# simonamtoft/downsampled-diffusion

Hardware: AMD Instinct MI355X
Metric: images/sec (T=1000 sampling), 256x256 dDDPM-x3 (higher is better)
Workload: dtype f32

## Files before the change

### downsampled-diffusion_amd/csrc/conv_wino.hip

```cpp
#include <atomic>
#include <cstdlib>
#include <type_traits>
#include <utility>

#include "cluster_sync.h"
#include "conv_common.h"
#include "pack_elems.h"

namespace ddk {

__device__ __attribute__((aligned(128))) float g_wino_zero[32];

struct WinoParams {
    const float* src0;
    const float* src1;
    const float* wu;
    const float* bias;
    const float* resid;
    float* out;
    int c0, c1, cin;
    int B, H, W, TH, TW;
    int N, tiles;
    int splits, chunks, chunks_per_split;
    long long slab_stride;
    int post_mish;
    FastDivU dTW, dTH;
    float2* gn_part;
    int cpg, groups;
    const float* gn_gamma;
    const float* gn_beta;
    const float* gn_temb;
    const long long* gn_temb_rows;
    int gn_temb_stride;
    float gn_eps;
    float* cl_rec;
    unsigned* cl_cnt;
    unsigned* cl_fail;
    int cl_np;
    float* cl_slab;
    unsigned* cl_pair;
    const float* r1_x;
    const float* r1_w;
    const float* r1_b;
    int r1_cin, r1_ld;
};

constexpr int WBT = 32, WBN = 64;
constexpr int W_V = 4 * WBT * 32, W_U = 4 * WBN * 32;
constexpr int W_STAGE = W_V + W_U, W_NS = 3;
constexpr int W_LDS_FLOATS = W_NS * W_STAGE;
constexpr int W_TP = WBN + 4;
#ifndef DDK_WINO_LP
#define DDK_WINO_LP 4
#endif
constexpr int W_LP = DDK_WINO_LP;
static_assert(4 * 2 * WBT * W_TP <= W_LDS_FLOATS, "epilogue staging fits");

template <bool DGRAD>
__global__ __launch_bounds__(256) void pack_conv_weight_wino_kernel(const float* __restrict__ w, float* __restrict__ dst, int O, int I,
                                                                     int i_pad, long long total, int lo, int wi) {
    for (long long idx = blockIdx.x * 256LL + threadIdx.x; idx < total; idx += (long long)gridDim.x * 256)
        pack_wino_elem<DGRAD>(w, dst, idx, O, I, i_pad, lo, wi);
}

typedef int i32x4 __attribute__((ext_vector_type(4)));
typedef float f32x4 __attribute__((ext_vector_type(4)));

__device__ __forceinline__ i32x4 make_srd(const void* p, unsigned bytes) {
    const unsigned long long a = reinterpret_cast<unsigned long long>(p);
    i32x4 r;
    r.x = __builtin_amdgcn_readfirstlane((int)(unsigned)a);
    r.y = __builtin_amdgcn_readfirstlane((int)(unsigned)((a >> 32) & 0xFFFFu));
    r.z = __builtin_amdgcn_readfirstlane((int)bytes);
    r.w = 0x00020000;
    return r;
}
constexpr unsigned WINO_OOB = 0x80000000u;

__device__ __forceinline__ void buf_load16(f32x4& d, unsigned voff, const i32x4& srd, unsigned soff) {
    asm volatile("buffer_load_dwordx4 %0, %1, %2, %3 offen" : "=v"(d) : "v"(voff), "s"(srd), "s"(soff) : "memory");
}

__device__ __forceinline__ float4 f4add(float4 a, float4 b) { return make_float4(a.x + b.x, a.y + b.y, a.z + b.z, a.w + b.w); }
typedef float wino_f32x4 __attribute__((ext_vector_type(4)));
__device__ __forceinline__ void st_sc1_f4(float* p, float4 v) {
    const wino_f32x4 t = {v.x, v.y, v.z, v.w};
    asm volatile("global_store_dwordx4 %0, %1, off sc1\n\ts_nop 1" ::"v"(p), "v"(t) : "memory");
}
__device__ __forceinline__ void ld_sc1_f4x4(float4& a, float4& b, float4& c, float4& d, const float* pa, const float* pb, const float* pc,
                                            const float* pd) {
    wino_f32x4 x, y, z, w;
    asm volatile("global_load_dwordx4 %0, %4, off sc1\n\tglobal_load_dwordx4 %1, %5, off sc1\n\tglobal_load_dwordx4 %2, %6, off sc1\n\t"
                 "global_load_dwordx4 %3, %7, off sc1\n\ts_waitcnt vmcnt(0)"
                 : "=&v"(x), "=&v"(y), "=&v"(z), "=&v"(w)
                 : "v"(pa), "v"(pb), "v"(pc), "v"(pd)
                 : "memory");
    a = make_float4(x.x, x.y, x.z, x.w); b = make_float4(y.x, y.y, y.z, y.w);
    c = make_float4(z.x, z.y, z.z, z.w); d = make_float4(w.x, w.y, w.z, w.w);
}
__device__ __forceinline__ float4 f4sub(float4 a, float4 b) { return make_float4(a.x - b.x, a.y - b.y, a.z - b.z, a.w - b.w); }

__device__ unsigned long long g_wino_stamps[8 * 1024];

template <int DBG, bool CL = false>
__global__ __launch_bounds__(512) void conv3x3_wino_kernel(const WinoParams p) {
    extern __shared__ __attribute__((aligned(16))) float smem[];
    unsigned long long r_entry = 0;
    if (DBG) r_entry = __builtin_amdgcn_s_memrealtime();
    const int tid = threadIdx.x, lane = tid & 63;
    const int wid = __builtin_amdgcn_readfirstlane(tid >> 6);
    int tile_m, tile_n, split;
    {
        const int nwg = gridDim.x * gridDim.y * gridDim.z;
        const int bid = blockIdx.x + gridDim.x * (blockIdx.y + gridDim.y * blockIdx.z);
        const int q = nwg >> 3, r = nwg & 7, xcd = bid & 7, idx = bid >> 3;
        const int logical = (xcd < r ? xcd * (q + 1) : r * (q + 1) + (xcd - r) * q) + idx;
        tile_n = logical % gridDim.y;
        const int rest = logical / gridDim.y;
        tile_m = rest % gridDim.x;
        split = rest / gridDim.x;
    }
    const int t0 = tile_m * WBT, n0 = tile_n * WBN;
    const int c_begin = split * p.chunks_per_split;
    const int n_chunks = min(p.chunks, c_begin + p.chunks_per_split) - c_begin;
    const int n_stages = n_chunks * 4;
    const unsigned lds_base = (unsigned)(size_t)(__attribute__((address_space(3))) float*)smem;

// ... 326 lines not shown
                    rs[it][0] = rs[it][1] = make_float4(0.f, 0.f, 0.f, 0.f);
                    if (p.resid) {
                        rs[it][0] = *reinterpret_cast<const float4*>(p.resid + oo[it]);
                        rs[it][1] = *reinterpret_cast<const float4*>(p.resid + oo[it] + p.N);
                    }
                }
            };
            if (wid != 0) { load_affine(); load_resid(); }
            if (wid == 0) {
                asm volatile("s_waitcnt vmcnt(0)" ::: "memory");
                if (lane == 0) __hip_atomic_fetch_add(cnt, 1u, __ATOMIC_RELAXED, __HIP_MEMORY_SCOPE_AGENT);
                load_affine();
                load_resid();
                if (lane == 0 && cl_wait_ge<4>(cnt, (unsigned)p.cl_np, p.cl_fail)) *gave_up = 1;
            }
            __syncthreads();
            const unsigned long long* r0 = reinterpret_cast<const unsigned long long*>(p.cl_rec) +
                                           ((long long)image * p.cl_np * gridDim.y + tile_n) * 16 + gl;
            const bool poisoned = *gave_up != 0;
            float rm[8], rq[8];
            cl_load_stats(r0, (long long)gridDim.y * 16, p.cl_np, rm, rq);
            if (tid == 0) cl_depart(cnt, cnt + 1, (unsigned)p.cl_np);
            const float2 st = cl_merge_stats(rm, rq, p.cl_np, 128.0f * (float)p.cpg, p.gn_eps, poisoned);
            const float gmean = st.x, rstd = st.y;
            auto fin = [&](float4 v) {
                return make_float4(mish_f((v.x - gmean) * rstd * ga.x + be.x) + ts.x, mish_f((v.y - gmean) * rstd * ga.y + be.y) + ts.y,
                                   mish_f((v.z - gmean) * rstd * ga.z + be.z) + ts.z, mish_f((v.w - gmean) * rstd * ga.w + be.w) + ts.w);
            };
#pragma unroll
            for (int it = 0; it < 2; ++it) {
                *reinterpret_cast<float4*>(p.out + oo[it]) = f4add(fin(keep[it][0]), rs[it][0]);
                *reinterpret_cast<float4*>(p.out + oo[it] + p.N) = f4add(fin(keep[it][1]), rs[it][1]);
            }
        }
    }
    if (DBG && tid == 0) {
        asm volatile("s_waitcnt vmcnt(0)" ::: "memory");
        const int wg = (blockIdx.x + gridDim.x * (blockIdx.y + gridDim.y * blockIdx.z)) & 1023;
        g_wino_stamps[wg * 8 + 6] = __builtin_amdgcn_s_memrealtime();
        g_wino_stamps[wg * 8 + 7] = 1;
    }
}

#include "conv_wino2_kernel.inc"
#include "conv_winoT_kernel.inc"

enum { WINO_V_OLD = 0, WINO_V_D = 1, WINO_V_F = 2 };
static int wino_variant(int B, int H, int W, int N) {
#ifdef DDK_TUNING
    if (const char* e = getenv("DDK_WINO_VARIANT")) {
        const int v = atoi(e);
        if (v == WINO_V_OLD || v == WINO_V_D || (v == WINO_V_F && N % 128 == 0)) return v;
    }
#endif
    const long long mt = ceil_div((long long)B * (H / 2) * (W / 2), WBT);
    return (N % 128 == 0 && mt * (N / 128) >= 224) ? WINO_V_F : WINO_V_D;
}
static int wino_nt(int variant) { return variant == WINO_V_F ? 128 : WBN; }
bool conv_wino_ok(int kind, int H, int W, int cin, int N) {
    return kind == DDK_CONV3X3_S1 && H >= 2 && W >= 2 && H % 2 == 0 && W % 2 == 0 && cin > 0 && cin % 32 == 0 && N % 64 == 0;
}

int conv_wino_splits(int B, int H, int W, int cin, int N) {
    const long long tiles = (long long)B * (H / 2) * (W / 2);
    const long long wgs = ceil_div(tiles, WBT) * (N / wino_nt(wino_variant(B, H, W, N)));
    const int chunks = cin / 32;
    int s = 1;
    while (wgs * s < 256 && s * 2 <= chunks) s *= 2;
    const int cps = (int)ceil_div(chunks, s);
    return (int)ceil_div(chunks, cps);
}

static int wino_stats_shape_parts(int B, int H, int W, int cin, int N, int groups) {
    if (!conv_wino_ok(DDK_CONV3X3_S1, H, W, cin, N) || groups <= 0 || N % groups) return 0;
    const int cpg = N / groups, tpi = (H / 2) * (W / 2), nt_w = wino_nt(wino_variant(B, H, W, N));
    if (cpg % 4 || nt_w % cpg || nt_w / cpg > 8 || tpi % WBT || tpi / WBT > 32) return 0;
    return tpi / WBT;
}
int conv_wino_stats_parts(int B, int H, int W, int cin, int N, int groups) {
    if (conv_wino_splits(B, H, W, cin, N) != 1) return 0;
    return wino_stats_shape_parts(B, H, W, cin, N, groups);
}

bool convT_wino_ok(int H, int W, int cin, int N) {
    return H >= 2 && W >= 2 && H % 2 == 0 && W % 2 == 0 && cin > 0 && cin % 32 == 0 && N > 0 && N % WT_NT == 0;
}
int convT_wino_splits(int B, int H, int W, int cin, int N) {
    const long long wgs = ceil_div((long long)B * (H / 2) * (W / 2), WBT) * (N / WT_NT) * 4;
    const int chunks = cin / 32;
    int s = 1;
    while (wgs * s < 256 && s * 2 <= chunks) s *= 2;
    const int cps = (int)ceil_div(chunks, s);
    return (int)ceil_div(chunks, cps);
}
int convT_wino_forward(const ddk_conv_args& a, int splits, hipStream_t st) {
    WinoParams p{};
    p.src0 = a.src0; p.wu = a.weight_wino; p.bias = a.bias; p.out = a.out;
    p.c0 = a.c0; p.c1 = 0; p.cin = a.c0;
    p.B = a.B; p.H = a.H; p.W = a.W; p.TH = a.H / 2; p.TW = a.W / 2;
    p.N = a.N; p.tiles = a.B * p.TH * p.TW;
    p.chunks = p.cin / 32;
    p.chunks_per_split = (int)ceil_div(p.chunks, splits);
    p.splits = (int)ceil_div(p.chunks, p.chunks_per_split);
    p.slab_stride = (long long)a.B * (2 * a.H) * (2 * a.W) * a.N;
    p.dTW = make_fastdiv_u((unsigned)p.TW);
    p.dTH = make_fastdiv_u((unsigned)p.TH);
    if (p.splits > 1) p.out = static_cast<float*>(a.workspace);
    dim3 grid((unsigned)ceil_div(p.tiles, WBT), (unsigned)(a.N / WT_NT), (unsigned)(4 * p.splits));
#ifdef DDK_TUNING
    if (getenv("DDK_WINO_STAMPS")) {
        hipLaunchKernelGGL(convT_wino_kernel<1>, grid, dim3(1024), WT_LDS_FL * sizeof(float), st, p);
        return check_launch("convT_wino_kernel<dbg>");
    }
#endif
    hipLaunchKernelGGL(convT_wino_kernel<0>, grid, dim3(1024), WT_LDS_FL * sizeof(float), st, p);
    return check_launch("convT_wino_kernel");
}

int conv_wino_init_device() {
    DDK_HIP(hipFuncSetAttribute(reinterpret_cast<const void*>(&convT_wino_kernel<0>), hipFuncAttributeMaxDynamicSharedMemorySize,
                                (int)(WT_LDS_FL * sizeof(float))));
#ifdef DDK_TUNING
    DDK_HIP(hipFuncSetAttribute(reinterpret_cast<const void*>(&convT_wino_kernel<1>), hipFuncAttributeMaxDynamicSharedMemorySize,
                                (int)(WT_LDS_FL * sizeof(float))));
#endif
    DDK_HIP(hipFuncSetAttribute(reinterpret_cast<const void*>(&conv3x3_wino_kernel<0>), hipFuncAttributeMaxDynamicSharedMemorySize,
                                (int)(W_LDS_FLOATS * sizeof(float))));
    DDK_HIP(hipFuncSetAttribute(reinterpret_cast<const void*>(&conv3x3_wino_kernel<0, true>), hipFuncAttributeMaxDynamicSharedMemorySize,
                                (int)(W_LDS_FLOATS * sizeof(float))));
    DDK_HIP(hipFuncSetAttribute(reinterpret_cast<const void*>(&conv3x3_wino2_kernel<2, 0, false>), hipFuncAttributeMaxDynamicSharedMemorySize,
                                (int)(W2<2>::LDS_FL * sizeof(float))));
    DDK_HIP(hipFuncSetAttribute(reinterpret_cast<const void*>(&conv3x3_wino2_kernel<2, 0, true>), hipFuncAttributeMaxDynamicSharedMemorySize,
                                (int)(W2<2>::LDS_FL * sizeof(float))));
    DDK_HIP(hipFuncSetAttribute(reinterpret_cast<const void*>(&conv3x3_wino2_kernel<4, 0, false>), hipFuncAttributeMaxDynamicSharedMemorySize,
                                (int)(W2<4>::LDS_FL * sizeof(float))));
    DDK_HIP(hipFuncSetAttribute(reinterpret_cast<const void*>(&conv3x3_wino2_kernel<4, 0, true>), hipFuncAttributeMaxDynamicSharedMemorySize,
                                (int)(W2<4>::LDS_FL * sizeof(float))));
#ifdef DDK_TUNING
#define W2_DBG_ATTR(P_, D_) DDK_HIP(hipFuncSetAttribute(reinterpret_cast<const void*>(&conv3x3_wino2_kernel<P_, D_, false>), \
                                                hipFuncAttributeMaxDynamicSharedMemorySize, (int)(W2<P_>::LDS_FL * sizeof(float))))
    W2_DBG_ATTR(2, 1); W2_DBG_ATTR(2, 7); W2_DBG_ATTR(2, 9); W2_DBG_ATTR(2, 15); W2_DBG_ATTR(2, 17);
    W2_DBG_ATTR(4, 1); W2_DBG_ATTR(4, 7); W2_DBG_ATTR(4, 9); W2_DBG_ATTR(4, 15); W2_DBG_ATTR(4, 17);
#undef W2_DBG_ATTR
    DDK_HIP(hipFuncSetAttribute(reinterpret_cast<const void*>(&conv3x3_wino_kernel<1>), hipFuncAttributeMaxDynamicSharedMemorySize, (int)(W_LDS_FLOATS * sizeof(float))));
    DDK_HIP(hipFuncSetAttribute(reinterpret_cast<const void*>(&conv3x3_wino_kernel<2>), hipFuncAttributeMaxDynamicSharedMemorySize, (int)(W_LDS_FLOATS * sizeof(float))));
    DDK_HIP(hipFuncSetAttribute(reinterpret_cast<const void*>(&conv3x3_wino_kernel<3>), hipFuncAttributeMaxDynamicSharedMemorySize, (int)(W_LDS_FLOATS * sizeof(float))));
    DDK_HIP(hipFuncSetAttribute(reinterpret_cast<const void*>(&conv3x3_wino_kernel<4>), hipFuncAttributeMaxDynamicSharedMemorySize, (int)(W_LDS_FLOATS * sizeof(float))));
#endif
    return DDK_OK;
}

int conv_wino_cluster_np(int B, int H, int W, int cin, int N, int groups) {
    const int np = conv_wino_stats_parts(B, H, W, cin, N, groups);
    if (np <= 0 || np > 8) return 0;
    const int nt_w = wino_nt(wino_variant(B, H, W, N));
    if (N / groups > 32 || nt_w % (N / groups)) return 0;
    if (nt_w / (N / groups) > 8) return 0;
    const long long mt = (long long)B * np, nt = N / nt_w;
    if ((mt * nt) % 8) return 0;
    const long long run = mt * nt / 8;
    const long long per_round = run < 32 ? run : 32;
    if (run % (np * nt) || per_round % (np * nt)) return 0;
    return np;
}
int conv_wino_cluster_split_np(int B, int H, int W, int cin, int N, int groups, int* splits_out) {
    if (!conv_wino_ok(DDK_CONV3X3_S1, H, W, cin, N)) return 0;
    const int splits = conv_wino_splits(B, H, W, cin, N);
    if (splits_out) *splits_out = splits;
    if (splits <= 1 || splits > 4) return 0;
    const int np = wino_stats_shape_parts(B, H, W, cin, N, groups);
    if (np <= 0 || np > 8) return 0;
    const int variant = wino_variant(B, H, W, N);
    if (variant != WINO_V_D) return 0;
    const int nt_w = wino_nt(variant);
    if (N / groups > 32 || nt_w % (N / groups) || nt_w / (N / groups) > 8) return 0;
    const long long mt = (long long)B * np, nt = N / nt_w;
    if (mt * nt * splits > 256) return 0;
    return np;
}
size_t conv_wino_cluster_pair_words(int B, int H, int W, int N) {
    return (size_t)ceil_div((long long)B * (H / 2) * (W / 2), WBT) * (size_t)(N / WBN) * 16;
}
size_t conv_wino_cluster_ws_floats(int B, int H, int W, int N) {
    const long long mt = (long long)B * (H / 2) * (W / 2) / WBT, nt = N / WBN;
    return (size_t)(mt * nt * 32 + (long long)B * nt * 16);
}

bool conv_wino_cluster_device_ok() {
    static std::atomic<int> cached[64];
    int dev = 0;
    if (hipGetDevice(&dev) != hipSuccess || dev < 0 || dev >= 64) return false;
    int v = cached[dev].load(std::memory_order_relaxed);
    if (v == 0) {
        int cus = 0, xccs = 0;
        bool ok = hipDeviceGetAttribute(&cus, hipDeviceAttributeMultiprocessorCount, dev) == hipSuccess && cus == 256;
        ok = ok && hipDeviceGetAttribute(&xccs, hipDeviceAttributeNumberOfXccs, dev) == hipSuccess && xccs == 8;
        ok = ok && !getenv("HSA_CU_MASK") && !getenv("ROC_GLOBAL_CU_MASK");
        (void)hipGetLastError();
        v = ok ? 1 : 2;
        cached[dev].store(v, std::memory_order_relaxed);
    }
    return v == 1;
}

bool conv_wino_variant_new(int B, int H, int W, int N) { return wino_variant(B, H, W, N) != WINO_V_OLD; }

int conv_wino_forward(const ddk_conv_args& a, int splits, hipStream_t st, const WinoGnFuse* fuse) {
    WinoParams p{};
    if (fuse) {
        const int np = splits == 1 ? conv_wino_cluster_np(a.B, a.H, a.W, a.c0 + a.c1, a.N, fuse->groups)
                                   : conv_wino_cluster_split_np(a.B, a.H, a.W, a.c0 + a.c1, a.N, fuse->groups, nullptr);
        DDK_REQUIRE(np > 0 && !a.post_mish && !a.gn_partials, "conv(wino): shape not eligible for the in-launch GroupNorm");
        if (splits > 1) {
            DDK_REQUIRE(fuse->pairs && a.workspace && aligned16(a.workspace) && !fuse->res_x,
                        "conv(wino, cluster): a split shape needs pair counters and the slab workspace");
// ... 236 lines not shown
```

### downsampled-diffusion_amd/csrc/conv_wino2_kernel.inc

```

template <int... I, class F>
__device__ __forceinline__ void static_for_impl(std::integer_sequence<int, I...>, F&& f) { (f(std::integral_constant<int, I>{}), ...); }
template <int N, class F>
__device__ __forceinline__ void static_for(F&& f) { static_for_impl(std::make_integer_sequence<int, N>{}, f); }

#ifndef DDK_WINO2_LP_F
#define DDK_WINO2_LP_F 8
#endif
#ifndef DDK_WINO2_LP_D
#define DDK_WINO2_LP_D 4
#endif
template <int P>
struct W2 {
    static constexpr int NT = 256 / P;
    static constexpr int NB = NT / 32;
    static constexpr int SPC = 16 / P;
    static constexpr int SPR = 4 / P;
    static constexpr int V_FL = P * WBT * 32;
    static constexpr int U_FL = P * NT * 32;
    static constexpr int STAGE = V_FL + U_FL;
    static constexpr int PPI = NT / 8;
    static constexpr int TP = NT + 4;
    static constexpr int T_FL = 4 * 2 * WBT * TP;
    static constexpr int LDS_FL = (3 * STAGE > T_FL + 320) ? 3 * STAGE : T_FL + 320;
    static constexpr int QUADS = NT / 4;
    static constexpr int ITEMS = 2 * WBT * QUADS / 512;
    static constexpr int LPL = P == 2 ? DDK_WINO2_LP_F : DDK_WINO2_LP_D;
    static constexpr int LPM = (32 - 4 * LPL) / 8;
    static_assert(4 * LPL + 8 * LPM == 32 && LPL % 2 == 0 && LPM % 2 == 0, "piece split: (8,0), (4,2) or (0,4)");
};
#ifndef DDK_WINO2_STAGGER
#define DDK_WINO2_STAGGER 1
#endif
constexpr bool W2_STAGGER = DDK_WINO2_STAGGER != 0;

__device__ unsigned long long g_wino_timeline[12 * 8 * 2];

template <int P, int DBG, bool CL>
__global__ __launch_bounds__(768) void conv3x3_wino2_kernel(const WinoParams p) {
    using G = W2<P>;
    constexpr int NT = G::NT, SPC = G::SPC, SPR = G::SPR, STAGE = G::STAGE, V_FL = G::V_FL;
    extern __shared__ __attribute__((aligned(16))) float smem[];
    unsigned long long r_entry = 0;
    if (DBG) r_entry = __builtin_amdgcn_s_memrealtime();
    const int tid = threadIdx.x, lane = tid & 63;
    const int wid = __builtin_amdgcn_readfirstlane(tid >> 6);
    int tile_m, tile_n, split;
    {
        const int nwg = gridDim.x * gridDim.y * gridDim.z;
        const int bid = blockIdx.x + gridDim.x * (blockIdx.y + gridDim.y * blockIdx.z);
        const int q = nwg >> 3, r = nwg & 7, xcd = bid & 7, idx = bid >> 3;
        const int logical = (xcd < r ? xcd * (q + 1) : r * (q + 1) + (xcd - r) * q) + idx;
        tile_n = logical % gridDim.y;
        const int rest = logical / gridDim.y;
        tile_m = rest % gridDim.x;
        split = rest / gridDim.x;
    }
    const int t0 = tile_m * WBT, n0 = tile_n * NT;
    const int c_begin = split * p.chunks_per_split;
    const int n_chunks = min(p.chunks, c_begin + p.chunks_per_split) - c_begin;
    const int n_stages = n_chunks * SPC;
    const unsigned lds_base = (unsigned)(size_t)(__attribute__((address_space(3))) float*)smem;
    const int prow = lane >> 3, ppos = lane & 7;
    const unsigned uv_even = (unsigned)((prow * 32 + ((ppos ^ (prow >> 1)) << 2)) * 4);
    const unsigned uv_odd = (unsigned)((prow * 32 + ((ppos ^ (4 + (prow >> 1))) << 2)) * 4);
    auto issue_u = [&](int T, int buf, int g_first, auto count) {
        const int chunk = c_begin + T / SPC, st = T % SPC;
        const float* base = p.wu + (((long long)chunk * 16 + P * st) * p.N + n0) * 32;
        const unsigned dst = lds_base + (unsigned)((buf * STAGE + V_FL) * 4);
#pragma unroll
        for (int j = 0; j < decltype(count)::value; ++j) {
            const int g = g_first + j;
            const int image = g / G::PPI, rb = g % G::PPI;
            lds_dma16_s(base + ((long long)image * p.N + rb * 8) * 32, (j & 1) ? uv_odd : uv_even, dst + (unsigned)(g * 1024));
        }
    };

    if (wid >= 8) {
        const int lw = wid - 8;
        const int lt = lw * 64 + lane;
        const int t = lt >> 3, cq = lt & 7;
        __builtin_amdgcn_s_setprio(3);
        const int g = t0 + t;
        const bool tile_ok = g < p.tiles;
        const unsigned gg = tile_ok ? (unsigned)g : 0u;
        const unsigned tmp = fdiv_u(gg, p.dTW);
        const int tx = (int)(gg - tmp * (unsigned)p.TW);
        const unsigned bq = fdiv_u(tmp, p.dTH);
        const int ty = (int)(tmp - bq * (unsigned)p.TH), b = (int)bq;
        const int py0 = 2 * ty - 1, px0 = 2 * tx - 1;
        const int pix0 = (b * p.H + py0) * p.W + px0;
        unsigned mask = 0;
#pragma unroll
        for (int dy = 0; dy < 4; ++dy)
#pragma unroll
            for (int dx = 0; dx < 4; ++dx)
                if (tile_ok && (unsigned)(py0 + dy) < (unsigned)p.H && (unsigned)(px0 + dx) < (unsigned)p.W) mask |= 1u << (dy * 4 + dx);
        const i32x4 srd0 = make_srd(p.src0, (unsigned)((long long)p.B * p.H * p.W * p.c0 * 4));
        const i32x4 srd1 = make_srd(p.src1 ? p.src1 : p.src0, (unsigned)((long long)p.B * p.H * p.W * (p.src1 ? p.c1 : p.c0) * 4));
        unsigned voff[16];
        int cur_src = -1;
        auto set_source = [&](int which) {
            const int cs = which == 0 ? p.c0 : p.c1;
#pragma unroll
            for (int dy = 0; dy < 4; ++dy)
#pragma unroll
                for (int dx = 0; dx < 4; ++dx)
                    voff[dy * 4 + dx] = ((mask >> (dy * 4 + dx)) & 1u) ? (unsigned)(((pix0 + dy * p.W + dx) * cs + cq * 4) * 4) : WINO_OOB;
            cur_src = which;
        };
        const int v_off = t * 32 + ((cq ^ ((t >> 1) & 7)) << 2);
        f32x4 d[16];
        auto load_row = [&](int chunk, int row) {
            const int cc = chunk << 5;
            const bool first = cc < p.c0;
            if ((first ? 0 : 1) != cur_src) set_source(first ? 0 : 1);
            const unsigned soff = (unsigned)((first ? cc : cc - p.c0) * 4);
            i32x4 srd;
            srd.x = first ? srd0.x : srd1.x; srd.y = first ? srd0.y : srd1.y; srd.z = first ? srd0.z : srd1.z; srd.w = srd0.w;
#pragma unroll
            for (int dy = 0; dy < 4; ++dy)
                if (dy == row) {
// ... 169 lines not shown
                            frag(a[1], b[1], As, Bs, 0);
                            __builtin_amdgcn_sched_barrier(0);
                            mma4(acc[(s + SPC - 1) % SPC], a[0], b[0]);
                        }
                        frag(a[0], b[0], As, Bs, 1);
                        __builtin_amdgcn_sched_barrier(0);
                        mma4(acc[s], a[1], b[1]);
                        dma();
                        frag(a[1], b[1], As, Bs, 2);
                        __builtin_amdgcn_sched_barrier(0);
                        mma4(acc[s], a[0], b[0]);
                        frag(a[0], b[0], As, Bs, 3);
                        __builtin_amdgcn_sched_barrier(0);
                        mma4(acc[s], a[1], b[1]);
                    }
                    if (more && !(DBG & 4)) wait_vmcnt<G::LPM>(); else wait_vmcnt<0>();
                    unsigned long long tA = 0, tB = 0;
                    if (DBG) { asm volatile("s_memtime %0\n\ts_waitcnt lgkmcnt(0)" : "=s"(tA)::"memory"); }
                    __builtin_amdgcn_s_barrier();
                    if (DBG) { asm volatile("s_memtime %0\n\ts_waitcnt lgkmcnt(0)" : "=s"(tB)::"memory"); c_wait += tB - tA; if (c_mma == 0) c_mma = tA; }
                    if ((DBG & 16) && blockIdx.x + blockIdx.y + blockIdx.z == 0 && S >= 8 && S < 16 && lane == 0) {
                        g_wino_timeline[(wid * 8 + (S - 8)) * 2] = tA;
                        g_wino_timeline[(wid * 8 + (S - 8)) * 2 + 1] = tB;
                    }
                    buf = nbuf;
                    ++S;
                });
            }
            if (STG) mma4(acc[SPC - 1], a[0], b[0]);
        };
        if (W2_STAGGER && wid >= 4) mloop(std::true_type{}); else mloop(std::false_type{});
        if (DBG && lane == 0 && wid == 0) {
            const int wg = (blockIdx.x + gridDim.x * (blockIdx.y + gridDim.y * blockIdx.z)) & 1023;
            unsigned long long tE;
            asm volatile("s_memtime %0\n\ts_waitcnt lgkmcnt(0)" : "=s"(tE)::"memory");
            g_wino_stamps[wg * 8 + 0] = r_entry;
            g_wino_stamps[wg * 8 + 1] = r_loop0;
            g_wino_stamps[wg * 8 + 2] = __builtin_amdgcn_s_memrealtime();
            g_wino_stamps[wg * 8 + 3] = c_wait;
            g_wino_stamps[wg * 8 + 4] = tE - c_mma;
            g_wino_stamps[wg * 8 + 5] = (unsigned long long)n_stages;
        }
    }
    {
        constexpr int TP = G::TP;
#pragma unroll
        for (int r = 0; r < 16; ++r) {
            const int row = (r & 3) + 8 * (r >> 2) + 4 * (lane >> 5);
            const int col = nb * 32 + (lane & 31);
            if constexpr (P == 4) {
                float* Ts = smem + pp * (2 * WBT * TP);
                const float m0 = acc[0][r], m1 = acc[1][r], m2 = acc[2][r], m3 = acc[3][r];
                Ts[row * TP + col] = (m0 + m1) + m2;
                Ts[(WBT + row) * TP + col] = (m1 - m2) - m3;
            } else {
                const float l0 = acc[0][r], l1 = acc[2][r], l2 = acc[4][r], l3 = acc[6][r];
                const float h0 = acc[1][r], h1 = acc[3][r], h2 = acc[5][r], h3 = acc[7][r];
                const float tl0 = (l0 + l1) + l2, tl1 = (l1 - l2) - l3;
                const float th0 = (h0 + h1) + h2, th1 = (h1 - h2) - h3;
                float* B0 = smem + (pp * 2 + 0) * (2 * WBT * TP);
                float* B1 = smem + (pp * 2 + 1) * (2 * WBT * TP);
                if (pp == 0) {
                    B0[row * TP + col] = tl0 + th0;          B0[(WBT + row) * TP + col] = tl1 + th1;
                    B1[row * TP + col] = -th0;               B1[(WBT + row) * TP + col] = -th1;
                } else {
                    B0[row * TP + col] = tl0;                B0[(WBT + row) * TP + col] = tl1;
                    B1[row * TP + col] = tl0 - th0;          B1[(WBT + row) * TP + col] = tl1 - th1;
                }
            }
        }
    }
    __syncthreads();

    constexpr int TP = G::TP, QUADS = G::QUADS, ITEMS = G::ITEMS;
    constexpr bool CLS = CL && P == 4;
    const bool partner = CLS && split > 0;
    const bool direct = p.splits == 1 || (CLS && !partner);
    float* outp = p.splits == 1 ? p.out : CLS ? p.cl_slab + (long long)(split - 1) * p.slab_stride : p.out + (long long)split * p.slab_stride;
    float4 keep[ITEMS][2];
    long long oo[ITEMS];
    int opix[ITEMS];
    const int cq = tid & (QUADS - 1);
    const int gn = n0 + cq * 4;
#pragma unroll
    for (int it = 0; it < ITEMS; ++it) {
        const int item = tid + it * 512;
        const int t = item / (2 * QUADS), a = (item / QUADS) & 1;
        const int g = t0 + t;
        keep[it][0] = keep[it][1] = make_float4(0.f, 0.f, 0.f, 0.f);
        oo[it] = -1;
        opix[it] = 0;
        if (g >= p.tiles || gn >= p.N) continue;
        const float* tp = smem + (a * WBT + t) * TP + cq * 4;
        const float4 q0 = *reinterpret_cast<const float4*>(tp);
        const float4 q1 = *reinterpret_cast<const float4*>(tp + 1 * (2 * WBT * TP));
        const float4 q2 = *reinterpret_cast<const float4*>(tp + 2 * (2 * WBT * TP));
        const float4 q3 = *reinterpret_cast<const float4*>(tp + 3 * (2 * WBT * TP));
        float4 y0, y1;
        if constexpr (P == 4) {
            y0 = f4add(f4add(q0, q1), q2);
            y1 = f4sub(f4sub(q1, q2), q3);
        } else {
            y0 = f4add(q0, q2);
            y1 = f4add(q1, q3);
        }
        const unsigned tmp = fdiv_u((unsigned)g, p.dTW);
        const int tx = g - (int)tmp * p.TW;
        const unsigned bq = fdiv_u(tmp, p.dTH);
        const int ty = (int)tmp - (int)bq * p.TH;
        const long long o0 = ((((long long)bq * p.H + 2 * ty + a) * p.W) + 2 * tx) * p.N + gn;
        oo[it] = o0;
        opix[it] = ((int)bq * p.H + 2 * ty + a) * p.W + 2 * tx;
        if (direct) {
            if (p.bias) {
                const float4 bb = *reinterpret_cast<const float4*>(p.bias + gn);
                y0 = f4add(y0, bb);
                y1 = f4add(y1, bb);
            }
            if (!CL && p.resid) {
                y0 = f4add(y0, *reinterpret_cast<const float4*>(p.resid + o0));
                y1 = f4add(y1, *reinterpret_cast<const float4*>(p.resid + o0 + p.N));
            }
            if (p.post_mish) {
                y0 = make_float4(mish_f(y0.x), mish_f(y0.y), mish_f(y0.z), mish_f(y0.w));
                y1 = make_float4(mish_f(y1.x), mish_f(y1.y), mish_f(y1.z), mish_f(y1.w));
            }
        }
        if (!CL) {
            *reinterpret_cast<float4*>(outp + o0) = y0;
            *reinterpret_cast<float4*>(outp + o0 + p.N) = y1;
        } else if (CLS && partner) {
            st_sc1_f4(outp + o0, y0);
            st_sc1_f4(outp + o0 + p.N, y1);
        }
        keep[it][0] = y0;
        keep[it][1] = y1;
    }
    if (CLS && p.splits > 1) {
        unsigned* pair = p.cl_pair + ((long long)tile_m * gridDim.y + tile_n) * 16;
        if (partner) {
            asm volatile("s_waitcnt vmcnt(0)" ::: "memory");
            __syncthreads();
            if (tid == 0) __hip_atomic_fetch_add(pair, 1u, __ATOMIC_RELAXED, __HIP_MEMORY_SCOPE_AGENT);
            return;
        }
        int* pair_gave_up = reinterpret_cast<int*>(smem + G::T_FL + 258);
        if (tid == 0) {
            *pair_gave_up = 0;
            const unsigned want = (unsigned)p.splits - 1u;
            if (cl_wait_ge<2>(pair, want, p.cl_fail)) *pair_gave_up = 1;
            __hip_atomic_store(pair, 0u, __ATOMIC_RELAXED, __HIP_MEMORY_SCOPE_AGENT);
        }
        __syncthreads();
        const bool pair_poisoned = *pair_gave_up != 0;
        for (int s = 1; s < p.splits; ++s) {
            const float* sl = p.cl_slab + (long long)(s - 1) * p.slab_stride;
            static_assert(ITEMS % 2 == 0, "two items per load group");
#pragma unroll
            for (int it = 0; it < ITEMS; it += 2) {
                float4 a0, a1, b0, b1;
                ld_sc1_f4x4(a0, a1, b0, b1, sl + oo[it], sl + oo[it] + p.N, sl + oo[it + 1], sl + oo[it + 1] + p.N);
                keep[it][0] = f4add(keep[it][0], a0);
                keep[it][1] = f4add(keep[it][1], a1);
                keep[it + 1][0] = f4add(keep[it + 1][0], b0);
                keep[it + 1][1] = f4add(keep[it + 1][1], b1);
            }
        }
        if (pair_poisoned) {
#pragma unroll
            for (int it = 0; it < ITEMS; ++it) keep[it][0].x = __builtin_nanf("");
        }
    }
    if (CL || p.gn_part) {
        const int qpg = p.cpg >> 2;
        const int gl = cq / qpg;
        float* red = smem + G::T_FL;
        auto group_sum = [&](float v, float* rd) {
            for (int o = 1; o < qpg; o <<= 1) v += __shfl_xor(v, o, 64);
#pragma unroll
            for (int o = QUADS; o < 64; o <<= 1) v += __shfl_xor(v, o, 64);
            if (lane < QUADS && (cq & (qpg - 1)) == 0) rd[wid * 16 + gl] = v;
            asm volatile("s_waitcnt lgkmcnt(0)\n\ts_barrier" ::: "memory");
            float t = rd[gl];
#pragma unroll
            for (int w = 1; w < 8; ++w) t += rd[w * 16 + gl];
            return t;
        };
        auto sum4 = [](float4 v) { return (v.x + v.y) + (v.z + v.w); };
        const float inv = 1.0f / (float)(4 * WBT * p.cpg);
        float s1 = 0.f;
#pragma unroll
        for (int it = 0; it < ITEMS; ++it) s1 += sum4(keep[it][0]) + sum4(keep[it][1]);
// ... 116 lines not shown
```

### downsampled-diffusion_amd/csrc/ddk_internal.h

```cpp
#pragma once
#include <hip/hip_runtime.h>

#include <cstdarg>
#include <cstddef>
#include <cstdint>
#include <cstdio>

#include "ddk.h"

#ifdef DDK_HOST_SANITIZE
#include "host_sanitize.h"
#endif

namespace ddk {

void set_error(const char* fmt, ...);

inline int fail_arg(const char* what) {
    set_error("bad argument: %s", what);
    return DDK_ERR_ARG;
}

inline int check_launch(const char* what) {
    hipError_t e = hipGetLastError();
// ... 62 lines not shown
    return v;
}

__device__ __forceinline__ float block_sum(float v, float* red) {
    v = wave_sum(v);
    const int lane = threadIdx.x & 63, wid = threadIdx.x >> 6, nw = blockDim.x >> 6;
    __syncthreads();
    if (lane == 0) red[wid] = v;
    __syncthreads();
    float t = (lane < nw) ? red[lane] : 0.0f;
    t = wave_sum(t);
    return t;
}

__device__ __forceinline__ float block_max(float v, float* red) {
    v = wave_max(v);
    const int lane = threadIdx.x & 63, wid = threadIdx.x >> 6, nw = blockDim.x >> 6;
    __syncthreads();
    if (lane == 0) red[wid] = v;
    __syncthreads();
    float t = (lane < nw) ? red[lane] : -INFINITY;
    t = wave_max(t);
    return t;
}

int ensure_device_init();
int conv_init_device();
int wgrad_init_device();

size_t conv_workspace_bytes(int kind, int B, int H, int W, int cin, int N);
struct ConvLnFold {
    const float* c1;
    const float* c2;
    float eps;
};
struct WinoGnFuse {
    const float* gamma;
    const float* beta;
    const float* temb;
    const long long* temb_rows;
    int temb_stride;
    float eps;
    int groups;
    float* records;
    unsigned* counters;
    unsigned* fail;
    unsigned* pairs = nullptr;
    const float* res_x = nullptr;
    const float* res_w = nullptr;
    const float* res_b = nullptr;
    int res_cin = 0, res_ld = 0;
};
bool conv_ln_fold_ok(int B, int H, int W, int cin, int N);
int conv_forward(const ddk_conv_args& a, hipStream_t st, const ConvLnFold* ln = nullptr, const WinoGnFuse* fuse = nullptr);
int conv_splits(int kind, int B, int H, int W, int cin, int N);
bool conv_wino_ok(int kind, int H, int W, int cin, int N);
int conv_wino_splits(int B, int H, int W, int cin, int N);
int conv_wino_forward(const ddk_conv_args& a, int splits, hipStream_t st, const WinoGnFuse* fuse = nullptr);
int conv_wino_cluster_np(int B, int H, int W, int cin, int N, int groups);
int conv_wino_cluster_split_np(int B, int H, int W, int cin, int N, int groups, int* splits_out);
size_t conv_wino_cluster_pair_words(int B, int H, int W, int N);
bool conv_wino_variant_new(int B, int H, int W, int N);
bool conv_wino_cluster_device_ok();
size_t conv_wino_cluster_ws_floats(int B, int H, int W, int N);
unsigned conv_wino_cluster_timeouts();
unsigned conv_first_cluster_timeouts();
unsigned level_chain_cluster_timeouts();
unsigned attention_cluster_timeouts();
constexpr size_t CL_PAIR_WORDS = 128 * 16;
inline size_t cl_fail_offset(int B) { return (size_t)B * 8 * 16; }
inline size_t cl_front_floats(int B) { return cl_fail_offset(B) + 16; }
inline size_t cl_chain_offset(int B) { return cl_front_floats(B); }
inline size_t cl_pair_offset(int B) { return cl_chain_offset(B) + (size_t)B * 64; }
inline size_t cl_attn_offset(int B) { return cl_pair_offset(B) + CL_PAIR_WORDS; }
inline size_t cl_counter_floats(int B) { return cl_attn_offset(B) + (size_t)B * 4 * 32; }
struct ClWords { unsigned* counters; unsigned* fail; };
inline ClWords cl_words(float* cl, int B) { return {reinterpret_cast<unsigned*>(cl), reinterpret_cast<unsigned*>(cl + cl_fail_offset(B))}; }
int cluster_fail_check(unsigned* word, hipStream_t st, const char* who, const char* tail);
bool convT_wino_ok(int H, int W, int cin, int N);
int convT_wino_splits(int B, int H, int W, int cin, int N);
int convT_wino_forward(const ddk_conv_args& a, int splits, hipStream_t st);
int conv_wino_init_device();
int conv_wino_stats_parts(int B, int H, int W, int cin, int N, int groups);
bool conv_first_ok(int cin, int N, int H, int W, int groups);
int conv_first(const float* x, const float* wp, const float* bias, float* out, float* gn_partials, int B, int H, int W, int cin, int N,
               int groups, int64_t* counter, int64_t* t_cur, hipStream_t st);
int conv_first_init_device();
bool conv_first_gn_ok(int cin, int N, int H, int W, int groups);
size_t conv_first_gn_ws_floats(int B, int H, int W);
int conv_first_gn(const float* x, const float* wp, const float* bias, const float* gamma, const float* beta, const float* temb,
                  int temb_stride, const long long* temb_rows, float eps, float* out, int B, int H, int W, int cin, int N, int groups,
                  float* records, unsigned* counters, unsigned* fail, int64_t* counter, int64_t* t_cur, hipStream_t st);
bool conv1x1_sm_ok(long long M, int c0, int c1, int N);
int conv1x1_sm(const float* src0, int c0, const float* src1, int c1, const float* w, const float* bias, const float* resid, float* out,
               long long M, int N, const ConvLnFold* ln, hipStream_t st);
int conv1x1_sm_init_device();
bool conv1x1_stream_ok(long long M, int cin, int N);
int conv1x1_stream(const float* x, int cin, const float* w, const float* bias, const float* dmish_src, const float* resid, float* out,
                   float* mish_out, long long M, int N, int pre_mish, int post_mish, hipStream_t st);
bool conv1x1_ws_ok(long long M, int K, int N);
int conv1x1_ws(const float* x, const float* w, const float* bias, const float* resid, float* out, long long M, int N, const ConvLnFold* ln,
               hipStream_t st, int images = 0);
int conv1x1_ws_init_device();
struct AddendSlabs {
    int n = 1;
    long long stride = 0;
    const float* bias = nullptr;
};
bool conv_gn_local_ok(int H, int W, int cin, int c0, int N, int groups);
int conv_gn_local(const float* src0, int c0, const float* src1, int c1, const float* w, const float* bias, const float* gamma,
                  const float* beta, const float* temb, int temb_stride, const long long* temb_rows, const float* addend, float* out,
                  int B, int H, int W, int N, int groups, float eps, hipStream_t st, const AddendSlabs& as = AddendSlabs(),
                  const AddendSlabs& src_slabs = AddendSlabs());
int conv_gn_local_init_device();
bool conv_gn_wlocal_ok(int H, int W, int cin, int c0, int N, int groups);
int conv_gn_wlocal(const float* src0, int c0, const float* src1, int c1, const float* w, const float* bias, const float* gamma,
                   const float* beta, const float* temb, int temb_stride, const long long* temb_rows, const float* addend, float* out,
                   int B, int H, int W, int N, int groups, float eps, hipStream_t st, const AddendSlabs& as = AddendSlabs(),
                   const AddendSlabs& src_slabs = AddendSlabs());
double conv_flops(int kind, int B, int H, int W, int cin, int N);
size_t groupnorm_workspace_bytes(int B, int HW, int C, int groups);
int gn_train_nsplit(int HW, int cpg);
int gn_stats_partials(const float* x, float* part, int B, int HW, int C, int groups, int ns, hipStream_t st);
int groupnorm_mish(const float* x, const float* gamma, const float* beta, const float* temb, int temb_stride,
                   const float* addend, float* out, int B, int HW, int C, int groups, float eps, void* ws, size_t ws_bytes,
                   hipStream_t st, const long long* temb_rows = nullptr);
int groupnorm_mish_ex(const float* x, int nslab, long long slab_stride, const float* cbias, const float* gamma,
                      const float* beta, const float* temb, int temb_stride, const float* addend, float* out, int B, int HW, int C,
                      int groups, float eps, void* ws, size_t ws_bytes, hipStream_t st, const long long* temb_rows = nullptr);
int groupnorm_mish_parts(const float* x, const float* part, int np, const float* gamma, const float* beta, const float* temb,
                         int temb_stride, const float* addend, float* out, int B, int HW, int C, int groups, float eps, hipStream_t st,
                         const long long* temb_rows = nullptr, const float* rc_x = nullptr, const float* rc_w = nullptr,
                         const float* rc_b = nullptr, int rc_cin = 0, int rc_ld = 0);
int chan_layernorm(const float* x, const float* g, const float* b, float* out, long long M, int C, float eps, hipStream_t st);
int groupnorm_mish_generic(const float* x, const float* gamma, const float* beta, const float* temb, int temb_stride, const float* addend,
                           float* out, int B, int HW, int CP, int C, int groups, float eps, hipStream_t st, const long long* temb_rows = nullptr);
int chan_layernorm_generic(const float* x, const float* g, const float* b, float* out, long long M, int CP, int C, float eps, hipStream_t st);
int unary(int op, const float* x, float* out, long long n, hipStream_t st);
int add(const float* a, const float* b, float* out, long long n, hipStream_t st);
int avgpool2(const float* x, float* out, int B, int H, int W, int C, hipStream_t st);
int upsample_nearest2(const float* x, float* out, int B, int H, int W, int C, hipStream_t st);
size_t linattn_context_workspace_bytes(int B, int HW, int heads);
int linattn_context(const float* qkv, float* ctx, int B, int HW, int heads, void* workspace, size_t workspace_bytes, hipStream_t st,
                    bool kv_only = false);
bool attn_fold_ok(int C, int heads);
bool attn_kvctx_ok(int B, int HW, int C, int heads);
size_t attn_kvctx_workspace_bytes(int B, int HW);
int attn_kvctx(const float* x, const float* w_kv, const float* c1, const float* c2, float ln_eps, float* ctx, int B, int HW, void* workspace,
               size_t workspace_bytes, hipStream_t st);
size_t attn_fold_out_floats(int B);
int attn_fold(const float* ctx, const float* wqg, const float* c1q, const float* c2q, const float* wout, const float* bout, float* A,
              float* a1, float* a2, int B, int C, int heads, hipStream_t st);
int linattn_apply(const float* qkv, const float* ctx, float* out, int B, int HW, int heads, hipStream_t st);
int linattn_fused_small(const float* qkv, float* ctx, float* out, int B, int HW, int heads, hipStream_t st);
bool attn_split_ok(int B, int HW, int C, int heads);
size_t attn_split_counter_words(int B);
size_t attn_split_record_floats(int B);
int attn_split(const float* x, const float* w, const float* c1, const float* c2, float ln_eps, float* ctx, float* out, int B, int HW, int C,
               unsigned* counters, float* records, unsigned* fail, hipStream_t st);
bool linattn_small_qkv_ok(int HW, int C);
int linattn_small_qkv_init_device();
int qkv_operand_pack(const float* lnw, float* wop, int heads, int cp, hipStream_t st);
int linattn_small_qkv(const float* x, const float* wop, const float* c1, const float* c2, float ln_eps, float* ctx, float* out, int B, int HW,
                      int C, int heads, hipStream_t st);
int time_mlp(const int64_t* t, const float* freqs, const float* w1t, const float* b1, const float* w2t, const float* b2,
             float* act, float* raw, int B, int dim, hipStream_t st);
// ... 117 lines not shown
```

### downsampled-diffusion_amd/csrc/unet_plan.hip

```cpp
#include <algorithm>
#include <mutex>
#include <string>
#include <vector>

#include "ddk_internal.h"
#include "level_chain.h"

namespace ddk {

constexpr int HEADS = 4;
constexpr int HIDDEN = HEADS * 32;
constexpr int GROUPS = 8;
constexpr float GN_EPS = 1e-5f, LN_EPS = 1e-5f;

static inline int pad32(int c) { return (c + 31) / 32 * 32; }

enum PackKind { PK_COPY = 0, PK_CONV = 1, PK_CONVT = 2, PK_LINEAR_T = 3, PK_WINO = 4, PK_LOCAL = 5, PK_WLOCAL = 6, PK_FIRST = 7, PK_CONVT_WINO = 8,
                PK_ROWS = 9 , PK_LOCAL1 = 10 ,
                PK_CONVT_LOCAL = 11  };

struct Slot {
    std::string name;
    long long numel;
    int kind;
// ... 12 lines not shown
    size_t wl = 0;
    bool has_wl = false;
    size_t wwl = 0;
    bool has_wwl = false;
    size_t wf = 0;
    bool has_wf = false;
    size_t wl1 = 0;
    bool has_wl1 = false;
    size_t wtl = 0;
    bool has_wtl = false;
};
struct NormW { size_t g = 0, b = 0; int c_real = 0; };
struct ResW {
    int ci = 0, ci_pad = 0, co = 0, temb_off = 0, ci_real = 0, co_real = 0;
    ConvW c1, c2, res;
    NormW n1, n2;
    bool has_res = false;
};
struct AttnW {
    int c = 0, c_real = 0;
    NormW ln;
    ConvW qkv, out;
    size_t qkv_lnw = 0, ln_c1 = 0, ln_c2 = 0;
    size_t qkv_op = 0;
};

}

using namespace ddk;

struct ChainKey {
    StepKind kind;
    const void* bufs[14];
    const void* ws;
    const void* noise;
    int B, H, W, t_start, device;
    unsigned long long pack_epoch;
    int restore_n = 0;
    bool restore_mask = false;
    int restore_gray = 0;
    bool operator==(const ChainKey& o) const {
        for (int i = 0; i < 14; ++i)
            if (bufs[i] != o.bufs[i]) return false;
        return kind == o.kind && ws == o.ws && noise == o.noise && B == o.B && H == o.H && W == o.W && t_start == o.t_start &&
               device == o.device && pack_epoch == o.pack_epoch && restore_n == o.restore_n && restore_mask == o.restore_mask && restore_gray == o.restore_gray;
    }
};
struct SamplerGraph {
    ChainKey key;
    hipGraph_t graph = nullptr;
    hipGraphExec_t exec = nullptr;
    hipGraph_t graph_multi = nullptr;
    hipGraphExec_t exec_multi = nullptr;
    hipEvent_t done = nullptr;
    unsigned long long last_use = 0;
};
constexpr int SAMPLER_MULTI = 16;

struct ddk_unet {
    std::mutex mu;
    std::vector<SamplerGraph> graphs;
    unsigned long long use_clock = 0;
    unsigned long long pack_epoch = 0;
    struct {
        const void* ws = nullptr;
        int t_start = -1, B = 0, H = 0, W = 0;
        unsigned long long pack_epoch = 0;
        std::vector<int64_t> map;
    } table;
    ddk_unet_config cfg;
    int cluster_gn = 1;
    int cluster_limit = 1 << 30;
    int cluster_np_max = 8;
    bool cluster_split = true;
    bool attn_kvctx = true;
    bool attn_split = true;
    bool fold_down_reduce = false;
    bool restore_fused = true;
    bool first_gn = true;
    int level_chain = 9;
    int level_chain_max_batch = 32;
    int attn_fold_min_hw = 256;
    bool attn_fold = true;
    bool generic = false;
    std::vector<int> dimp;
    std::vector<Slot> slots;
    size_t packed_floats = 0;
    int L = 0;
    std::vector<int> dims;
    int time_dim = 0, temb_total = 0;
    size_t freqs = 0, w1t = 0, b1 = 0, w2t = 0, b2 = 0, temb_wt = 0, temb_bias = 0;
    std::vector<ResW> down_res, up_res;
    std::vector<AttnW> down_attn, up_attn;
    std::vector<ConvW> down_conv, up_conv;
    ResW mid1, mid2;
    AttnW mid_attn;
    ConvW final_conv;
    NormW final_norm;
    size_t final_w = 0, final_b = 0;

    size_t alloc(size_t n) {
        const size_t o = packed_floats;
        packed_floats += (n + 3) / 4 * 4;
        return o;
    }
    size_t add_copy(const std::string& name, long long n) {
        const size_t o = alloc((size_t)n);
        slots.push_back(Slot{name, n, PK_COPY, o, 0, 0, 0, 0, 0, 0, 0});
        return o;
    }
    void add_copy_at(const std::string& name, long long n, size_t off) {
        slots.push_back(Slot{name, n, PK_COPY, off, 0, 0, 0, 0, 0, 0, 0});
    }
    ConvW add_conv(const std::string& prefix, int cout, int cin, int k, bool bias, bool gn_follows = false, int split = 0, bool local = false) {
        ConvW c;
        c.cin = cin; c.cin_pad = split > 0 ? pad32(split) + pad32(cin - split) : pad32(cin); c.cout = cout;
        const int cout_rows = pad32(cout);
        c.w = alloc((size_t)cout_rows * k * k * c.cin_pad);
        Slot sl{prefix + "weight", (long long)cout * cin * k * k, PK_CONV, c.w, cout, cin, k, k, c.cin_pad, 0, 0};
        if (split > 0 && c.cin_pad != cin) { sl.split = split; sl.split_pad = pad32(split); }
        slots.push_back(sl);
        c.has_bias = bias;
        if (bias) {
            c.b = alloc((size_t)cout_rows);
            slots.push_back(Slot{prefix + "bias", cout, PK_COPY, c.b, 0, 0, 0, 0, 0, 0, 0});
        }
        if (generic) return c;
        if (k == 1 && bias && cout % 32 == 0 && c.cin_pad == cin && cin % 32 == 0) {
            c.wl1 = alloc((size_t)cout * c.cin_pad);
            c.has_wl1 = true;
            slots.push_back(Slot{prefix + "weight", (long long)cout * cin, PK_LOCAL1, c.wl1, cout, cin, 1, 1, c.cin_pad, 0, 0});
        }
        if (k == 3 && cout % 64 == 0) {
            c.wu = alloc((size_t)16 * cout * c.cin_pad);
            c.has_wu = true;
            slots.push_back(Slot{prefix + "weight", (long long)cout * cin * k * k, PK_WINO, c.wu, cout, cin, k, k, c.cin_pad, 0, 0});
        }
        if (k == 3 && (gn_follows || local) && cout % 32 == 0) {
            c.wl = alloc((size_t)9 * cout * c.cin_pad);
            c.has_wl = true;
            slots.push_back(Slot{prefix + "weight", (long long)cout * cin * k * k, PK_LOCAL, c.wl, cout, cin, k, k, c.cin_pad, 0, 0});
            if (gn_follows && (c.cin_pad <= 320 || c.cin_pad == 512)) {
                c.wwl = alloc((size_t)16 * cout * c.cin_pad);
                c.has_wwl = true;
                slots.push_back(Slot{prefix + "weight", (long long)cout * cin * k * k, PK_WLOCAL, c.wwl, cout, cin, k, k, c.cin_pad, 0, 0});
            }
        }
        return c;
    }
    ConvW add_convT(const std::string& prefix, int ch, bool local = false) {
        ConvW c;
        c.cin = ch; c.cin_pad = pad32(ch); c.cout = ch;
        c.w = alloc((size_t)16 * pad32(ch) * pad32(ch));
        slots.push_back(Slot{prefix + "weight", (long long)16 * ch * ch, PK_CONVT, c.w, ch, ch, 4, 4, pad32(ch), 0, 0});
        c.has_bias = true;
        c.b = alloc((size_t)pad32(ch));
        slots.push_back(Slot{prefix + "bias", ch, PK_COPY, c.b, 0, 0, 0, 0, 0, 0, 0});
        if (local && ch % 32 == 0 && !generic) {
            c.wtl = alloc((size_t)16 * ch * ch);
            c.has_wtl = true;
            slots.push_back(Slot{prefix + "weight", (long long)16 * ch * ch, PK_CONVT_LOCAL, c.wtl, ch, ch, 4, 4, ch, 0, 0});
        }
        if (ch % 128 == 0) {
            c.wu = alloc((size_t)36 * ch * ch);
            c.has_wu = true;
            slots.push_back(Slot{prefix + "weight", (long long)16 * ch * ch, PK_CONVT_WINO, c.wu, ch, ch, 4, 4, ch, 0, 0});
// ... 49 lines not shown
        return a;
    }
};

static int total_temb(const ddk_unet& u) {
    int tot = 0;
    for (int l = 0; l < u.L; ++l) tot += 2 * u.dims[l + 1];
    tot += 2 * u.dims[u.L];
    for (int i = 0; i < u.L - 1; ++i) tot += 2 * u.dims[u.L - 1 - i];
    return tot;
}

extern "C" ddk_unet* ddk_unet_create(const ddk_unet_config* cfg) {
    if (!cfg || cfg->n_levels < 1 || cfg->n_levels > 8 || cfg->in_ch < 1 || cfg->chan < 8 || cfg->chan % 8 ||
        cfg->chan > 512) {
        set_error("unet_create: need 1 <= n_levels <= 8, in_ch >= 1, unet_chan a multiple of 8 in [8, 512]");
        return nullptr;
    }
    for (int i = 0; i < cfg->n_levels; ++i)
        if (cfg->mults[i] < 1) { set_error("unet_create: unet_dims entries must be >= 1"); return nullptr; }
    if (cfg->mults[0] != 1) {
        set_error("unet_create: unet_dims[0] must be 1 (the reference's final Block(dim, dim) meets dim * unet_dims[0] channels "
                  "otherwise and raises, unet.py:69-72)");
        return nullptr;
    }
    {
        int ndev = 0;
        if (hipGetDeviceCount(&ndev) == hipSuccess && ndev > 0 && ensure_device_init() != DDK_OK) return nullptr;
        (void)hipGetLastError();
    }
    ddk_unet* u = new ddk_unet();
    u->cfg = *cfg;
    u->L = cfg->n_levels;
    u->generic = cfg->chan % 32 != 0;
    for (int i = 0; i < cfg->n_levels; ++i)
        if (cfg->chan * cfg->mults[i] > 512) { set_error("unet_create: level widths above 512 channels are not supported"); delete u; return nullptr; }
    u->dims.push_back(cfg->in_ch);
    for (int i = 0; i < u->L; ++i) u->dims.push_back(cfg->chan * cfg->mults[i]);
    for (int d : u->dims) u->dimp.push_back(u->generic ? pad32(d) : d);
    u->time_dim = cfg->chan;
    u->temb_total = total_temb(*u);
    const int td = u->time_dim;

    u->freqs = u->add_copy("@sinusoidal_freqs", td / 2);
    u->w1t = u->alloc((size_t)td * 4 * td);
    u->slots.push_back(Slot{"time_mlp.1.weight", (long long)4 * td * td, PK_LINEAR_T, u->w1t, 4 * td, td, 0, 0, 0, 4 * td, 0});
    u->b1 = u->add_copy("time_mlp.1.bias", 4 * td);
    u->w2t = u->alloc((size_t)4 * td * td);
    u->slots.push_back(Slot{"time_mlp.3.weight", (long long)4 * td * td, PK_LINEAR_T, u->w2t, td, 4 * td, 0, 0, 0, td, 0});
    u->b2 = u->add_copy("time_mlp.3.bias", td);
    u->temb_wt = u->alloc((size_t)td * u->temb_total);
    u->temb_bias = u->alloc((size_t)u->temb_total);

    int cur = 0;
    for (int l = 0; l < u->L; ++l) {
        const std::string p = "downs." + std::to_string(l) + ".";
        const int ci = u->dims[l], co = u->dims[l + 1];
        u->down_res.push_back(u->add_res(p + "0.", ci, co, cur));
        if (l == 0 && ci <= 8 && co <= 256 && !u->generic) {
            ConvW& c1 = u->down_res[0].c1;
            const int K2 = (9 * ci + 1) / 2;
            c1.wf = u->alloc((size_t)(co / 32) * K2 * 64);
            c1.has_wf = true;
            u->slots.push_back(Slot{p + "0.block1.block.0.weight", (long long)co * ci * 9, PK_FIRST, c1.wf, co, ci, 3, 3, 0, 0, 0});
        }
        u->down_res.push_back(u->add_res(p + "1.", co, co, cur));
        u->down_attn.push_back(u->add_attn(p + "2.", co));
        if (l < u->L - 1) u->down_conv.push_back(u->add_conv(p + "3.conv.", co, co, 3, true, false, 0, l == u->L - 2));
    }
    const int mid = u->dims[u->L];
    u->mid1 = u->add_res("mid_block1.", mid, mid, cur);
    u->mid_attn = u->add_attn("mid_attn.", mid);
    u->mid2 = u->add_res("mid_block2.", mid, mid, cur);
    for (int i = 0; i < u->L - 1; ++i) {
        const std::string p = "ups." + std::to_string(i) + ".";
        const int din = u->dims[u->L - 1 - i], dout = u->dims[u->L - i];
        u->up_res.push_back(u->add_res(p + "0.", 2 * dout, din, cur, dout));
        u->up_res.push_back(u->add_res(p + "1.", din, din, cur));
        u->up_attn.push_back(u->add_attn(p + "2.", din));
        u->up_conv.push_back(u->add_convT(p + "3.conv.", din, i == 0));
    }
    u->final_conv = u->add_conv("final_conv.0.block.0.", cfg->chan, cfg->chan, 3, true, true);
    u->final_norm = u->add_norm("final_conv.0.block.1.weight", "final_conv.0.block.1.bias", cfg->chan);
    if (u->generic) {
        u->final_w = u->alloc((size_t)cfg->in_ch * pad32(cfg->chan));
        u->slots.push_back(Slot{"final_conv.1.weight", (long long)cfg->in_ch * cfg->chan, PK_ROWS, u->final_w, cfg->in_ch, cfg->chan, 0, 0, 0,
                                pad32(cfg->chan), 0});
    } else {
        u->final_w = u->add_copy("final_conv.1.weight", (long long)cfg->in_ch * cfg->chan);
    }
    u->final_b = u->add_copy("final_conv.1.bias", cfg->in_ch);
    if (cur != u->temb_total) {
        set_error("unet_create: internal temb accounting mismatch");
        delete u;
        return nullptr;
    }
    return u;
}

static void drop_graphs(ddk_unet* u) {
    for (SamplerGraph& g : u->graphs) {
        if (g.exec) (void)hipGraphExecDestroy(g.exec);
        if (g.graph) (void)hipGraphDestroy(g.graph);
        if (g.exec_multi) (void)hipGraphExecDestroy(g.exec_multi);
        if (g.graph_multi) (void)hipGraphDestroy(g.graph_multi);
        if (g.done) (void)hipEventDestroy(g.done);
    }
    u->graphs.clear();
    u->table.ws = nullptr;
}

extern "C" void ddk_unet_destroy(ddk_unet* u) {
    if (!u) return;
    if (!u->graphs.empty()) (void)hipDeviceSynchronize();
    drop_graphs(u);
    delete u;
}

extern "C" int ddk_sampler_invalidate(ddk_unet* u) {
    DDK_REQUIRE(u, "sampler_invalidate: null plan");
    std::lock_guard<std::mutex> lock(u->mu);
    if (!u->graphs.empty()) DDK_HIP(hipDeviceSynchronize());
    drop_graphs(u);
    return DDK_OK;
}
static void destroy_entry(SamplerGraph& g) {
    if (g.done) { (void)hipEventSynchronize(g.done); (void)hipEventDestroy(g.done); }
    if (g.exec) (void)hipGraphExecDestroy(g.exec);
    if (g.graph) (void)hipGraphDestroy(g.graph);
    if (g.exec_multi) (void)hipGraphExecDestroy(g.exec_multi);
    if (g.graph_multi) (void)hipGraphDestroy(g.graph_multi);
}

extern "C" int ddk_sampler_release_workspace(ddk_unet* u, const void* workspace) {
    DDK_REQUIRE(u && workspace, "sampler_release_workspace: arguments");
    std::lock_guard<std::mutex> lock(u->mu);
    for (size_t i = 0; i < u->graphs.size();) {
        if (u->graphs[i].key.ws == workspace) {
            destroy_entry(u->graphs[i]);
            u->graphs.erase(u->graphs.begin() + (long)i);
        } else {
            ++i;
        }
    }
    if (u->table.ws == workspace) u->table.ws = nullptr;
    return DDK_OK;
}

extern "C" int ddk_unet_set_option(ddk_unet* u, int option, int value) {
    DDK_REQUIRE(u, "unet_set_option: null plan");
    static const struct {
        int option;
        bool drops_graphs;
        void (*set)(ddk_unet&, int);
    } options[] = {
        {DDK_OPT_CLUSTER_GROUPNORM, true, [](ddk_unet& p, int v) { p.cluster_gn = v < 0 ? 0 : v > 2 ? 2 : v; }},
        {DDK_OPT_ATTENTION_FOLD, true, [](ddk_unet& p, int v) { p.attn_fold = v != 0; }},
        {DDK_OPT_ATTENTION_KV_CONTEXT, true, [](ddk_unet& p, int v) { p.attn_kvctx = v != 0; }},
        {DDK_OPT_FIRST_GROUPNORM, true, [](ddk_unet& p, int v) { p.first_gn = v != 0; }},
        {DDK_OPT_RESTORE_FUSED_TAIL, true, [](ddk_unet& p, int v) { p.restore_fused = v != 0; }},
        {DDK_OPT_ATTENTION_SPLIT, true, [](ddk_unet& p, int v) { p.attn_split = v != 0; }},
        {DDK_OPT_LEVEL_CHAIN, true, [](ddk_unet& p, int v) {
             p.level_chain = v == 1 ? 9 : v == 2 ? 1 : v == 3 ? 15 : v == 4 ? 6 : v == 8 ? 2 : v == 16 ? 4 : v != 0 ? 9 : 0;
         }},
        {DDK_OPT_FOLD_DOWNSAMPLE_REDUCE, true, [](ddk_unet& p, int v) { p.fold_down_reduce = v != 0; }},
        {10, true, [](ddk_unet& p, int v) { p.level_chain_max_batch = v; }},
        {9, true, [](ddk_unet& p, int v) { p.attn_fold_min_hw = v; }},
        {2, false, [](ddk_unet& p, int v) { p.cluster_limit = v; }},
        {4, true, [](ddk_unet& p, int v) { p.cluster_np_max = v; }},
        {11, true, [](ddk_unet& p, int v) { p.cluster_split = v != 0; }},
    };
    for (const auto& o : options) {
        if (o.option != option) continue;
        std::lock_guard<std::mutex> lock(u->mu);
        if (o.drops_graphs) {
            if (!u->graphs.empty()) DDK_HIP(hipDeviceSynchronize());
            drop_graphs(u);
        }
        o.set(*u, value);
        return DDK_OK;
    }
    return fail_arg("unet_set_option: unknown option");
}
extern "C" unsigned ddk_debug_cluster_timeouts(void) {
    unsigned sum = 0;
    for (unsigned v : {ddk::conv_wino_cluster_timeouts(), ddk::conv_first_cluster_timeouts(), ddk::level_chain_cluster_timeouts(),
                       ddk::attention_cluster_timeouts()}) {
        if (v == ~0u) return ~0u;
        sum += v;
    }
    return sum;
}
extern "C" int ddk_unet_num_slots(const ddk_unet* u) { return u ? (int)u->slots.size() : 0; }
extern "C" const char* ddk_unet_slot_name(const ddk_unet* u, int slot) {
    return (u && slot >= 0 && slot < (int)u->slots.size()) ? u->slots[slot].name.c_str() : nullptr;
}
extern "C" long long ddk_unet_slot_numel(const ddk_unet* u, int slot) {
    return (u && slot >= 0 && slot < (int)u->slots.size()) ? u->slots[slot].numel : -1;
}
extern "C" size_t ddk_unet_packed_bytes(const ddk_unet* u) { return u ? u->packed_floats * sizeof(float) : 0; }

__global__ __launch_bounds__(64) void ln_fold_kernel(const float* __restrict__ w, const float* __restrict__ g, const float* __restrict__ b,
                                                     float* __restrict__ wg, float* __restrict__ c1, float* __restrict__ c2, int C, int cp) {
    const int n = blockIdx.x;
    float s1 = 0.f, s2 = 0.f;
    for (int c = threadIdx.x; c < cp; c += 64) {
        const float wv = w[(long long)n * cp + c];
        const float gv = c < C ? g[c] : 0.f, bv = c < C ? b[c] : 0.f;
        wg[(long long)n * cp + c] = wv * gv;
        s1 += wv * gv;
        s2 += wv * bv;
    }
    s1 = wave_sum(s1);
    s2 = wave_sum(s2);
    if (threadIdx.x == 0) { c1[n] = s1; c2[n] = s2; }
}

static int fold_attn(const AttnW& a, float* P, hipStream_t st) {
    hipLaunchKernelGGL(ln_fold_kernel, dim3(3 * HIDDEN), dim3(64), 0, st, P + a.qkv.w, P + a.ln.g, P + a.ln.b, P + a.qkv_lnw, P + a.ln_c1,
                       P + a.ln_c2, a.c, pad32(a.c));
    DDK_TRY(check_launch("ln_fold_kernel"));
    return qkv_operand_pack(P + a.qkv_lnw, P + a.qkv_op, HEADS, pad32(a.c), st);
}

static void weights_changed(const ddk_unet* u) {
    ddk_unet* m = const_cast<ddk_unet*>(u);
    std::lock_guard<std::mutex> lock(m->mu);
    ++m->pack_epoch;
}

extern "C" int ddk_unet_finalize_pack(const ddk_unet* u, void* packed, ddk_stream_t s) {
    DDK_REQUIRE(u && packed, "unet_finalize_pack: arguments");
    weights_changed(u);
    for (const AttnW& a : u->attn_all) DDK_TRY(fold_attn(a, static_cast<float*>(packed), as_stream(s)));
    return DDK_OK;
}

extern "C" int ddk_unet_pack_slot(const ddk_unet* u, int slot, const float* canonical, void* packed, ddk_stream_t s) {
    DDK_REQUIRE(u && canonical && packed && slot >= 0 && slot < (int)u->slots.size(), "unet_pack_slot: arguments");
    const Slot& sl = u->slots[slot];
    float* dst = static_cast<float*>(packed) + sl.off;
    weights_changed(u);
    int rc;
    switch (sl.kind) {
        case PK_COPY:
            DDK_HIP(hipMemcpyAsync(dst, canonical, (size_t)sl.numel * sizeof(float), hipMemcpyDeviceToDevice, as_stream(s)));
            rc = DDK_OK;
            break;
        case PK_CONV:
            rc = sl.split > 0 ? ddk_pack_conv_weight_split(canonical, dst, sl.O, sl.I, sl.KH, sl.KW, sl.i_pad, sl.split, sl.split_pad, s)
                              : ddk_pack_conv_weight(canonical, dst, sl.O, sl.I, sl.KH, sl.KW, sl.i_pad, s);
            break;
        case PK_CONVT: rc = sl.i_pad == sl.I ? ddk_pack_convT_weight(canonical, dst, sl.I, sl.O, s)
                                             : ddk_pack_convT_weight_padded(canonical, dst, sl.I, sl.O, sl.i_pad, s); break;
        case PK_ROWS:
            DDK_HIP(hipMemcpy2DAsync(dst, (size_t)sl.ld * sizeof(float), canonical, (size_t)sl.I * sizeof(float), (size_t)sl.I * sizeof(float),
                                     (size_t)sl.O, hipMemcpyDeviceToDevice, as_stream(s)));
            rc = DDK_OK;
            break;
        case PK_LINEAR_T: rc = ddk_pack_linear_T(canonical, dst, sl.O, sl.I, sl.ld, sl.col0, s); break;
        case PK_WINO: rc = ddk_pack_conv_weight_wino(canonical, dst, sl.O, sl.I, sl.i_pad, s); break;
        case PK_LOCAL: rc = ddk_pack_conv_weight_local(canonical, dst, sl.O, sl.I, sl.i_pad, s); break;
        case PK_LOCAL1: rc = ddk_pack_conv1x1_weight_local(canonical, dst, sl.O, sl.I, sl.i_pad, s); break;
        case PK_CONVT_LOCAL: rc = ddk_pack_convT_weight_local(canonical, dst, sl.I, sl.O, s); break;
        case PK_WLOCAL: rc = ddk_pack_conv_weight_wino_local(canonical, dst, sl.O, sl.I, sl.i_pad, s); break;
        case PK_FIRST: rc = ddk_pack_conv_weight_first(canonical, dst, sl.O, sl.I, s); break;
        case PK_CONVT_WINO: rc = ddk_pack_convT_weight_wino(canonical, dst, sl.I, sl.O, sl.i_pad, s); break;
        default: return fail_arg("unet_pack_slot: slot kind");
    }
    DDK_TRY(rc);
    if (sl.attn >= 0) DDK_TRY(fold_attn(u->attn_all[sl.attn], static_cast<float*>(packed), as_stream(s)));
    return DDK_OK;
}

namespace ddk {

struct Layout {
    size_t act = 0;
    size_t qkv = 0, o = 0, ctx = 0, splitk = 0, gn_ws = 0, cl = 0, chain = 0;
    std::vector<size_t> skip;
    size_t xpad = 0, temb = 0, tact = 0;
    size_t off_A = 0, off_B = 0, off_C = 0, off_raw = 0, off_a1 = 0, off_res = 0, off_xn = 0, off_qkv = 0, off_o = 0, off_ctx = 0,
           off_splitk = 0, off_gn = 0, off_xpad = 0, off_temb = 0, off_tact = 0, off_cl = 0, off_chain = 0;
    std::vector<size_t> off_skip;
    size_t total = 0;
};

static size_t al4(size_t n) { return (n + 3) / 4 * 4; }

static void upd(size_t& m, size_t v) { if (v > m) m = v; }

static bool convT_wino_use(int B, int H, int W, int cin, int N) {
    return convT_wino_ok(H, W, cin, N) && convT_wino_splits(B, H, W, cin, N) <= 2;
}
static bool use_wino(const ConvW& cw, int H, int W, int cin, int N) {
    return cw.has_wu && conv_wino_ok(DDK_CONV3X3_S1, H, W, cin, N);
}
static size_t conv3_ws_floats(const ConvW& cw, int B, int H, int W, int cin, int N) {
    if (!use_wino(cw, H, W, cin, N)) return conv_workspace_bytes(DDK_CONV3X3_S1, B, H, W, cin, N) / 4;
    const int s = conv_wino_splits(B, H, W, cin, N);
    return s > 1 ? (size_t)s * B * H * W * N : 0;
}

constexpr int CHAIN_BUFS = 18;
constexpr int CHAIN8_BUFS = 5;

static void res_sizes(const ResW& r, int B, int H, int W, Layout& ly) {
    const size_t M = (size_t)B * H * W;
    upd(ly.act, M * r.co);
    upd(ly.splitk, conv3_ws_floats(r.c1, B, H, W, r.ci_pad, r.co));
    upd(ly.splitk, conv3_ws_floats(r.c2, B, H, W, r.co, r.co));
    if (r.has_res) upd(ly.splitk, conv_workspace_bytes(DDK_CONV1X1, B, H, W, r.ci_pad, r.co) / 4);
    upd(ly.gn_ws, groupnorm_workspace_bytes(B, H * W, r.co, GROUPS) / 4);
    upd(ly.gn_ws, (size_t)2 * GROUPS * (M / 128 + 1));
    upd(ly.cl, cl_counter_floats(B) + conv_wino_cluster_ws_floats(B, H, W, r.co));
    if (H * W % 128 == 0 && H * W / 128 <= 8) upd(ly.cl, cl_counter_floats(B) + conv_first_gn_ws_floats(B, H, W));
}

static void attn_sizes(const AttnW& a, int B, int H, int W, Layout& ly) {
    const size_t M = (size_t)B * H * W;
    upd(ly.act, M * a.c);
    upd(ly.qkv, M * 3 * HIDDEN);
    upd(ly.o, M * HIDDEN);
    upd(ly.ctx, (size_t)B * HEADS * 32 * 32);
    upd(ly.splitk, linattn_context_workspace_bytes(B, H * W, HEADS) / 4);
    if (attn_kvctx_ok(B, H * W, a.c, HEADS)) upd(ly.splitk, attn_kvctx_workspace_bytes(B, H * W) / 4);
    upd(ly.splitk, conv_workspace_bytes(DDK_CONV1X1, B, H, W, a.c, 3 * HIDDEN) / 4);
    upd(ly.splitk, conv_workspace_bytes(DDK_CONV1X1, B, H, W, HIDDEN, a.c) / 4);
    if ((H * W == 64 || H * W == 256) && B <= 32) upd(ly.cl, cl_counter_floats(B) + attn_split_record_floats(B));
}

static bool chain_plain(const ResW& r, bool wino) {
    return r.ci == 256 && r.co == 256 && !r.has_res && r.c1.has_bias && r.c2.has_bias && (wino ? r.c1.has_wwl && r.c2.has_wwl : r.c1.has_wl && r.c2.has_wl);
}
static bool chain_att(const AttnW& a) { return a.c == 256 && a.out.has_wl1 && a.out.has_bias; }
static bool chain_cat(const ResW& r, bool wino) {
    return r.ci == 512 && r.ci_pad == 512 && r.co == 256 && r.has_res && r.res.has_wl1 && r.res.has_bias && r.c1.cin_pad == 512 && r.c1.has_bias &&
           r.c2.has_bias && (wino ? r.c1.has_wwl && r.c2.has_wwl : r.c1.has_wl && r.c2.has_wl);
}
static bool level_chain_shape_ok(const ddk_unet& u, int H0, int W0) {
    if (u.generic || u.L < 2) return false;
    const int sh = u.L - 1;
    if ((H0 >> sh) != 4 || (W0 >> sh) != 4 || (H0 & ((1 << sh) - 1)) || (W0 & ((1 << sh) - 1))) return false;
    if (u.dimp[u.L] != 256 || u.dimp[u.L - 1] != 256 || GROUPS != 8) return false;
    return chain_plain(u.down_res[2 * sh], false) && chain_plain(u.down_res[2 * sh + 1], false) && chain_plain(u.mid1, false) &&
           chain_plain(u.mid2, false) && chain_plain(u.up_res[1], false) && chain_att(u.down_attn[sh]) && chain_att(u.mid_attn) &&
           chain_att(u.up_attn[0]) && chain_cat(u.up_res[0], false);
}
static bool level8_chain_shape_ok(const ddk_unet& u, int H0, int W0) {
    if (u.generic || u.L < 3) return false;
    const int sh = u.L - 2;
    if ((H0 >> sh) != 8 || (W0 >> sh) != 8 || (H0 & ((1 << sh) - 1)) || (W0 & ((1 << sh) - 1))) return false;
    if (u.dimp[sh + 1] != 256 || u.dimp[sh] != 256 || u.dimp[sh + 2] != 256 || GROUPS != 8) return false;
    return chain_plain(u.down_res[2 * sh], true) && chain_plain(u.down_res[2 * sh + 1], true) && chain_att(u.down_attn[sh]) &&
           chain_cat(u.up_res[2], true) && chain_plain(u.up_res[3], true) && chain_att(u.up_attn[1]);
}

static Layout make_layout(const ddk_unet& u, int B, int H0, int W0) {
    Layout ly;
    int H = H0, W = W0;
    ly.skip.resize(u.L);
    for (int l = 0; l < u.L; ++l) {
        res_sizes(u.down_res[2 * l], B, H, W, ly);
        res_sizes(u.down_res[2 * l + 1], B, H, W, ly);
        attn_sizes(u.down_attn[l], B, H, W, ly);
        ly.skip[l] = al4((size_t)B * H * W * u.dimp[l + 1]);
        if (l < u.L - 1) {
            upd(ly.splitk, conv_workspace_bytes(DDK_CONV3X3_S2, B, H, W, u.dimp[l + 1], u.dimp[l + 1]) / 4);
            H /= 2; W /= 2;
            upd(ly.act, (size_t)B * H * W * u.dimp[l + 1]);
        }
    }
    res_sizes(u.mid1, B, H, W, ly);
    attn_sizes(u.mid_attn, B, H, W, ly);
    res_sizes(u.mid2, B, H, W, ly);
    for (int i = 0; i < u.L - 1; ++i) {
        res_sizes(u.up_res[2 * i], B, H, W, ly);
        res_sizes(u.up_res[2 * i + 1], B, H, W, ly);
        attn_sizes(u.up_attn[i], B, H, W, ly);
        const int c = pad32(u.up_conv[i].cout);
        upd(ly.splitk, conv_workspace_bytes(DDK_CONVT4X4_S2, B, H, W, c, c) / 4);
        H *= 2; W *= 2;
        upd(ly.act, (size_t)B * H * W * c);
    }
    upd(ly.act, (size_t)B * H * W * pad32(u.cfg.chan));
    upd(ly.splitk, conv3_ws_floats(u.final_conv, B, H, W, pad32(u.cfg.chan), pad32(u.cfg.chan)));
    upd(ly.gn_ws, groupnorm_workspace_bytes(B, H * W, pad32(u.cfg.chan), GROUPS) / 4);
    upd(ly.gn_ws, (size_t)2 * GROUPS * ((size_t)B * H * W / 128 + 1));
    ly.xpad = al4((size_t)B * H0 * W0 * pad32(u.cfg.in_ch));
    ly.temb = al4((size_t)B * u.temb_total);
    ly.tact = al4((size_t)B * u.time_dim);
    ly.act = al4(ly.act); ly.qkv = al4(ly.qkv); ly.o = al4(ly.o); ly.ctx = al4(ly.ctx);
    ly.splitk = al4(ly.splitk); ly.gn_ws = al4(ly.gn_ws); ly.cl = al4(ly.cl);
    if (level_chain_shape_ok(u, H0, W0)) ly.chain = (size_t)CHAIN_BUFS * B * 16 * 256;
    if (level8_chain_shape_ok(u, H0, W0)) upd(ly.chain, (size_t)CHAIN8_BUFS * B * 64 * 256);

    size_t off = 0;
    auto take = [&](size_t n) { const size_t o = off; off += n; return o; };
    ly.off_A = take(ly.act); ly.off_B = take(ly.act); ly.off_C = take(ly.act);
    ly.off_raw = take(ly.act); ly.off_a1 = take(ly.act); ly.off_res = take(ly.act); ly.off_xn = take(ly.act);
    ly.off_qkv = take(ly.qkv); ly.off_o = take(ly.o); ly.off_ctx = take(ly.ctx);
    ly.off_splitk = take(ly.splitk); ly.off_gn = take(ly.gn_ws); ly.off_cl = take(ly.cl); ly.off_chain = take(ly.chain);
    ly.off_xpad = take(ly.xpad); ly.off_temb = take(ly.temb); ly.off_tact = take(ly.tact);
    ly.off_skip.resize(u.L);
    for (int l = 0; l < u.L; ++l) ly.off_skip[l] = take(ly.skip[l]);
    ly.total = off;
    return ly;
}

struct Ctx {
    const ddk_unet& u;
    const float* P;
    float* W;
    const Layout& ly;
    int B;
    hipStream_t st;
    const float* temb;
    const long long* temb_rows;
    bool allow_cluster = false;
    int n_cluster = 0;
    const float* x_first = nullptr;
    const float* x_padded = nullptr;

    ddk_conv_args conv_args(int kind, const ConvW& cw, const float* src0, int c0, const float* src1, int c1, float* out, int H, int Wd, int N,
                            const float* weight_override = nullptr) const {
        ddk_conv_args a{};
        a.kind = kind;
        a.src0 = src0; a.src1 = src1; a.c0 = c0; a.c1 = c1;
        a.weight = weight_override ? weight_override : P + cw.w;
        a.bias = cw.has_bias ? P + cw.b : nullptr;
        a.out = out;
        a.B = B; a.H = H; a.W = Wd; a.N = N;
        a.workspace = W + ly.off_splitk;
        a.workspace_bytes = ly.splitk * sizeof(float);
        if (kind == DDK_CONV3X3_S1 && !weight_override && use_wino(cw, H, Wd, c0 + c1, N)) a.weight_wino = P + cw.wu;
        if (kind == DDK_CONVT4X4_S2 && !weight_override && cw.has_wu && !src1 && convT_wino_use(B, H, Wd, c0, N)) a.weight_wino = P + cw.wu;
        return a;
    }
    WinoGnFuse gn_fuse(const NormW& n, const float* temb_shift, const long long* rows) const {
        float* cl = W + ly.off_cl;
        const ClWords w = cl_words(cl, B);
        return WinoGnFuse{P + n.g, P + n.b, temb_shift, rows, u.temb_total, GN_EPS, GROUPS, cl + cl_counter_floats(B), w.counters, w.fail};
    }
};

static int run_conv(Ctx& c, int kind, const ConvW& cw, const float* src0, int c0, const float* src1, int c1, const float* resid,
                    float* out, int H, int W, int N, const float* weight_override = nullptr, const ConvLnFold* ln = nullptr) {
    ddk_conv_args a = c.conv_args(kind, cw, src0, c0, src1, c1, out, H, W, N, weight_override);
    a.resid = resid;
    return conv_forward(a, c.st, ln);
}
static int run_conv_slabs(Ctx& c, int kind, const ConvW& cw, const float* src0, int c0, const float* src1, int c1, float* out, int H, int W, int N,
                          int splits, AddendSlabs& left) {
    ddk_conv_args a = c.conv_args(kind, cw, src0, c0, src1, c1, out, H, W, N);
    a.bias = nullptr;
    a.defer_reduce = 1;
    const int s = kind == DDK_CONV3X3_S2 ? 2 : 1;
    left = AddendSlabs{splits, (long long)c.B * (H / s) * (W / s) * N, cw.has_bias ? c.P + cw.b : nullptr};
    return conv_forward(a, c.st);
}
static int run_conv_parts(Ctx& c, const ConvW& cw, const float* src0, int c0, const float* src1, int c1, float* raw, int H, int W, int N) {
    ddk_conv_args a = c.conv_args(DDK_CONV3X3_S1, cw, src0, c0, src1, c1, raw, H, W, N);
    a.gn_partials = c.W + c.ly.off_gn;
    a.gn_groups = GROUPS;
    return conv_forward(a, c.st);
}

enum ConvGnPath {
    CG_GENERIC,
    CG_LOCAL,
    CG_WLOCAL,
    CG_FIRST,
    CG_CLUSTER,
    CG_CLUSTER_SPLIT,
    CG_PARTS,
    CG_SLABS,
    CG_PLAIN
};
struct ConvGnChoice {
    ConvGnPath path = CG_PLAIN;
    int np = 0;
    int cl_splits = 1;
    int splits = 1;
    bool wino = false;
    bool local() const { return path == CG_LOCAL || path == CG_WLOCAL; }
};
static ConvGnChoice classify_conv_gn(const ddk_unet& u, const ConvW& cw, int B, int H, int W, int c0, int c1, int N, bool first_input,
                                     bool cluster, size_t splitk_floats) {
// ... 197 lines not shown
        conv1(r.res, x, 256, sk, 256, (x_external ? 0 : CHF_WAIT) | CHF_SAVE_KEEP2 | CHF_NO_OUT, nullptr);
        float* h = buf(e++);
        conv3(r.c1, r.n1, x, 256, sk, 256, r.temb_off, CHF_SIGNAL, h);
        conv3(r.c2, r.n2, h, 256, nullptr, 0, -1, WS | CHF_ADD_KEEP2 | CHF_SAVE_KEEP, o);
    };
    if (part == 0) {
        const int sh = u.L - 1;
        if (down_src) {
            const ConvW& dc = u.down_conv[sh - 1];
            float* dn = buf(e++);
            ChainOp& op = p.op[n++];
            op = ChainOp{down_src, nullptr, c.P + dc.wl, c.P + dc.b, nullptr, nullptr, dn, 256, 0, CH_CONV3,
                         CHF_DOWN | CHF_NO_GN | CHF_SIGNAL | CHF_SAVE_KEEP, -1, 256};
            in = dn;
        }
        float* d0 = buf(e++);
        res_plain(u.down_res[2 * sh], in, down_src == nullptr, d0);
        float* d1 = buf(e++);
        res_plain(u.down_res[2 * sh + 1], d0, false, d1);
        attn_block(u.down_attn[sh], d1, skip, true);
        float* m1 = buf(e++);
        res_plain(u.mid1, skip, false, m1);
        float* ma = buf(e++);
        attn_block(u.mid_attn, m1, ma, true);
        float* m2 = buf(e++);
        res_plain(u.mid2, ma, false, m2);
        float* u0 = buf(e++);
        res_cat(u.up_res[0], m2, false, skip, u0);
        float* u1 = buf(e++);
        res_plain(u.up_res[1], u0, false, u1);
        if (up_out) {
            float* ua = buf(e++);
            attn_block(u.up_attn[0], u1, ua, true);
            const ConvW& uc = u.up_conv[0];
            ChainOp& op = p.op[n++];
            op = ChainOp{ua, nullptr, c.P + uc.wtl, c.P + uc.b, nullptr, nullptr, up_out, 256, 0, CH_UPT, CHF_WAIT, -1, 256};
        } else {
            attn_block(u.up_attn[0], u1, out, false);
        }
    } else if (part == 1) {
        const int sh = u.L - 2;
        float* d0 = buf(e++);
        res_plain(u.down_res[2 * sh], in, true, d0);
        float* d1 = buf(e++);
        res_plain(u.down_res[2 * sh + 1], d0, false, d1);
        attn_block(u.down_attn[sh], d1, skip, false);
    } else {
        float* u0 = buf(e++);
        res_cat(u.up_res[2], in, true, skip, u0);
        float* u1 = buf(e++);
        res_plain(u.up_res[3], u0, false, u1);
        attn_block(u.up_attn[1], u1, out, false);
    }
    if (n > CH_MAX_OPS || e > (part == 0 ? CHAIN_BUFS : CHAIN8_BUFS)) return fail_arg("level_chain: internal op / buffer count");
    p.n_ops = n;
    p.B = c.B;
    p.hw = hw;
    p.temb = c.temb;
    p.temb_rows = c.temb_rows;
    p.temb_stride = u.temb_total;
    float* cl = c.W + c.ly.off_cl;
    p.cnt = reinterpret_cast<unsigned*>(cl + cl_chain_offset(c.B));
    p.done = p.cnt + (size_t)c.B * 32;
    p.fail = cl_words(cl, c.B).fail;
    p.gn_eps = GN_EPS;
    p.ln_eps = LN_EPS;
    return level_chain_launch(p, c.st);
}

struct StepArgs {
    int64_t* state;
    float* eps_hat;
    long long per;
    StepRule rule;
};

static int fused_tail_parts(const ddk_unet& u, int B, int H, int W, int cin, StepKind kind, int restore_n = 0) {
    const int chan = u.generic ? pad32(u.cfg.chan) : u.cfg.chan, n_out = u.cfg.in_ch;
    const int npf = u.final_conv.has_wu ? conv_wino_stats_parts(B, H, W, cin, chan, GROUPS) : 0;
    if (npf <= 0 || (restore_kind(kind) && !u.restore_fused)) return 0;
    return final_tail_ok(H * W, chan, GROUPS, n_out, npf, kind, W, restore_n) ? npf : 0;
}

__global__ __launch_bounds__(256) void step_prepare_kernel(const float* __restrict__ x, float* __restrict__ xpad, long long total,
                                                           int C, int c_pad, int64_t* __restrict__ counter,
                                                           int64_t* __restrict__ t_cur, int B) {
    if (blockIdx.x == 0) {
        const int64_t v = *counter;
        for (int b = threadIdx.x; b < B; b += blockDim.x) t_cur[b] = v;
        __syncthreads();
        if (threadIdx.x == 0) *counter = v - 1;
    }
    for (long long i = blockIdx.x * 256LL + threadIdx.x; i < total; i += (long long)gridDim.x * 256) {
        const int ch = (int)(i % c_pad);
        const long long m = i / c_pad;
        xpad[i] = ch < C ? x[m * C + ch] : 0.f;
    }
}

static bool first_fast(const ddk_unet& u, int B, int H, int W) {
    const ResW& r = u.down_res[0];
    if (!r.c1.has_wf || !r.has_res || !r.c2.has_wu) return false;
    if (!conv_first_ok(r.ci, r.co, H, W, GROUPS)) return false;
    const int upr = r.co / 4;
    if (upr > 256 || 256 % upr) return false;
    if ((long long)H * W / 128 * GROUPS > 1024) return false;
    return conv_wino_stats_parts(B, H, W, r.co, r.co, GROUPS) > 0;
}

static int run_first_res(Ctx& c, const float* x, bool fused, int64_t* counter, int64_t* t_cur, float* out, int H, int W) {
    const ResW& r = c.u.down_res[0];
    const float* P = c.P;
    float* raw = c.W + c.ly.off_raw;
    float* a1 = c.W + c.ly.off_a1;
    float* gnp = c.W + c.ly.off_gn;
    const float* bias1 = r.c1.has_bias ? P + r.c1.b : nullptr;
    const float* res_b = r.res.has_bias ? P + r.res.b : nullptr;
    if (fused) {
        const WinoGnFuse f = c.gn_fuse(r.n1, c.temb + r.temb_off, c.temb_rows);
        DDK_TRY(conv_first_gn(x, P + r.c1.wf, bias1, f.gamma, f.beta, f.temb, f.temb_stride, f.temb_rows, f.eps, a1, c.B, H, W, r.ci, r.co,
                              f.groups, f.records, f.counters, f.fail, counter, t_cur, c.st));
    } else {
        DDK_TRY(conv_first(x, P + r.c1.wf, bias1, raw, gnp, c.B, H, W, r.ci, r.co, GROUPS, counter, t_cur, c.st));
        DDK_TRY(groupnorm_mish_parts(raw, gnp, H * W / 128, P + r.n1.g, P + r.n1.b, c.temb + r.temb_off, c.u.temb_total, nullptr, a1, c.B,
                                     H * W, r.co, GROUPS, GN_EPS, c.st, c.temb_rows));
    }
    const int cl_np = c.allow_cluster && conv_wino_cluster_device_ok() && r.ci <= 8 ? conv_wino_cluster_np(c.B, H, W, r.co, r.co, GROUPS) : 0;
    if (cl_np > 0 && cl_np <= c.u.cluster_np_max && conv_wino_variant_new(c.B, H, W, r.co) && c.n_cluster < c.u.cluster_limit) {
        ++c.n_cluster;
        const ddk_conv_args a = c.conv_args(DDK_CONV3X3_S1, r.c2, a1, r.co, nullptr, 0, out, H, W, r.co);
        WinoGnFuse f = c.gn_fuse(r.n2, nullptr, nullptr);
        f.res_x = x; f.res_w = P + r.res.w; f.res_b = res_b; f.res_cin = r.ci; f.res_ld = r.res.cin_pad;
        return conv_forward(a, c.st, nullptr, &f);
    }
    DDK_TRY(run_conv_parts(c, r.c2, a1, r.co, nullptr, 0, raw, H, W, r.co));
    return groupnorm_mish_parts(raw, gnp, conv_wino_stats_parts(c.B, H, W, r.co, r.co, GROUPS), P + r.n2.g, P + r.n2.b, nullptr, c.u.temb_total,
                                nullptr, out, c.B, H * W, r.co, GROUPS, GN_EPS, c.st, nullptr, x, P + r.res.w, res_b, r.ci, r.res.cin_pad);
}

static int forward_core(const ddk_unet& u, const float* P, const float* x, int64_t* t, float* out, int B, int H0, int W0,
                        float* ws, const Layout& ly, hipStream_t st, bool allow_cluster, const float* temb_table = nullptr,
                        const StepArgs* step = nullptr) {
    float* tact = ws + ly.off_tact;
    float* temb = ws + ly.off_temb;
    float* xpad = ws + ly.off_xpad;
    const bool fast0 = first_fast(u, B, H0, W0);
    if (!fast0) {
        const int C = u.cfg.in_ch, cp = pad32(C);
        const long long padded = (long long)B * H0 * W0 * cp;
        if (step) {
            const int prep_blocks = (int)(ceil_div(padded, 256) < 1024 ? ceil_div(padded, 256) : 1024);
            hipLaunchKernelGGL(step_prepare_kernel, dim3(prep_blocks), dim3(256), 0, st, x, xpad, padded, C, cp, step->state, t, B);
            DDK_TRY(check_launch("step_prepare_kernel"));
        } else {
            DDK_TRY(ddk_pad_channels(x, xpad, (long long)B * H0 * W0, C, cp, st));
        }
    }
    if (!temb_table) {
        DDK_TRY(time_mlp(t, P + u.freqs, P + u.w1t, P + u.b1, P + u.w2t, P + u.b2, tact, nullptr, B, u.time_dim, st));
        DDK_TRY(time_proj(tact, P + u.temb_wt, P + u.temb_bias, temb, B, u.time_dim, u.temb_total, st));
    }
    static_assert(sizeof(long long) == sizeof(int64_t), "timestep rows are read as long long");
    Ctx c{u, P, ws, ly, B, st, temb_table ? temb_table : temb, temb_table ? reinterpret_cast<const long long*>(t) : nullptr};
    if (!fast0) { c.x_first = x; c.x_padded = xpad; }
    c.allow_cluster = allow_cluster;
    float* bufA = ws + ly.off_A;
    float* bufB = ws + ly.off_B;
    float* bufC = ws + ly.off_C;
    float* raw = ws + ly.off_raw;
    float* a1 = ws + ly.off_a1;
    float* gnp = ws + ly.off_gn;

    int H = H0, W = W0;
    const float* cur = xpad;
    int cur_c = pad32(u.cfg.in_ch);
    AddendSlabs cur_ss;
    const bool first_fused = fast0 && c.allow_cluster && u.first_gn && conv_wino_cluster_device_ok() &&
                             conv_first_gn_ok(u.down_res[0].ci, u.down_res[0].co, H0, W0, GROUPS) && u.cluster_limit > 0;
    int64_t* dec_counter = (first_fused && step) ? step->state : nullptr;
    const bool chained = level_chain_use(c, H0, W0, 1);
    const bool chain_edges = chained && (u.level_chain & 8) && u.L >= 2 && u.down_conv[u.L - 2].has_wl && u.down_conv[u.L - 2].has_bias &&
                             u.up_conv[0].has_wtl && u.up_conv[0].cin == 256 && u.down_conv[u.L - 2].cin == 256;
    const bool chained8 = level_chain_use(c, H0, W0, 2);
    const bool chained8u = level_chain_use(c, H0, W0, 4);
    for (int l = 0; l < u.L; ++l) {
        float* skip = ws + ly.off_skip[l];
        const int co = u.dimp[l + 1];
        if (chained && l == u.L - 1) {
            DDK_TRY(run_level_chain(c, 0, cur, skip, bufB, chain_edges ? ws + ly.off_skip[l - 1] : nullptr, chain_edges ? bufA : nullptr));
            cur_c = co;
            break;
        }
        const bool level_chained = chained8 && l == u.L - 2 && cur_ss.n == 1;
        if (level_chained) {
            DDK_TRY(run_level_chain(c, 1, cur, skip, nullptr));
        } else if (l == 0 && fast0) {
            DDK_TRY(run_first_res(c, x, first_fused, step ? step->state : nullptr, step ? t : nullptr, bufB, H, W));
        } else {
            DDK_TRY(run_res(c, u.down_res[2 * l], cur, cur_c, nullptr, 0, bufB, H, W, cur_ss));
            cur_ss = AddendSlabs();
        }
        if (!level_chained) {
            DDK_TRY(run_res(c, u.down_res[2 * l + 1], bufB, co, nullptr, 0, bufC, H, W));
            DDK_TRY(run_attn(c, u.down_attn[l], bufC, skip, H, W));
        }
        if (l < u.L - 1 && chain_edges && l + 1 == u.L - 1) {
            H /= 2; W /= 2;
            cur = skip;
        } else if (l < u.L - 1) {
            const int s2 = conv_splits(DDK_CONV3X3_S2, B, H, W, co, co);
            if (u.fold_down_reduce && s2 > 1 && !(chained && l + 1 == u.L - 1) && !(chained8 && l + 1 == u.L - 2) &&
                res_takes_slab_source(u, u.down_res[2 * l + 2], B, H / 2, W / 2, co)) {
                DDK_TRY(run_conv_slabs(c, DDK_CONV3X3_S2, u.down_conv[l], skip, co, nullptr, 0, bufA, H, W, co, s2, cur_ss));
                H /= 2; W /= 2;
                cur = ws + ly.off_splitk;
            } else {
                DDK_TRY(run_conv(c, DDK_CONV3X3_S2, u.down_conv[l], skip, co, nullptr, 0, nullptr, bufA, H, W, co));
                H /= 2; W /= 2;
                cur = bufA;
            }
        } else {
            cur = skip;
        }
        cur_c = co;
    }
    if (!chained) {
        DDK_TRY(run_res(c, u.mid1, cur, cur_c, nullptr, 0, bufB, H, W));
        DDK_TRY(run_attn(c, u.mid_attn, bufB, bufC, H, W));
        DDK_TRY(run_res(c, u.mid2, bufC, cur_c, nullptr, 0, bufA, H, W));
        cur = bufA;
    }
    for (int i = 0; i < u.L - 1; ++i) {
        const int lvl = u.L - 1 - i;
        const float* skip = ws + ly.off_skip[lvl];
        const int dout = u.dimp[lvl + 1], din = u.dimp[lvl];
        if (chained8u && i == 1) {
            DDK_TRY(run_level_chain(c, 2, cur, const_cast<float*>(skip), bufB));
        } else if (!(chained && i == 0)) {
            DDK_TRY(run_res(c, u.up_res[2 * i], cur, cur_c, skip, dout, bufB, H, W));
            DDK_TRY(run_res(c, u.up_res[2 * i + 1], bufB, din, nullptr, 0, bufC, H, W));
            DDK_TRY(run_attn(c, u.up_attn[i], bufC, bufB, H, W));
        }
        if (!(chain_edges && i == 0))
            DDK_TRY(run_conv(c, DDK_CONVT4X4_S2, u.up_conv[i], bufB, din, nullptr, 0, nullptr, bufA, H, W, din));
        H *= 2; W *= 2;
        cur = bufA;
        cur_c = din;
    }
    const int chan = u.generic ? pad32(u.cfg.chan) : u.cfg.chan, n_out = u.cfg.in_ch;
    StepRule plain{};
    plain.kind = StepKind::Eps;
    plain.eps_out = out;
    const StepRule& rule = step ? step->rule : plain;
    ChainHooks hooks{};
    if (step) {
        hooks.chain_state = step->state;
        hooks.dec_counter = dec_counter;
    }
    const int npf = fused_tail_parts(u, B, H, W, cur_c, rule.kind, rule.rst.n);
    const int npe = (npf == 0 && step && restore_kind(rule.kind)) ? fused_tail_parts(u, B, H, W, cur_c, StepKind::Eps) : 0;
    if ((npf > 0 || npe > 0) && (!step || step->per == (long long)H * W * n_out)) {
        DDK_TRY(run_conv_parts(c, u.final_conv, cur, cur_c, nullptr, 0, raw, H, W, chan));
        const TailIn in{raw, gnp, npf > 0 ? npf : npe, P + u.final_norm.g, P + u.final_norm.b, GN_EPS, P + u.final_w, P + u.final_b, n_out, B, H * W, chan, GROUPS};
        if (npf > 0) return final_tail(in, rule, t, hooks, st);
        StepRule eps_only{};
        eps_only.kind = StepKind::Eps;
        eps_only.eps_out = step->eps_hat;
        DDK_TRY(final_tail(in, eps_only, t, ChainHooks{}, st));
        return p_update(rule, step->eps_hat, t, B, step->per, hooks, st);
    }
    DDK_TRY(run_conv_gn(c, u.final_conv, cur, cur_c, nullptr, 0, raw, u.final_norm, nullptr, nullptr, a1, H, W, chan));
    float* eps_hat = step ? step->eps_hat : out;
    DDK_TRY(conv1x1_small_n(a1, P + u.final_w, P + u.final_b, eps_hat, (long long)B * H * W, chan, n_out, st));
    return step ? p_update(rule, eps_hat, t, B, step->per, hooks, st) : DDK_OK;
}

static int check_shape(const ddk_unet* u, int B, int H, int W) {
    DDK_REQUIRE(u, "unet: null plan");
    DDK_REQUIRE(B > 0 && H > 0 && W > 0, "unet: B/H/W must be positive");
    const int f = 1 << (u->L - 1);
    if (H % f || W % f) {
        set_error("unet: spatial size %dx%d must be divisible by %d (%d stride-2 stages, unet.py:43-50)", H, W, f, u->L - 1);
        return DDK_ERR_ARG;
    }
    return DDK_OK;
}

__global__ void set_chain_state_kernel(int64_t* state, int64_t t_start, uint64_t seed, uint32_t stream_id) {
    state[0] = t_start;
    state[1] = (int64_t)seed;
    state[2] = (int64_t)stream_id;
}

}

extern "C" size_t ddk_unet_workspace_bytes(const ddk_unet* u, int B, int H, int W) {
    if (check_shape(u, B, H, W) != DDK_OK) return 0;
    return make_layout(*u, B, H, W).total * sizeof(float);
}

extern "C" int ddk_unet_forward(const ddk_unet* u, const void* packed, const float* x, const int64_t* t, float* out, int B, int H,
                                int W, void* workspace, size_t workspace_bytes, ddk_stream_t s) {
    DDK_TRY(check_shape(u, B, H, W));
    DDK_REQUIRE(packed && x && t && out && workspace, "unet_forward: null pointer");
    DDK_REQUIRE(aligned16(packed) && aligned16(workspace) && aligned16(x) && aligned16(out), "unet_forward: alignment");
    const Layout ly = make_layout(*u, B, H, W);
    if (workspace_bytes < ly.total * sizeof(float)) {
        set_error("unet_forward: workspace too small (%zu < %zu)", workspace_bytes, ly.total * sizeof(float));
        return DDK_ERR_WORKSPACE;
    }
    float* ws = static_cast<float*>(workspace);
    DDK_TRY(ensure_device_init());
    DDK_HIP(hipMemsetAsync(ws + ly.off_cl, 0, cl_counter_floats(B) * sizeof(float), as_stream(s)));
    return forward_core(*u, static_cast<const float*>(packed), x, const_cast<int64_t*>(t), out, B, H, W, ws, ly, as_stream(s),
                        u->cluster_gn >= 2);
}

extern "C" int ddk_unet_cluster_check(const ddk_unet* u, void* workspace, int B, int H, int W, ddk_stream_t s) {
    DDK_TRY(check_shape(u, B, H, W));
    DDK_REQUIRE(workspace, "unet_cluster_check: null workspace");
    const Layout ly = make_layout(*u, B, H, W);
    return cluster_fail_check(cl_words(static_cast<float*>(workspace) + ly.off_cl, B).fail, as_stream(s), "in-launch GroupNorm",
                              " (the GPU is shared, masked or partitioned); results on this workspace are invalid -- rerun with "
                              "DDK_OPT_CLUSTER_GROUPNORM = 0");
}

extern "C" double ddk_unet_flops(const ddk_unet* u, int B, int H0, int W0) {
    if (check_shape(u, B, H0, W0) != DDK_OK) return 0;
    double f = 0;
    auto res = [&](const ResW& r, int H, int W) {
        f += conv_flops(DDK_CONV3X3_S1, B, H, W, r.ci_real, r.co_real) + conv_flops(DDK_CONV3X3_S1, B, H, W, r.co_real, r.co_real);
        if (r.has_res) f += conv_flops(DDK_CONV1X1, B, H, W, r.ci_real, r.co_real);
        f += 2.0 * B * u->time_dim * r.co_real;
    };
    auto attn = [&](const AttnW& a, int H, int W) {
        f += conv_flops(DDK_CONV1X1, B, H, W, a.c_real, 3 * HIDDEN) + conv_flops(DDK_CONV1X1, B, H, W, HIDDEN, a.c_real);
        f += 2.0 * 2.0 * B * HEADS * 32.0 * 32.0 * H * W;
    };
    int H = H0, W = W0;
    f += 2.0 * B * (u->time_dim * 4.0 * u->time_dim) * 2;
    for (int l = 0; l < u->L; ++l) {
        res(u->down_res[2 * l], H, W); res(u->down_res[2 * l + 1], H, W); attn(u->down_attn[l], H, W);
        if (l < u->L - 1) { f += conv_flops(DDK_CONV3X3_S2, B, H, W, u->dims[l + 1], u->dims[l + 1]); H /= 2; W /= 2; }
    }
    res(u->mid1, H, W); attn(u->mid_attn, H, W); res(u->mid2, H, W);
    for (int i = 0; i < u->L - 1; ++i) {
        res(u->up_res[2 * i], H, W); res(u->up_res[2 * i + 1], H, W); attn(u->up_attn[i], H, W);
        f += conv_flops(DDK_CONVT4X4_S2, B, H, W, u->up_conv[i].cin, u->up_conv[i].cout);
        H *= 2; W *= 2;
    }
    f += conv_flops(DDK_CONV3X3_S1, B, H, W, u->cfg.chan, u->cfg.chan) + conv_flops(DDK_CONV1X1, B, H, W, u->cfg.chan, u->cfg.in_ch);
    return f;
}

extern "C" double ddk_unet_flops_executed(const ddk_unet* u, int B, int H0, int W0) {
    if (check_shape(u, B, H0, W0) != DDK_OK) return 0;
    double f = 0;
    auto conv3 = [&](const ConvW& cw, int H, int W, int c0, int c1, int N) {
        const ConvGnChoice k = classify_conv_gn(*u, cw, B, H, W, c0, c1, N, false, false, 0);
        const int cin = c0 + c1;
        if (k.path == CG_WLOCAL) return 2.0 * B * (H * W / 4) * 16.0 * cin * N;
        if (k.wino) return 2.0 * (double)(ceil_div((long long)B * (H / 2) * (W / 2), 32) * 32) * 16.0 * cin * N;
        return 2.0 * B * H * W * 9.0 * cin * N;
    };
    auto res = [&](const ResW& r, int H, int W, int c0, int c1, bool fast) {
        if (fast) {
            f += 2.0 * B * H * W * (2.0 * ((9 * r.ci + 1) / 2)) * r.co;
            f += 2.0 * B * H * W * (double)r.ci * r.co;
        } else {
            f += conv3(r.c1, H, W, c0, c1, r.co);
            if (r.has_res) f += conv_flops(DDK_CONV1X1, B, H, W, c0 + c1, r.co);
        }
        f += conv3(r.c2, H, W, r.co, 0, r.co);
    };
    auto attn = [&](const AttnW& a, int H, int W) {
        if (attn_fold_eligible(*u, a, B, H, W)) {
            f += conv_flops(DDK_CONV1X1, B, H, W, a.c, 2 * HIDDEN) + 2.0 * B * HEADS * 32.0 * 32.0 * H * W;
            f += 2.0 * B * (4.0 * HIDDEN * 32.0 * a.c + (double)a.c * HIDDEN * a.c) + conv_flops(DDK_CONV1X1, B, H, W, a.c, a.c);
            return;
        }
        f += conv_flops(DDK_CONV1X1, B, H, W, a.c, 3 * HIDDEN) + conv_flops(DDK_CONV1X1, B, H, W, HIDDEN, a.c);
        f += 2.0 * 2.0 * B * HEADS * 32.0 * 32.0 * H * W;
    };
    int H = H0, W = W0, cur_c = pad32(u->cfg.in_ch);
    for (int l = 0; l < u->L; ++l) {
        const int co = u->dims[l + 1];
        res(u->down_res[2 * l], H, W, cur_c, 0, l == 0 && first_fast(*u, B, H, W));
        res(u->down_res[2 * l + 1], H, W, co, 0, false);
        attn(u->down_attn[l], H, W);
        if (l < u->L - 1) { f += conv_flops(DDK_CONV3X3_S2, B, H, W, co, co); H /= 2; W /= 2; }
        cur_c = co;
    }
    res(u->mid1, H, W, cur_c, 0, false); attn(u->mid_attn, H, W); res(u->mid2, H, W, cur_c, 0, false);
    for (int i = 0; i < u->L - 1; ++i) {
        const int lvl = u->L - 1 - i, dout = u->dims[lvl + 1], din = u->dims[lvl];
        res(u->up_res[2 * i], H, W, cur_c, dout, false);
        res(u->up_res[2 * i + 1], H, W, din, 0, false);
        attn(u->up_attn[i], H, W);
        if (u->up_conv[i].has_wu && convT_wino_use(B, H, W, din, din))
            f += 2.0 * (double)(ceil_div((long long)B * (H / 2) * (W / 2), 32) * 32) * 36.0 * din * din;
        else
            f += conv_flops(DDK_CONVT4X4_S2, B, H, W, din, din);
        H *= 2; W *= 2;
        cur_c = din;
    }
    f += conv3(u->final_conv, H, W, cur_c, 0, u->cfg.chan) + 2.0 * B * H * W * (double)u->cfg.chan * u->cfg.in_ch;
    return f;
}

namespace ddk {
struct SamplerLayout {
    size_t unet_floats, off_eps, off_t, off_table, off_tact_all, off_tall, total;
};
static SamplerLayout sampler_layout(const ddk_unet& u, int B, int H, int W, int t_start) {
    SamplerLayout s;
    const size_t rows = (size_t)t_start + 1;
    s.unet_floats = make_layout(u, B, H, W).total;
    s.off_eps = s.unet_floats;
    s.off_t = s.off_eps + al4((size_t)B * H * W * u.cfg.in_ch);
    s.off_table = s.off_t + al4(2 * (size_t)(B + 3));
    s.off_tact_all = s.off_table + al4(rows * u.temb_total);
    s.off_tall = s.off_tact_all + al4(rows * u.time_dim);
    s.total = s.off_tall + al4(2 * rows);
    return s;
}

__global__ void iota64_kernel(int64_t* out, int n) {
    const int i = blockIdx.x * blockDim.x + threadIdx.x;
    if (i < n) out[i] = i;
}
}


namespace ddk {
static int ensure_temb_table(ddk_unet& u, const float* P, float* ws, const SamplerLayout& sl, int t_start, int B, int H, int W,
                             hipStream_t st, const int64_t* map) {
    const int rows = t_start + 1;
    const bool same_map = map ? (u.table.map.size() == (size_t)rows && std::equal(map, map + rows, u.table.map.begin()))
                              : u.table.map.empty();
    if (u.table.ws == ws && u.table.t_start == t_start && u.table.B == B && u.table.H == H && u.table.W == W &&
        u.table.pack_epoch == u.pack_epoch && same_map)
        return DDK_OK;
    u.table.ws = nullptr;
    int64_t* t_all = reinterpret_cast<int64_t*>(ws + sl.off_tall);
    float* tact_all = ws + sl.off_tact_all;
    if (map) {
        u.table.map.assign(map, map + rows);
        DDK_HIP(hipMemcpyAsync(t_all, u.table.map.data(), (size_t)rows * sizeof(int64_t), hipMemcpyHostToDevice, st));
        DDK_HIP(hipStreamSynchronize(st));
    } else {
        u.table.map.clear();
        hipLaunchKernelGGL(iota64_kernel, dim3((unsigned)ceil_div(rows, 256)), dim3(256), 0, st, t_all, rows);
        DDK_TRY(check_launch("iota64_kernel"));
    }
    DDK_TRY(time_mlp(t_all, P + u.freqs, P + u.w1t, P + u.b1, P + u.w2t, P + u.b2, tact_all, nullptr, rows, u.time_dim, st));
    DDK_TRY(time_proj(tact_all, P + u.temb_wt, P + u.temb_bias, ws + sl.off_table, rows, u.time_dim, u.temb_total, st));
    u.table.ws = ws; u.table.t_start = t_start; u.table.B = B; u.table.H = H; u.table.W = W;
    u.table.pack_epoch = u.pack_epoch;
    return DDK_OK;
}

template <class F>
static int run_chain(ddk_unet& u, const ChainKey& key, int n_steps, bool use_graph, F&& one_step, hipStream_t st, const char* who) {
    if (!use_graph || n_steps == 1) {
        for (int k = 0; k < n_steps; ++k) DDK_TRY(one_step());
        return DDK_OK;
    }
    auto capture = [&](int steps, hipGraph_t& graph, hipGraphExec_t& exec) -> int {
        hipError_t e = hipStreamBeginCapture(st, hipStreamCaptureModeThreadLocal);
        if (e != hipSuccess) {
            set_error("%s: hipStreamBeginCapture failed (%s); the legacy NULL stream cannot be captured -- pass a created stream", who,
                      hipGetErrorString(e));
            return DDK_ERR_HIP;
        }
        int rc = DDK_OK;
        for (int i = 0; i < steps && rc == DDK_OK; ++i) rc = one_step();
        e = hipStreamEndCapture(st, &graph);
        if (rc != DDK_OK) { if (graph) (void)hipGraphDestroy(graph); graph = nullptr; return rc; }
        if (e != hipSuccess) { graph = nullptr; set_error("%s: hipStreamEndCapture: %s", who, hipGetErrorString(e)); return DDK_ERR_HIP; }
        e = hipGraphInstantiate(&exec, graph, nullptr, nullptr, 0);
        if (e != hipSuccess) {
            (void)hipGraphDestroy(graph);
            graph = nullptr; exec = nullptr;
            set_error("%s: hipGraphInstantiate: %s", who, hipGetErrorString(e));
            return DDK_ERR_HIP;
        }
        return DDK_OK;
    };

    SamplerGraph* hit = nullptr;
// ... 464 lines not shown
```

### downsampled-diffusion_amd/ddk/lib.py

```python
import ctypes as C
import os

import torch

_HERE = os.path.dirname(os.path.abspath(__file__))
LIB_PATH = os.environ.get("DDK_LIB", os.path.join(os.path.dirname(_HERE), "csrc", "libddk.so"))


class DDKError(RuntimeError):
    pass


ABI_VERSION = 400
ERR_CLUSTER = -4


class ConvArgs(C.Structure):
    _fields_ = [
        ("kind", C.c_int), ("src0", C.c_void_p), ("src1", C.c_void_p), ("c0", C.c_int), ("c1", C.c_int),
        ("weight", C.c_void_p), ("bias", C.c_void_p), ("resid", C.c_void_p), ("out", C.c_void_p),
        ("B", C.c_int), ("H", C.c_int), ("W", C.c_int), ("N", C.c_int), ("pre_mish", C.c_int), ("post_mish", C.c_int), ("defer_reduce", C.c_int),
        ("workspace", C.c_void_p), ("workspace_bytes", C.c_size_t), ("weight_wino", C.c_void_p),
        ("gn_partials", C.c_void_p), ("gn_groups", C.c_int), ("mish_out", C.c_void_p), ("dmish_src", C.c_void_p),
    ]
# ... 74 lines not shown
    "ddk_conv_first": (_I, [_P, _P, _P, _P, _P, _I, _I, _I, _I, _I, _I, _P]),
    "ddk_conv1x1_ws_ok": (_I, [C.c_longlong, _I, _I]),
    "ddk_conv1x1_ws": (_I, [_P, _P, _P, _P, _P, C.c_longlong, _I, _P, _P, _F, _P]),
    "ddk_conv1x1_ws_images": (_I, [_P, _P, _P, _P, _P, C.c_longlong, _I, _P, _P, _F, _I, _P]),
    "ddk_linattn_context_kv": (_I, [_P, _P, _I, _I, _I, _P, _SZ, _P]),
    "ddk_attention_fold": (_I, [_P, _P, _P, _P, _P, _P, _P, _P, _P, _I, _I, _I, _P]),
    "ddk_groupnorm_mish_partials_res1x1": (_I, [_P, _P, _I, _P, _P, _P, _I, _P, _P, _P, _I, _P, _I, _I, _I, _I, _F, _P]),
    "ddk_final_tail": (_I, [_P, _P, _I, _P, _P, _F, _P, _P, _I, _P, _P, _P, _P, _P, _P, _P, _P, _P, C.c_uint64, C.c_uint32, _I, _I, _I, _I, _P]),
    "ddk_pack_conv_weight_local": (_I, [_P, _P, _I, _I, _I, _P]),
    "ddk_pack_conv1x1_weight_local": (_I, [_P, _P, _I, _I, _I, _P]),
    "ddk_pack_convT_weight_local": (_I, [_P, _P, _I, _I, _P]),
    "ddk_pack_conv_weight_wino_local": (_I, [_P, _P, _I, _I, _I, _P]),
    "ddk_conv3x3_gn_mish_wino_ok": (_I, [_I, _I, _I, _I, _I, _I]),
    "ddk_conv3x3_gn_mish_wino": (_I, [_P, _I, _P, _I, _P, _P, _P, _P, _P, _I, _P, _P, _I, _I, _I, _I, _I, _F, _P]),
    "ddk_conv3x3_gn_mish_slabs": (_I, [_P, _I, _LL, _P, _I, _P, _P, _P, _P, _P, _I, _P, _I, _LL, _P, _P, _I, _I, _I, _I, _I, _F, _P]),
    "ddk_attention_kv_context_workspace_bytes": (_SZ, [_I, _I]),
    "ddk_attention_kv_context_ok": (_I, [_I, _I, _I, _I]),
    "ddk_attention_kv_context": (_I, [_P, _P, _P, _P, _F, _P, _I, _I, _P, _SZ, _P]),
    "ddk_attention_split_workspace_bytes": (_SZ, [_I]),
    "ddk_attention_split_ok": (_I, [_I, _I, _I, _I]),
    "ddk_attention_split_from_x": (_I, [_P, _P, _P, _P, _F, _P, _P, _I, _I, _I, _I, _P, _SZ, _P]),
    "ddk_pack_qkv_operand": (_I, [_P, _P, _I, _I, _P]),
    "ddk_linattn_small_from_x": (_I, [_P, _P, _P, _P, _F, _P, _P, _I, _I, _I, _I, _P]),
    "ddk_conv3x3_gn_mish_ok": (_I, [_I, _I, _I, _I, _I, _I]),
    "ddk_conv3x3_gn_mish": (_I, [_P, _I, _P, _I, _P, _P, _P, _P, _P, _I, _P, _P, _I, _I, _I, _I, _I, _F, _P]),
    "ddk_conv_workspace_bytes": (_SZ, [_I, _I, _I, _I, _I, _I]),
    "ddk_conv_splits": (_I, [_I, _I, _I, _I, _I, _I]),
    "ddk_conv_forward": (_I, [C.POINTER(ConvArgs), _P]),
    "ddk_debug_read_stamps": (_I, [_P]),
    "ddk_groupnorm_mish": (_I, [_P, _P, _P, _P, _I, _P, _P, _I, _I, _I, _I, _F, _P, _SZ, _P]),
    "ddk_groupnorm_workspace_bytes": (_SZ, [_I, _I, _I, _I]),
    "ddk_groupnorm_mish_slabs": (_I, [_P, _I, _LL, _P, _P, _P, _P, _I, _P, _P, _I, _I, _I, _I, _F, _P]),
    "ddk_chan_layernorm": (_I, [_P, _P, _P, _P, _LL, _I, _F, _P]),
    "ddk_mish": (_I, [_P, _P, _LL, _P]),
    "ddk_tanh": (_I, [_P, _P, _LL, _P]),
    "ddk_avgpool2": (_I, [_P, _P, _I, _I, _I, _I, _P]),
    "ddk_upsample_nearest2": (_I, [_P, _P, _I, _I, _I, _I, _P]),
    "ddk_add": (_I, [_P, _P, _P, _LL, _P]),
    "ddk_linattn_context_workspace_bytes": (_SZ, [_I, _I, _I]),
    "ddk_linattn_context": (_I, [_P, _P, _I, _I, _I, _P, _SZ, _P]),
    "ddk_linattn_apply": (_I, [_P, _P, _P, _I, _I, _I, _P]),
    "ddk_linattn_fused_small": (_I, [_P, _P, _P, _I, _I, _I, _P]),
    "ddk_time_mlp": (_I, [_P, _P, _P, _P, _P, _P, _P, _P, _I, _I, _P]),
    "ddk_time_proj": (_I, [_P, _P, _P, _P, _I, _I, _I, _P]),
    "ddk_conv1x1_small_n": (_I, [_P, _P, _P, _P, _LL, _I, _I, _P]),
    "ddk_q_sample": (_I, [_P, _P, _P, _P, _P, _P, _I, _LL, _P]),
    "ddk_p_sample_update": (_I, [_P, _P, _P, _P, _P, _P, _P, _P, _P, _I, _LL, C.c_uint64, C.c_uint32, _P]),
    "ddk_p_sample_update_multistep": (_I, [_P, _P, _P, _P, _P, _P, _P, _P, _P, _I, _LL, _P]),
    "ddk_p_sample_update_inpaint": (_I, [_P] * 14 + [_I, _LL, C.c_uint64, C.c_uint32, _P]),
    "ddk_p_sample_update_restore": (_I, [_P, _P, _P, _I] + [_P] * 6 + [_I, _I, _I, _I, C.c_uint64, C.c_uint32, _P]),
    "ddk_p_sample_update_restore_masked": (_I, [_P, _P, _P, _P, _I] + [_P] * 6 + [_I, _I, _I, _I, C.c_uint64, C.c_uint32, _P]),
    "ddk_p_sample_update_restore_multistep": (_I, [_P, _P, _P, _P, _P, _I] + [_P] * 6 + [_I, _I, _I, _I, _P]),
    "ddk_p_sample_update_restore_noisy": (_I, [_P, _P, _P, _P, _I] + [_P] * 8 + [_I, _I, _I, _I, C.c_uint64, C.c_uint32, _P]),
    "ddk_p_sample_update_restore_gray": (_I, [_P, _P, _P, _P, _I, _I] + [_P] * 8 + [_I, _I, _I, _I, C.c_uint64, C.c_uint32, _P]),
    "ddk_separable_apply": (_I, [_P, _P, _P, _P, _I, _I, _I, _I, _P]),
    "ddk_separable_apply_rect": (_I, [_P, _P, _P, _P, _P, _I, _I, _I, _I, _I, _I, _P]),
    "ddk_p_sample_update_restore_blur": (_I, [_P] * 12 + [_I, _I, _I, _I, C.c_uint64, C.c_uint32, _P]),
    "ddk_randn": (_I, [_P, _LL, C.c_uint64, C.c_uint32, C.c_uint32, _P]),
    "ddk_fix_samples": (_I, [_P, _P, _I, _I, _I, _I, _P]),
    "ddk_sq_err_sum": (_I, [_P, _P, _P, _I, _LL, _P]),
    "ddk_vlb_terms_workspace_bytes": (_SZ, [_I, _LL]),
    "ddk_vlb_terms": (_I, [_P, _P, _P, _P, _P, _P, _P, _P, _P, _P, _P, _P, _I, _LL, _P, _SZ, _P]),
    "ddk_image_metrics_workspace_bytes": (_SZ, [_I, _I, _I, _I]),
    "ddk_image_metrics": (_I, [_P, _P, _P, _I, _I, _I, _I, _P, _P, _P, _SZ, _P]),
    "ddk_knn_radii_workspace_bytes": (_SZ, [_I]),
    "ddk_knn_radii": (_I, [_P, _I, _I, _I, _P, _P, _SZ, _P]),
    "ddk_manifold_members_workspace_bytes": (_SZ, [_I, _I]),
    "ddk_manifold_members": (_I, [_P, _P, _I, _P, _P, _I, _I, _P, _P, _P, _SZ, _P]),
    "ddk_unet_create": (_P, [C.POINTER(UnetConfig)]),
    "ddk_unet_destroy": (None, [_P]),
    "ddk_unet_num_slots": (_I, [_P]),
    "ddk_unet_slot_name": (C.c_char_p, [_P, _I]),
    "ddk_unet_slot_numel": (_LL, [_P, _I]),
    "ddk_unet_packed_bytes": (_SZ, [_P]),
    "ddk_unet_pack_slot": (_I, [_P, _I, _P, _P, _P]),
    "ddk_unet_finalize_pack": (_I, [_P, _P, _P]),
    "ddk_unet_workspace_bytes": (_SZ, [_P, _I, _I, _I]),
    "ddk_unet_forward": (_I, [_P, _P, _P, _P, _P, _I, _I, _I, _P, _SZ, _P]),
    "ddk_conv3x3_gn_mish_cluster_ok": (_I, [_I, _I, _I, _I, _I, _I]),
    "ddk_conv3x3_gn_mish_cluster_workspace_bytes": (_SZ, [_I, _I, _I, _I]),
    "ddk_conv3x3_gn_mish_cluster_split_workspace_bytes": (_SZ, [_I, _I, _I, _I, _I, _I]),
    "ddk_conv3x3_gn_mish_cluster": (_I, [_P, _I, _P, _I, _P, _P, _P, _P, _P, _I, _P, _P, _I, _I, _I, _I, _I, _F, _P, _SZ, _P]),
    "ddk_unet_set_option": (_I, [_P, _I, _I]),
    "ddk_debug_cluster_timeouts": (C.c_uint, []),
    "ddk_conv3x3_gn_mish_cluster_check": (_I, [_P, _I, _P]),
    "ddk_unet_cluster_check": (_I, [_P, _P, _I, _I, _I, _P]),
    "ddk_debug_occupy": (_I, [_I, _I, _I, _P]),
    "ddk_debug_clock_probe": (_I, [_P, _I, _P]),
    "ddk_unet_flops": (C.c_double, [_P, _I, _I, _I]),
    "ddk_unet_flops_executed": (C.c_double, [_P, _I, _I, _I]),
    "ddk_sampler_workspace_bytes": (_SZ, [_P, _I, _I, _I, _I]),
    "ddk_sampler_run": (_I, [C.POINTER(SamplerArgs), _P]),
    "ddk_sampler_run_spaced": (_I, [C.POINTER(SamplerArgs), C.POINTER(C.c_int64), _P]),
    "ddk_sampler_multistep_workspace_bytes": (_SZ, [_P, _I, _I, _I, _I]),
    "ddk_sampler_run_multistep": (_I, [C.POINTER(SamplerArgs), C.POINTER(C.c_int64), _P, _P]),
    "ddk_sampler_inpaint_workspace_bytes": (_SZ, [_P, _I, _I, _I, _I]),
    "ddk_sampler_run_inpaint": (_I, [C.POINTER(SamplerArgs), C.POINTER(InpaintArgs), _P]),
    "ddk_sampler_restore_workspace_bytes": (_SZ, [_P, _I, _I, _I, _I]),
    "ddk_sampler_restore_tail_parts": (_I, [_P, _I, _I, _I, _I]),
    "ddk_sampler_run_restore": (_I, [C.POINTER(SamplerArgs), C.POINTER(C.c_int64), _P, _I, _P]),
    "ddk_sampler_restore_masked_workspace_bytes": (_SZ, [_P, _I, _I, _I, _I, _I]),
    "ddk_sampler_restore_masked_tail_parts": (_I, [_P, _I, _I, _I, _I]),
    "ddk_sampler_run_restore_masked": (_I, [C.POINTER(SamplerArgs), C.POINTER(C.c_int64), _P, _P, _I, _P]),
    "ddk_sampler_restore_multistep_workspace_bytes": (_SZ, [_P, _I, _I, _I, _I, _I]),
    "ddk_sampler_restore_multistep_tail_parts": (_I, [_P, _I, _I, _I, _I]),
    "ddk_sampler_run_restore_multistep": (_I, [C.POINTER(SamplerArgs), C.POINTER(C.c_int64), _P, _P, _P, _I, _P]),
    "ddk_sampler_restore_noisy_workspace_bytes": (_SZ, [_P, _I, _I, _I, _I, _I]),
    "ddk_sampler_restore_noisy_tail_parts": (_I, [_P, _I, _I, _I, _I]),
    "ddk_sampler_run_restore_noisy": (_I, [C.POINTER(SamplerArgs), C.POINTER(C.c_int64), _P, _P, _P, _P, _I, _P]),
    "ddk_sampler_restore_gray_workspace_bytes": (_SZ, [_P, _I, _I, _I, _I, _I]),
    "ddk_sampler_restore_gray_tail_parts": (_I, [_P, _I, _I, _I, _I]),
    "ddk_sampler_run_restore_gray": (_I, [C.POINTER(SamplerArgs), C.POINTER(C.c_int64), _P, _P, _P, _P, _I, _I, _P]),
    "ddk_sampler_restore_blur_workspace_bytes": (_SZ, [_P, _I, _I, _I, _I]),
    "ddk_sampler_restore_blur_tail_parts": (_I, [_P, _I, _I, _I]),
    "ddk_sampler_run_restore_blur": (_I, [C.POINTER(SamplerArgs), C.POINTER(C.c_int64), _P, _P, _P, _P, _P, _P]),
    "ddk_sampler_run_restore_sep": (_I, [C.POINTER(SamplerArgs), C.POINTER(C.c_int64), _P, _P, _P, _P, _P, _I, _I, _P]),
    "ddk_sampler_invalidate": (_I, [_P]),
    "ddk_sampler_release_workspace": (_I, [_P, _P]),
    "ddk_vlb_sweep_workspace_bytes": (_SZ, [_P, _I, _I, _I, _I]),
    "ddk_vlb_sweep_run": (_I, [C.POINTER(VlbSweepArgs), _P]),
    "ddk_pack_conv_weight_dgrad": (_I, [_P, _P, _I, _I, _I, _I, _I, _I, _P]),
    "ddk_zero_stuff2": (_I, [_P, _P, _I, _I, _I, _I, _I, _I, _P]),
    "ddk_conv_wgrad_workspace_bytes": (_SZ, [_I, _I, _I, _I, _I, _I]),
    "ddk_conv_wgrad": (_I, [_I, _P, _P, _P, _I, _I, _I, _I, _I, _I, _I, _I, _P, _SZ, _P]),
    "ddk_conv_wgrad_bias": (_I, [_I, _P, _P, _P, _P, _I, _I, _I, _I, _I, _I, _I, _I, _P, _SZ, _P]),
    "ddk_bias_grad": (_I, [_P, _P, _LL, _I, _I, _P, _SZ, _P]),
    "ddk_groupnorm_train_workspace_bytes": (_SZ, [_I, _I, _I, _I]),
    "ddk_dropout_epoch": (_I, [C.c_uint64, _I, _P]),
    "ddk_groupnorm_mish_train_fwd": (_I, [_P, _P, _P, _P, _I, _P, _F, C.c_uint64, C.c_uint32, _P, _I, _I, _I, _I, _F, _P, _SZ, _P]),
    "ddk_groupnorm_mish_bwd": (_I, [_P, _P, _P, _F, C.c_uint64, C.c_uint32, _P, _P, _P, _I, _I, _I, _I, _F, _P, _SZ, _P]),
    "ddk_groupnorm_mish_train_fwd_slabs": (_I, [_P, _I, _LL, _P, _P, _P, _P, _P, _I, _P, _F, C.c_uint64, C.c_uint32, _P, _I, _I, _I, _I,
                                                _F, _P]),
    "ddk_groupnorm_mish_bwd_slabs": (_I, [_P, _P, _P, _F, C.c_uint64, C.c_uint32, _P, _I, _LL, _P, _P, _I, _I, _I, _I, _F, _P]),
    "ddk_rows_sum": (_I, [_P, _I, _LL, _P, _I, _I, _P]),
    "ddk_rows_sum_batched": (_I, [_P, _I, _LL, _I, _LL, _P, _I, _I, _P]),
    "ddk_rows_sum_targets": (_I, [_P, _I, _LL, _I, _LL, _P, _P, _P, _P, _I, _I, _P]),
    "ddk_multi_add": (_I, [_P, _P, _I, _LL, _P]),
    "ddk_conv_wgrad_defer": (_I, [_I, _P, _P, _P, _P, _I, _I, _I, _I, _I, _I, _I, _I, _P, _SZ, _P, _P]),
    "ddk_wgrad_reduce_jobs": (_I, [_P, _I, _P]),
    "ddk_rows_sum_jobs": (_I, [_P, _I, _P]),
    "ddk_pack_jobs_layout": (_LL, [_P, _I]),
    "ddk_pack_jobs": (_I, [_P, _I, _LL, _P]),
    "ddk_chan_layernorm_bwd": (_I, [_P, _P, _P, _P, _P, _I, C.POINTER(C.c_int), _LL, _I, _F, _P]),
    "ddk_chan_layernorm_bwd_add": (_I, [_P, _P, _P, _P, _P, _P, _I, C.POINTER(C.c_int), _LL, _I, _F, _P]),
    "ddk_groupnorm_mish_generic_train_fwd": (_I, [_P, _P, _P, _P, _I, _P, _F, C.c_uint64, C.c_uint32, _P, _I, _I, _I, _I, _I, _F, _P]),
    "ddk_groupnorm_mish_generic_bwd": (_I, [_P, _P, _P, _F, C.c_uint64, C.c_uint32, _P, _P, _P, _I, _I, _I, _I, _I, _F, _P]),
    "ddk_chan_layernorm_generic": (_I, [_P, _P, _P, _P, _LL, _I, _I, _F, _P]),
    "ddk_chan_layernorm_generic_bwd": (_I, [_P, _P, _P, _P, _P, _P, _I, C.POINTER(C.c_int), _LL, _I, _I, _F, _P]),
    "ddk_linattn_train_workspace_bytes": (_SZ, [_I, _I, _I]),
    "ddk_linattn_stats": (_I, [_P, _P, _I, _I, _I, _P, _SZ, _P]),
    "ddk_linattn_bwd": (_I, [_P, _P, _P, _P, _P, _P, _I, _I, _I, _P, _SZ, _P]),
    "ddk_linattn_bwd_recompute": (_I, [_P, _P, _P, _P, _P, _P, _I, _I, _I, _P, _SZ, _P]),
    "ddk_mish_bwd": (_I, [_P, _P, _P, _LL, _P]),
    "ddk_tanh_bwd": (_I, [_P, _P, _P, _LL, _P]),
    "ddk_avgpool2_bwd": (_I, [_P, _P, _I, _I, _I, _I, _P]),
    "ddk_upsample_nearest2_bwd": (_I, [_P, _P, _I, _I, _I, _I, _P]),
    "ddk_sq_err_grad": (_I, [_P, _P, _P, _P, _I, _LL, _P]),
    "ddk_ae_objective": (_I, [_P, _P, _P, _I, _I, _P, _P]),
    "ddk_ae_objective_bwd": (_I, [_P, _P, _I, _I, _P, _P, _P]),
    "ddk_scale_per_sample": (_I, [_P, _P, _P, _I, _LL, _P]),
    "ddk_conv1x1_small_n_bwd": (_I, [_P, _P, _P, _P, _P, _I, C.POINTER(C.c_int), _LL, _I, _I, _P]),
    "ddk_small_gemm_workspace_bytes": (_SZ, [_I, _I, _I, _I]),
    "ddk_small_gemm": (_I, [_I, _P, _P, _P, _I, _I, _I, _I, _I, _I, _I, _P, _SZ, _P]),
    "ddk_sincos_embed": (_I, [_P, _P, _P, _I, _I, _P]),
    "ddk_bias_act": (_I, [_P, _P, _P, _LL, _I, _P]),
    "ddk_grad_norm_clip": (_I, [_P, _LL, _F, _P, _P, _SZ, _P]),
# ... 59 lines not shown
```

### downsampled-diffusion_amd/ddk/plan.py

```python
import contextlib
import ctypes as C
import math
import warnings

import torch

from . import lib as L


def sinusoidal_freqs(dim):
    half = dim // 2
    step = math.log(10000) / (half - 1)
    return torch.exp(torch.arange(half) * -step)


SAMPLERS = {"smp": ("sample", "sampler", "sampler"), "sms": ("sample_multistep", "sampler_multistep", "multistep sampler"),
            "sin": ("sample_inpaint", "sampler_inpaint", "inpainting sampler"),
            "srs": ("sample_restore", "sampler_restore", "super-resolution sampler"),
            "srm": ("sample_restore_masked", "sampler_restore_masked", "masked restoration sampler"),
            "srx": ("sample_restore_multistep", "sampler_restore_multistep", "restoration solver"),
            "srn": ("sample_restore_noisy", "sampler_restore_noisy", "noisy restoration sampler"),
            "srg": ("sample_restore_gray", "sampler_restore_gray", "colourisation sampler"),
            "srb": ("sample_restore_blur", "sampler_restore_blur", "deblurring sampler"),
            "srq": ("sample_restore_sep", "sampler_restore_sep", "separable restoration sampler")}
CHAIN_WORKSPACES = (*SAMPLERS, "vsw")


class UnetPlan:
    def __init__(self, in_ch, chan, mults):
        lib = L.load()
        cfg = L.UnetConfig(in_ch, chan, len(mults), (C.c_int * 8)(*list(mults) + [0] * (8 - len(mults))))
        self._lib = lib
        self.handle = lib.ddk_unet_create(C.byref(cfg))
        if not self.handle:
            raise L.DDKError(f"ddk_unet_create failed: {L.last_error()}")
        self.in_ch, self.chan, self.mults = in_ch, chan, tuple(mults)
        self.slot_names = [lib.ddk_unet_slot_name(self.handle, i).decode() for i in range(lib.ddk_unet_num_slots(self.handle))]
        self.slot_numel = [lib.ddk_unet_slot_numel(self.handle, i) for i in range(len(self.slot_names))]
        self.packed = None
        self._ws = {}
        self._state = {}
        self._cluster = 1
        self._cluster_dev = None

    def __deepcopy__(self, memo):
        return None

    def __del__(self):
        try:
            if getattr(self, "handle", None):
                self._lib.ddk_unet_destroy(self.handle)
                self.handle = None
        except Exception:
            pass

    def pack(self, tensors, device):
        lib = self._lib
        nbytes = lib.ddk_unet_packed_bytes(self.handle)
        packed = torch.zeros(nbytes // 4, device=device, dtype=torch.float32)
        keep = []
        for i, name in enumerate(self.slot_names):
            if name == "@sinusoidal_freqs":
                src = sinusoidal_freqs(self.chan)
            else:
                if name not in tensors:
                    raise L.DDKError(f"UNet weight '{name}' missing from the state dict")
                src = tensors[name]
            src = src.detach().to(device=device, dtype=torch.float32).contiguous()
            if src.numel() != self.slot_numel[i]:
                raise L.DDKError(f"UNet weight '{name}': expected {self.slot_numel[i]} elements, got {src.numel()}")
            keep.append(src)
            L.check(lib.ddk_unet_pack_slot(self.handle, i, L.ptr(src), L.ptr(packed), L.stream()), f"pack {name}")
        torch.cuda.current_stream().synchronize()
        self.packed = packed
        return packed

    def _workspace(self, kind, nbytes, device):
        key = (kind, nbytes, str(device))
        hit = self._ws.get(key)
        if hit is not None:
            self._ws[key] = self._ws.pop(key)
            return hit
        if kind in CHAIN_WORKSPACES:
            mine = [k for k in self._ws if k[0] == kind]
            if len(mine) >= 3:
                old = self._ws[mine[0]]
                L.check(self._lib.ddk_sampler_release_workspace(self.handle, L.ptr(old)), "sampler_release_workspace")
                del self._ws[mine[0]]
        else:
            for k in [k for k in self._ws if k[0] == kind]:
                del self._ws[k]
        buf = torch.empty(max(nbytes, 16) // 4 + 4, device=device, dtype=torch.float32)
        self._ws[key] = buf
        return buf

    OPT_CLUSTER_GROUPNORM = 1
    OPT_ATTENTION_FOLD = 3
    OPT_FOLD_DOWNSAMPLE_REDUCE = 5
    OPT_ATTENTION_KV_CONTEXT = 6
    OPT_LEVEL_CHAIN = 7
    OPT_FIRST_GROUPNORM = 8
    OPT_RESTORE_FUSED_TAIL = 12
    OPT_ATTENTION_SPLIT = 13

    def set_option(self, option, value):
        L.check(self._lib.ddk_unet_set_option(self.handle, option, int(value)), "unet_set_option")
        if option == self.OPT_CLUSTER_GROUPNORM:
            self._cluster = max(0, min(2, int(value)))

    @contextlib.contextmanager
    def forwards_as_in_chain(self):
        raised = self._cluster == 1
        if raised:
            self.set_option(self.OPT_CLUSTER_GROUPNORM, 2)
        try:
            yield
        finally:
            if raised and self._cluster == 2:
                self.set_option(self.OPT_CLUSTER_GROUPNORM, 1)

    def _cluster_failed(self, ws, b, h, w, stream_ptr):
        rc = self._lib.ddk_unet_cluster_check(self.handle, L.ptr(ws), b, h, w, stream_ptr)
        if rc == 0:
            return False
        if rc != L.ERR_CLUSTER:
            L.check(rc, "unet_cluster_check")
        warnings.warn("ddk: " + L.last_error() + " -- switching DDK_OPT_CLUSTER_GROUPNORM off for this plan and rerunning",
                      RuntimeWarning, stacklevel=3)
        self.set_option(self.OPT_CLUSTER_GROUPNORM, 0)
        return True

    def _chain_guarded(self):
        if self._cluster_dev is None:
            self._cluster_dev = self._lib.ddk_conv3x3_gn_mish_cluster_ok(32, 32, 32, 128, 128, 8) > 0
        return self._cluster >= 1 and self._cluster_dev

    def _run_chain(self, who, call, ws, b, h, w, graphed, restore=None):
        guard = self._chain_guarded()
        for rerun in (False, True):
            if rerun and restore is not None:
                restore()
            if graphed:
                cur = torch.cuda.current_stream()
                side = _side_stream(ws.device)
                side.wait_stream(cur)
                with torch.cuda.stream(side):
                    call(side.cuda_stream)
                    failed = guard and self._cluster >= 1 and self._cluster_failed(ws, b, h, w, side.cuda_stream)
                cur.wait_stream(side)
            else:
                call(L.stream())
                failed = guard and self._cluster >= 1 and self._cluster_failed(ws, b, h, w, L.stream())
            if not failed:
                return
        raise L.DDKError(f"{who}: in-launch GroupNorm reported a failure with the option off")

    def cluster_timeouts(self):
        return int(self._lib.ddk_debug_cluster_timeouts())

    def flops(self, b, h, w):
        return self._lib.ddk_unet_flops(self.handle, b, h, w)

    def flops_executed(self, b, h, w):
        return self._lib.ddk_unet_flops_executed(self.handle, b, h, w)

    def forward_nhwc(self, x, t):
        if self.packed is None:
            raise L.DDKError("UnetPlan.forward before pack()")
        b, h, w, c = x.shape
        if c != self.in_ch:
            raise L.DDKError(f"expected {self.in_ch} input channels, got {c}")
        if t.dtype != torch.int64:
            raise L.DDKError("timesteps must be int64")
        lib = self._lib
        nbytes = lib.ddk_unet_workspace_bytes(self.handle, b, h, w)
        if nbytes == 0:
            raise L.DDKError(f"unet workspace query failed: {L.last_error()}")
        ws = self._workspace("fwd", nbytes, x.device)
        out = torch.empty_like(x)
        for _ in range(2):
            L.check(lib.ddk_unet_forward(self.handle, L.ptr(self.packed), L.ptr(x), L.ptr(t), L.ptr(out), b, h, w,
                                         L.ptr(ws), nbytes, L.stream()), "unet_forward")
            if self._cluster < 2 or not self._cluster_failed(ws, b, h, w, L.stream()):
                break
        return out

    def _need_packed(self, kind):
        if self.packed is None:
            raise L.DDKError(f"UnetPlan.{SAMPLERS[kind][0]} before pack()")

    def _run_sampler(self, kind, x, t_start, t_end, bytes_query, call, use_graph):
        _, who, label = SAMPLERS[kind]
        b, h, w, _ = x.shape
        nbytes = bytes_query(b, h, w)
        if nbytes == 0:
            raise L.DDKError(f"{label} workspace query failed: {L.last_error()}")
        ws = self._workspace(kind, nbytes, x.device)
        caller_x, x = x, self._chain_x(x)
        x_start = x.clone() if self._chain_guarded() else None
        self._run_chain(who, lambda stream_ptr: call(x, ws, nbytes, stream_ptr), ws, b, h, w, use_graph and t_start - t_end + 1 > 1,
                        restore=lambda: x.copy_(x_start))
        if caller_x.data_ptr() != x.data_ptr():
            caller_x.copy_(x)
        return caller_x

    @staticmethod
    def _timestep_map(timesteps, t_start):
        if timesteps is None:
            return None
        if len(timesteps) != t_start + 1:
            raise L.DDKError(f"timestep map must have t_start + 1 = {t_start + 1} entries, got {len(timesteps)}")
        return (C.c_int64 * len(timesteps))(*[int(v) for v in timesteps])

    def _sampler_args(self, x, noise, tables, t_start, t_end, seed, stream_id, use_graph, ws, nbytes):
        b, h, w, _ = x.shape
        return L.SamplerArgs(self.handle, L.ptr(self.packed), L.ptr(x), L.ptr(noise), L.ptr(tables["c_recip"]),
                             L.ptr(tables["c_recipm1"]), L.ptr(tables["c1"]), L.ptr(tables["c2"]), L.ptr(tables.get("sigma")),
                             b, h, w, t_start, t_end, seed, stream_id, int(use_graph), L.ptr(ws), nbytes)

    def sample_nhwc(self, x, tables, t_start, t_end=0, noise=None, seed=0, stream_id=0, use_graph=True, timesteps=None):
        self._need_packed("smp")
        lib = self._lib
        tmap = self._timestep_map(timesteps, t_start)
        n_steps = t_start - t_end + 1
        if noise is not None and tuple(noise.shape) != (n_steps, *x.shape):
            raise L.DDKError(f"injected noise must be {(n_steps, *x.shape)}, got {tuple(noise.shape)}")

        def call(x, ws, nbytes, stream_ptr):
            a = self._sampler_args(x, noise, tables, t_start, t_end, seed, stream_id, use_graph, ws, nbytes)
            if tmap is None:
                L.check(lib.ddk_sampler_run(C.byref(a), stream_ptr), "sampler_run")
            else:
                L.check(lib.ddk_sampler_run_spaced(C.byref(a), tmap, stream_ptr), "sampler_run_spaced")

        return self._run_sampler("smp", x, t_start, t_end,
                                 lambda b, h, w: lib.ddk_sampler_workspace_bytes(self.handle, b, h, w, t_start), call, use_graph)

    def _chain_x(self, x):
        skey = (tuple(x.shape), str(x.device))
        mode = self._state.get(skey)
        if mode is None:
            mode = self._state[skey] = {"ptr": x.data_ptr(), "buf": None}
        if mode["buf"] is None and mode["ptr"] != x.data_ptr():
            mode["buf"] = torch.empty_like(x)
        if mode["buf"] is not None:
            mode["buf"].copy_(x)
            return mode["buf"]
# ... 186 lines not shown
```

### include/ddk.h

```cpp
#ifndef DDK_H
#define DDK_H

#include <stddef.h>
#include <stdint.h>

#ifdef __cplusplus
extern "C" {
#endif

typedef void* ddk_stream_t;

#define DDK_OK 0
#define DDK_ERR_ARG (-1)
#define DDK_ERR_HIP (-2)
#define DDK_ERR_WORKSPACE (-3)
#define DDK_ERR_CLUSTER (-4)

int ddk_version(void);
const char* ddk_last_error(void);
int ddk_device_ok(void);

int ddk_nchw_to_nhwc(const float* src, float* dst, int B, int C, int H, int W, int c_pad, ddk_stream_t s);
int ddk_nhwc_to_nchw(const float* src, float* dst, int B, int C, int H, int W, int c_stride, ddk_stream_t s);
int ddk_pad_channels(const float* src, float* dst, long long M, int C, int c_pad, ddk_stream_t s);
// ... 10 lines not shown
    DDK_CONV1X1 = 2,
    DDK_CONVT4X4_S2 = 3,
    DDK_CONV4X4_S2 = 4
};

typedef struct ddk_conv_args {
    int kind;
    const float* src0;
    const float* src1;
    int c0, c1;
    const float* weight;
    const float* bias;
    const float* resid;
    float* out;
    int B, H, W;
    int N;
    int pre_mish;
    int post_mish;
    int defer_reduce;
    void* workspace;
    size_t workspace_bytes;
    const float* weight_wino;
    float* gn_partials;
    int gn_groups;
    float* mish_out;
    const float* dmish_src;
} ddk_conv_args;

int ddk_pack_conv_weight_wino(const float* w_oihw, float* dst, int O, int I, int i_pad, ddk_stream_t s);
int ddk_conv_gn_partials(int B, int H, int W, int cin, int N, int groups);
int ddk_conv_wino_splits(int B, int H, int W, int cin, int N);
size_t ddk_conv_workspace_bytes(int kind, int B, int H, int W, int cin, int N);
int ddk_conv_splits(int kind, int B, int H, int W, int cin, int N);
int ddk_conv_forward(const ddk_conv_args* a, ddk_stream_t s);
int ddk_debug_read_stamps(unsigned long long* host_out);

int ddk_groupnorm_mish(const float* x, const float* gamma, const float* beta, const float* temb,
                       int temb_stride, const float* addend, float* out, int B, int HW, int C, int groups,
                       float eps, void* workspace, size_t workspace_bytes, ddk_stream_t s);
size_t ddk_groupnorm_workspace_bytes(int B, int HW, int C, int groups);
int ddk_groupnorm_mish_slabs(const float* slabs, int nslab, long long slab_stride, const float* conv_bias,
                             const float* gamma, const float* beta, const float* temb, int temb_stride,
                             const float* addend, float* out, int B, int HW, int C, int groups, float eps,
                             ddk_stream_t s);
int ddk_pack_conv_weight_local(const float* w_oihw, float* dst, int O, int I, int i_pad, ddk_stream_t s);
int ddk_pack_conv1x1_weight_local(const float* w_oi, float* dst, int O, int I, int i_pad, ddk_stream_t s);
int ddk_pack_convT_weight_local(const float* w_iohw, float* dst, int I, int O, ddk_stream_t s);
int ddk_conv3x3_gn_mish_ok(int H, int W, int cin, int c0, int N, int groups);
int ddk_conv3x3_gn_mish(const float* src0, int c0, const float* src1, int c1, const float* weight, const float* bias,
                        const float* gamma, const float* beta, const float* temb, int temb_stride, const float* addend,
                        float* out, int B, int H, int W, int N, int groups, float eps, ddk_stream_t s);
int ddk_groupnorm_mish_partials(const float* x, const float* partials, int tiles_per_image, const float* gamma, const float* beta,
                                const float* temb, int temb_stride, const float* addend, float* out, int B, int HW, int C,
                                int groups, float eps, ddk_stream_t s);
int ddk_pack_conv_weight_first(const float* w_oihw, float* dst, int O, int I, ddk_stream_t s);
int ddk_conv_first_ok(int cin, int N, int H, int W, int groups);
int ddk_conv_first(const float* x, const float* w_first, const float* bias, float* out, float* gn_partials, int B, int H, int W,
                   int cin, int N, int groups, ddk_stream_t s);
int ddk_conv1x1_ws_ok(long long M, int K, int N);
int ddk_conv1x1_ws(const float* x, const float* w, const float* bias, const float* resid, float* out, long long M, int N,
                   const float* ln_c1, const float* ln_c2, float ln_eps, ddk_stream_t s);
int ddk_conv1x1_ws_images(const float* x, const float* w, const float* bias, const float* resid, float* out, long long M, int N,
                          const float* ln_c1, const float* ln_c2, float ln_eps, int images, ddk_stream_t s);
int ddk_groupnorm_mish_partials_res1x1(const float* x, const float* partials, int tiles_per_image, const float* gamma, const float* beta,
                                       const float* temb, int temb_stride, const float* res_x, const float* res_w, const float* res_b,
                                       int res_cin, float* out, int B, int HW, int C, int groups, float eps, ddk_stream_t s);
int ddk_pack_conv_weight_wino_local(const float* w_oihw, float* dst, int O, int I, int i_pad, ddk_stream_t s);
int ddk_conv3x3_gn_mish_wino_ok(int H, int W, int cin, int c0, int N, int groups);
int ddk_conv3x3_gn_mish_wino(const float* src0, int c0, const float* src1, int c1, const float* weight, const float* bias,
                             const float* gamma, const float* beta, const float* temb, int temb_stride, const float* addend,
                             float* out, int B, int H, int W, int N, int groups, float eps, ddk_stream_t s);
int ddk_conv3x3_gn_mish_slabs(const float* src, int src_slabs, long long src_stride, const float* src_bias, int c0, const float* weight,
                              const float* bias, const float* gamma, const float* beta, const float* temb, int temb_stride,
                              const float* addend, int addend_slabs, long long addend_stride, const float* addend_bias, float* out, int B,
                              int H, int W, int N, int groups, float eps, ddk_stream_t s);
int ddk_conv3x3_gn_mish_cluster_ok(int B, int H, int W, int cin, int N, int groups);
int ddk_conv3x3_gn_mish_cluster_check(void* workspace, int B, ddk_stream_t s);
size_t ddk_conv3x3_gn_mish_cluster_workspace_bytes(int B, int H, int W, int N);
size_t ddk_conv3x3_gn_mish_cluster_split_workspace_bytes(int B, int H, int W, int cin, int N, int groups);
int ddk_conv3x3_gn_mish_cluster(const float* src0, int c0, const float* src1, int c1, const float* weight_wino, const float* bias,
                                const float* gamma, const float* beta, const float* temb, int temb_stride, const float* addend,
                                float* out, int B, int H, int W, int N, int groups, float eps, void* workspace, size_t workspace_bytes,
                                ddk_stream_t s);
int ddk_chan_layernorm(const float* x, const float* g, const float* b, float* out, long long M, int C,
                       float eps, ddk_stream_t s);
int ddk_mish(const float* x, float* out, long long n, ddk_stream_t s);
int ddk_tanh(const float* x, float* out, long long n, ddk_stream_t s);
int ddk_avgpool2(const float* x, float* out, int B, int H, int W, int C, ddk_stream_t s);
int ddk_upsample_nearest2(const float* x, float* out, int B, int H, int W, int C, ddk_stream_t s);
int ddk_add(const float* a, const float* b, float* out, long long n, ddk_stream_t s);

size_t ddk_linattn_context_workspace_bytes(int B, int HW, int heads);
int ddk_linattn_context(const float* qkv, float* ctx, int B, int HW, int heads, void* workspace, size_t workspace_bytes, ddk_stream_t s);
int ddk_linattn_context_kv(const float* kv, float* ctx, int B, int HW, int heads, void* workspace, size_t workspace_bytes, ddk_stream_t s);
int ddk_attention_fold(const float* ctx, const float* wqg, const float* c1q, const float* c2q, const float* wout, const float* bout, float* A,
                       float* a1, float* a2, int B, int C, int heads, ddk_stream_t s);
size_t ddk_attention_kv_context_workspace_bytes(int B, int HW);
int ddk_attention_kv_context_ok(int B, int HW, int C, int heads);
int ddk_attention_kv_context(const float* x, const float* w_kv, const float* c1, const float* c2, float ln_eps, float* ctx, int B, int HW,
                             void* workspace, size_t workspace_bytes, ddk_stream_t s);
size_t ddk_attention_split_workspace_bytes(int B);
int ddk_attention_split_ok(int B, int HW, int C, int heads);
int ddk_attention_split_from_x(const float* x, const float* w_folded, const float* c1, const float* c2, float ln_eps, float* ctx, float* out,
                               int B, int HW, int C, int heads, void* workspace, size_t workspace_bytes, ddk_stream_t s);
int ddk_linattn_fused_small(const float* qkv, float* ctx, float* out, int B, int HW, int heads, ddk_stream_t s);
int ddk_linattn_apply(const float* qkv, const float* ctx, float* out, int B, int HW, int heads, ddk_stream_t s);
int ddk_pack_qkv_operand(const float* folded_w, float* dst, int heads, int c_pad, ddk_stream_t s);
int ddk_linattn_small_from_x(const float* x, const float* w_operand, const float* c1, const float* c2, float ln_eps, float* ctx,
                             float* out, int B, int HW, int C, int heads, ddk_stream_t s);

int ddk_time_mlp(const int64_t* t, const float* freqs, const float* w1t, const float* b1, const float* w2t,
                 const float* b2, float* act, float* raw, int B, int dim, ddk_stream_t s);
int ddk_time_proj(const float* act, const float* wt, const float* bias, float* out, int B, int dim, int n_out,
                  ddk_stream_t s);

int ddk_conv1x1_small_n(const float* x, const float* w, const float* bias, float* out, long long M, int C,
                        int n_out, ddk_stream_t s);

int ddk_q_sample(const float* x, const float* eps, const int64_t* t, const float* sqrt_acp,
                 const float* sqrt_1m_acp, float* out, int B, long long per, ddk_stream_t s);
int ddk_p_sample_update(float* x, const float* eps_hat, const float* noise, const int64_t* t,
                        const float* c_recip, const float* c_recipm1, const float* c1, const float* c2,
                        const float* sigma, int B, long long per, uint64_t seed, uint32_t stream_id,
                        ddk_stream_t s);
int ddk_p_sample_update_multistep(float* x, const float* eps_hat, float* x0_hist, const int64_t* t, const float* c_recip,
                                  const float* c_recipm1, const float* c1, const float* c2, const float* c3, int B, long long per,
                                  ddk_stream_t s);
int ddk_p_sample_update_inpaint(float* x, const float* eps_hat, const float* known, const float* mask, const int64_t* t,
                                const float* c_recip, const float* c_recipm1, const float* c1, const float* c2, const float* sigma,
                                const float* ka, const float* kb, const float* ja, const float* jb, int B, long long per, uint64_t seed,
                                uint32_t stream_id, ddk_stream_t s);
int ddk_p_sample_update_restore(float* x, const float* eps_hat, const float* y, int n, const int64_t* t, const float* c_recip,
                                const float* c_recipm1, const float* c1, const float* c2, const float* sigma, int B, int H, int W,
                                int channels, uint64_t seed, uint32_t stream_id, ddk_stream_t s);
int ddk_p_sample_update_restore_masked(float* x, const float* eps_hat, const float* y, const float* mask, int n, const int64_t* t,
                                       const float* c_recip, const float* c_recipm1, const float* c1, const float* c2, const float* sigma,
                                       int B, int H, int W, int channels, uint64_t seed, uint32_t stream_id, ddk_stream_t s);
int ddk_p_sample_update_restore_multistep(float* x, const float* eps_hat, float* x0_hist, const float* y, const float* mask, int n,
                                          const int64_t* t, const float* c_recip, const float* c_recipm1, const float* c1, const float* c2,
                                          const float* c3, int B, int H, int W, int channels, ddk_stream_t s);
int ddk_p_sample_update_restore_noisy(float* x, const float* eps_hat, const float* y, const float* mask, int n, const int64_t* t,
                                      const float* c_recip, const float* c_recipm1, const float* c1, const float* c2, const float* sigma,
                                      const float* lam, const float* sgm, int B, int H, int W, int channels, uint64_t seed, uint32_t stream_id,
                                      ddk_stream_t s);
int ddk_p_sample_update_restore_gray(float* x, const float* eps_hat, const float* y, const float* mask, int n, int weights, const int64_t* t,
                                     const float* c_recip, const float* c_recipm1, const float* c1, const float* c2, const float* sigma,
                                     const float* lam, const float* sgm, int B, int H, int W, int channels, uint64_t seed, uint32_t stream_id,
                                     ddk_stream_t s);
int ddk_separable_apply(const float* in, const float* L, const float* R, float* out, int B, int H, int W, int channels, ddk_stream_t s);
int ddk_separable_apply_rect(const float* in, const float* L, const float* R, float* out, float* scratch, int B, int Hi, int Wi, int Ho, int Wo,
                             int channels, ddk_stream_t s);
int ddk_p_sample_update_restore_blur(float* x, const float* eps_hat, const float* P_h, const float* P_w, const float* Yp, float* scratch,
                                     const int64_t* t, const float* c_recip, const float* c_recipm1, const float* c1, const float* c2,
                                     const float* sigma, int B, int H, int W, int channels, uint64_t seed, uint32_t stream_id, ddk_stream_t s);
int ddk_final_tail(const float* raw, const float* partials, int tiles_per_image, const float* gamma, const float* beta, float eps,
                   const float* w, const float* bias, int n_out, float* eps_out, float* x, const float* noise, const int64_t* t,
                   const float* c_recip, const float* c_recipm1, const float* c1, const float* c2, const float* sigma, uint64_t seed,
                   uint32_t stream_id, int B, int HW, int C, int groups, ddk_stream_t s);
int ddk_randn(float* out, long long n, uint64_t seed, uint32_t step, uint32_t stream_id, ddk_stream_t s);
int ddk_fix_samples(const float* x_nchw, float* out_nhwc, int B, int C, int H, int W, ddk_stream_t s);
size_t ddk_vlb_terms_workspace_bytes(int B, long long per);
int ddk_vlb_terms(const float* x, const float* x_t, const float* eps_hat, const float* eps, const int64_t* t,
                  const float* c_recip, const float* c_recipm1, const float* c1, const float* c2,
                  const float* post_logvar, float* vlb, float* sqerr, int B, long long per, void* workspace,
                  size_t workspace_bytes, ddk_stream_t s);
int ddk_sq_err_sum(const float* a, const float* b, float* per_sample, int B, long long per, ddk_stream_t s);
size_t ddk_image_metrics_workspace_bytes(int N, int H, int W, int C);
int ddk_image_metrics(const uint8_t* a, const uint8_t* b, const uint8_t* mask, int N, int H, int W, int C,
                      unsigned long long* sq_sum_count, float* ssim, void* workspace, size_t workspace_bytes, ddk_stream_t s);
size_t ddk_knn_radii_workspace_bytes(int N);
int ddk_knn_radii(const float* x, int N, int D, int k, float* radii, void* workspace, size_t workspace_bytes, ddk_stream_t s);
size_t ddk_manifold_members_workspace_bytes(int Na, int Nb);
int ddk_manifold_members(const float* a, const float* ra, int Na, const float* b, const float* rb, int Nb, int D, uint8_t* a_in,
                         uint8_t* b_in, void* workspace, size_t workspace_bytes, ddk_stream_t s);

typedef struct ddk_unet_config {
    int in_ch;
    int chan;
    int n_levels;
    int mults[8];
} ddk_unet_config;

typedef struct ddk_unet ddk_unet;

ddk_unet* ddk_unet_create(const ddk_unet_config* cfg);
void ddk_unet_destroy(ddk_unet* u);
int ddk_unet_num_slots(const ddk_unet* u);
const char* ddk_unet_slot_name(const ddk_unet* u, int slot);
long long ddk_unet_slot_numel(const ddk_unet* u, int slot);
size_t ddk_unet_packed_bytes(const ddk_unet* u);
int ddk_unet_pack_slot(const ddk_unet* u, int slot, const float* canonical, void* packed, ddk_stream_t s);
int ddk_unet_finalize_pack(const ddk_unet* u, void* packed, ddk_stream_t s);
size_t ddk_unet_workspace_bytes(const ddk_unet* u, int B, int H, int W);
int ddk_unet_forward(const ddk_unet* u, const void* packed, const float* x, const int64_t* t, float* out,
                     int B, int H, int W, void* workspace, size_t workspace_bytes, ddk_stream_t s);
#define DDK_OPT_CLUSTER_GROUPNORM 1
#define DDK_OPT_ATTENTION_FOLD 3
#define DDK_OPT_FOLD_DOWNSAMPLE_REDUCE 5
#define DDK_OPT_ATTENTION_KV_CONTEXT 6
#define DDK_OPT_LEVEL_CHAIN 7
#define DDK_OPT_FIRST_GROUPNORM 8
#define DDK_OPT_RESTORE_FUSED_TAIL 12
#define DDK_OPT_ATTENTION_SPLIT 13
int ddk_unet_set_option(ddk_unet* u, int option, int value);
int ddk_unet_cluster_check(const ddk_unet* u, void* workspace, int B, int H, int W, ddk_stream_t s);
unsigned ddk_debug_cluster_timeouts(void);
int ddk_debug_clock_probe(unsigned long long* out, int workgroups, ddk_stream_t s);
int ddk_debug_occupy(int workgroups, int lds_bytes, int microseconds, ddk_stream_t s);
double ddk_unet_flops(const ddk_unet* u, int B, int H, int W);
double ddk_unet_flops_executed(const ddk_unet* u, int B, int H, int W);

typedef struct ddk_sampler_args {
    const ddk_unet* unet;
    const void* packed;
    float* x;
    const float* noise;
    const float* c_recip;
    const float* c_recipm1;
    const float* c1;
    const float* c2;
    const float* sigma;
    int B, H, W;
    int t_start;
    int t_end;
    uint64_t seed;
    uint32_t stream_id;
    int use_graph;
    void* workspace;
    size_t workspace_bytes;
} ddk_sampler_args;

size_t ddk_sampler_workspace_bytes(const ddk_unet* u, int B, int H, int W, int t_start);
int ddk_sampler_run(const ddk_sampler_args* a, ddk_stream_t s);
int ddk_sampler_run_spaced(const ddk_sampler_args* a, const int64_t* timestep_map, ddk_stream_t s);
size_t ddk_sampler_multistep_workspace_bytes(const ddk_unet* u, int B, int H, int W, int t_start);
int ddk_sampler_run_multistep(const ddk_sampler_args* a, const int64_t* timestep_map, const float* c3, ddk_stream_t s);
typedef struct ddk_inpaint_args {
    const int64_t* timestep_map;
    const float* known;
    const float* mask;
    const float* ka;
    const float* kb;
    const float* ja;
    const float* jb;
} ddk_inpaint_args;
size_t ddk_sampler_inpaint_workspace_bytes(const ddk_unet* u, int B, int H, int W, int n_ops);
int ddk_sampler_run_inpaint(const ddk_sampler_args* a, const ddk_inpaint_args* ip, ddk_stream_t s);
size_t ddk_sampler_restore_workspace_bytes(const ddk_unet* u, int B, int H, int W, int t_start);
int ddk_sampler_restore_tail_parts(const ddk_unet* u, int B, int H, int W, int n);
int ddk_sampler_run_restore(const ddk_sampler_args* a, const int64_t* timestep_map, const float* y, int n, ddk_stream_t s);
size_t ddk_sampler_restore_masked_workspace_bytes(const ddk_unet* u, int B, int H, int W, int t_start, int n);
int ddk_sampler_restore_masked_tail_parts(const ddk_unet* u, int B, int H, int W, int n);
int ddk_sampler_run_restore_masked(const ddk_sampler_args* a, const int64_t* timestep_map, const float* y, const float* mask, int n,
                                   ddk_stream_t s);
size_t ddk_sampler_restore_multistep_workspace_bytes(const ddk_unet* u, int B, int H, int W, int t_start, int n);
int ddk_sampler_restore_multistep_tail_parts(const ddk_unet* u, int B, int H, int W, int n);
int ddk_sampler_run_restore_multistep(const ddk_sampler_args* a, const int64_t* timestep_map, const float* c3, const float* y,
                                      const float* mask, int n, ddk_stream_t s);
size_t ddk_sampler_restore_noisy_workspace_bytes(const ddk_unet* u, int B, int H, int W, int t_start, int n);
int ddk_sampler_restore_noisy_tail_parts(const ddk_unet* u, int B, int H, int W, int n);
int ddk_sampler_run_restore_noisy(const ddk_sampler_args* a, const int64_t* timestep_map, const float* lam, const float* sgm, const float* y,
                                  const float* mask, int n, ddk_stream_t s);
size_t ddk_sampler_restore_gray_workspace_bytes(const ddk_unet* u, int B, int H, int W, int t_start, int n);
int ddk_sampler_restore_gray_tail_parts(const ddk_unet* u, int B, int H, int W, int n);
int ddk_sampler_run_restore_gray(const ddk_sampler_args* a, const int64_t* timestep_map, const float* lam, const float* sgm, const float* y,
                                 const float* mask, int n, int weights, ddk_stream_t s);
size_t ddk_sampler_restore_blur_workspace_bytes(const ddk_unet* u, int B, int H, int W, int t_start);
int ddk_sampler_restore_blur_tail_parts(const ddk_unet* u, int B, int H, int W);
int ddk_sampler_run_restore_blur(const ddk_sampler_args* a, const int64_t* timestep_map, const float* P_h, const float* P_w, const float* Q_h,
                                 const float* Q_w, const float* y, ddk_stream_t s);
int ddk_sampler_run_restore_sep(const ddk_sampler_args* a, const int64_t* timestep_map, const float* P_h, const float* P_w, const float* Q_h,
                                const float* Q_w, const float* y, int h, int w, ddk_stream_t s);
int ddk_sampler_invalidate(ddk_unet* u);
int ddk_sampler_release_workspace(ddk_unet* u, const void* workspace);

typedef struct ddk_vlb_sweep_args {
    const ddk_unet* unet;
    const void* packed;
    const float* x;
    const float* noise;
    const float* sqrt_acp;
    const float* sqrt_1m_acp;
    const float* c_recip;
    const float* c_recipm1;
    const float* c1;
    const float* c2;
    const float* post_logvar;
// ... 152 lines not shown
```

Measured before the change: 26.43.

## Fold last transposed-conv upsample into final 3x3 conv via depth-to-space Winograd

Composes the final 4x4 stride-2 transposed conv with the following 3x3 conv into one 3x3 conv at low resolution that emits 4x channels, written out through a depth-to-space epilogue. Border pixels, where the composition does not hold, are fixed with a separate ring correction kernel. Folded weights are built at pack time. This removes the full-resolution intermediate activation and one conv launch, at the cost of four times as many output channels per low-res pixel and an extra ring kernel.

Result: no change. 26.65, median of 6 (+0.8%).

```diff
diff --git a/downsampled-diffusion_amd/csrc/conv_wino.hip b/downsampled-diffusion_amd/csrc/conv_wino.hip
--- a/downsampled-diffusion_amd/csrc/conv_wino.hip
+++ b/downsampled-diffusion_amd/csrc/conv_wino.hip
@@ -43,6 +43,9 @@
     const float* r1_w;
     const float* r1_b;
     int r1_cin, r1_ld;
+    int d2s_n;
+    FastDivU d2s_dn;
+    const float* ring;
 };
 
 constexpr int WBT = 32, WBN = 64;
@@ -535,6 +538,40 @@
     return wino_stats_shape_parts(B, H, W, cin, N, groups);
 }
 
+int conv_wino_d2s_parts(int B, int H, int W, int cin, int n_out, int groups, bool forced) {
+    const int N = 4 * n_out;
+    if (B <= 0 || n_out <= 0 || n_out % 4 || groups <= 0 || n_out % groups || !conv_wino_ok(DDK_CONV3X3_S1, H, W, cin, N) || N % 128) return 0;
+    const int cpg = n_out / groups, tpi = (H / 2) * (W / 2);
+    if (cpg % 4 || 128 % cpg || 128 / cpg > 8 || tpi % WBT || tpi / WBT > 8) return 0;
+    if ((long long)B * (2 * H) * (2 * W) * n_out >= (1LL << 29) || (long long)B * H * W * cin >= (1LL << 29)) return 0;
+    if (!forced && (wino_variant(B, H, W, N) != WINO_V_F || conv_wino_splits(B, H, W, cin, N) != 1)) return 0;
+    return 4 * (tpi / WBT);
+}
+int conv_wino_d2s_forward(const float* x, const float* wu, const float* bias, const float* ring, float* out, float* gn_partials, int B, int H,
+                          int W, int cin, int n_out, int groups, hipStream_t st) {
+    DDK_REQUIRE(x && wu && ring && out && aligned16(x) && aligned16(wu) && aligned16(bias) && aligned16(ring) && aligned16(out) &&
+                    (reinterpret_cast<uintptr_t>(gn_partials) & 7u) == 0, "conv(wino, depth-to-space): pointers");
+    DDK_REQUIRE(conv_wino_d2s_parts(B, H, W, cin, n_out, groups, true) > 0, "conv(wino, depth-to-space): shape");
+    WinoParams p{};
+    p.src0 = x; p.wu = wu; p.bias = bias; p.out = out;
+    p.c0 = cin; p.cin = cin;
+    p.B = B; p.H = H; p.W = W; p.TH = H / 2; p.TW = W / 2;
+    p.N = 4 * n_out; p.tiles = B * p.TH * p.TW;
+    p.chunks = cin / 32; p.chunks_per_split = p.chunks; p.splits = 1;
+    p.slab_stride = (long long)B * H * W * p.N;
+    p.dTW = make_fastdiv_u((unsigned)p.TW);
+    p.dTH = make_fastdiv_u((unsigned)p.TH);
+    p.d2s_n = n_out; p.d2s_dn = make_fastdiv_u((unsigned)n_out); p.ring = ring;
+    if (gn_partials) {
+        p.gn_part = reinterpret_cast<float2*>(gn_partials);
+        p.groups = 4 * groups;
+        p.cpg = n_out / groups;
+    }
+    dim3 grid((unsigned)ceil_div(p.tiles, WBT), (unsigned)(p.N / 128), 1u);
+    hipLaunchKernelGGL((conv3x3_wino2_kernel<2, 0, false, true>), grid, dim3(768), (size_t)W2<2>::LDS_FL * sizeof(float), st, p);
+    return check_launch("conv3x3_wino2_kernel<depth-to-space>");
+}
+
 bool convT_wino_ok(int H, int W, int cin, int N) {
     return H >= 2 && W >= 2 && H % 2 == 0 && W % 2 == 0 && cin > 0 && cin % 32 == 0 && N > 0 && N % WT_NT == 0;
 }
@@ -584,6 +621,8 @@
     DDK_HIP(hipFuncSetAttribute(reinterpret_cast<const void*>(&conv3x3_wino2_kernel<2, 0, false>), hipFuncAttributeMaxDynamicSharedMemorySize,
                                 (int)(W2<2>::LDS_FL * sizeof(float))));
     DDK_HIP(hipFuncSetAttribute(reinterpret_cast<const void*>(&conv3x3_wino2_kernel<2, 0, true>), hipFuncAttributeMaxDynamicSharedMemorySize,
+                                (int)(W2<2>::LDS_FL * sizeof(float))));
+    DDK_HIP(hipFuncSetAttribute(reinterpret_cast<const void*>(&conv3x3_wino2_kernel<2, 0, false, true>), hipFuncAttributeMaxDynamicSharedMemorySize,
                                 (int)(W2<2>::LDS_FL * sizeof(float))));
     DDK_HIP(hipFuncSetAttribute(reinterpret_cast<const void*>(&conv3x3_wino2_kernel<4, 0, false>), hipFuncAttributeMaxDynamicSharedMemorySize,
                                 (int)(W2<4>::LDS_FL * sizeof(float))));
diff --git a/downsampled-diffusion_amd/csrc/conv_wino2_kernel.inc b/downsampled-diffusion_amd/csrc/conv_wino2_kernel.inc
--- a/downsampled-diffusion_amd/csrc/conv_wino2_kernel.inc
+++ b/downsampled-diffusion_amd/csrc/conv_wino2_kernel.inc
@@ -36,8 +36,9 @@
 
 __device__ unsigned long long g_wino_timeline[12 * 8 * 2];
 
-template <int P, int DBG, bool CL>
+template <int P, int DBG, bool CL, bool D2S = false>
 __global__ __launch_bounds__(768) void conv3x3_wino2_kernel(const WinoParams p) {
+    static_assert(!D2S || (P == 2 && !CL), "depth-to-space epilogue: variant F, plain finish");
     using G = W2<P>;
     constexpr int NT = G::NT, SPC = G::SPC, SPR = G::SPR, STAGE = G::STAGE, V_FL = G::V_FL;
     extern __shared__ __attribute__((aligned(16))) float smem[];
@@ -373,6 +374,13 @@
     int opix[ITEMS];
     const int cq = tid & (QUADS - 1);
     const int gn = n0 + cq * 4;
+    int d2s_c = 0, d2s_py = 0, d2s_px = 0;
+    if constexpr (D2S) {
+        const int ph = (int)fdiv_u((unsigned)gn, p.d2s_dn);
+        d2s_c = gn - ph * p.d2s_n;
+        d2s_py = ph >> 1;
+        d2s_px = ph & 1;
+    }
 #pragma unroll
     for (int it = 0; it < ITEMS; ++it) {
         const int item = tid + it * 512;
@@ -399,6 +407,27 @@
         const int tx = g - (int)tmp * p.TW;
         const unsigned bq = fdiv_u(tmp, p.dTH);
         const int ty = (int)tmp - (int)bq * p.TH;
+        if constexpr (D2S) {
+            const int H2 = 2 * p.H, W2 = 2 * p.W;
+            const int Y = 2 * (2 * ty + a) + d2s_py, X = 4 * tx + d2s_px;
+            const long long o0 = (((long long)bq * H2 + Y) * W2 + X) * p.d2s_n + d2s_c;
+            if (p.bias) {
+                const float4 bb = *reinterpret_cast<const float4*>(p.bias + gn);
+                y0 = f4add(y0, bb);
+                y1 = f4add(y1, bb);
+            }
+            const int rrow = Y == 0 ? 0 : Y == H2 - 1 ? W2 : -1;
+            const long long rbase = (long long)bq * (2 * W2 + 2 * H2 - 4) * p.d2s_n + d2s_c;
+            const int r0 = rrow >= 0 ? rrow + X : X == 0 ? 2 * W2 + Y - 1 : -1;
+            const int r1 = rrow >= 0 ? rrow + X + 2 : X + 2 == W2 - 1 ? 2 * W2 + (H2 - 2) + Y - 1 : -1;
+            if (r0 >= 0) y0 = f4add(y0, *reinterpret_cast<const float4*>(p.ring + rbase + (long long)r0 * p.d2s_n));
+            if (r1 >= 0) y1 = f4add(y1, *reinterpret_cast<const float4*>(p.ring + rbase + (long long)r1 * p.d2s_n));
+            *reinterpret_cast<float4*>(p.out + o0) = y0;
+            *reinterpret_cast<float4*>(p.out + o0 + 2 * p.d2s_n) = y1;
+            keep[it][0] = y0;
+            keep[it][1] = y1;
+            continue;
+        }
         const long long o0 = ((((long long)bq * p.H + 2 * ty + a) * p.W) + 2 * tx) * p.N + gn;
         oo[it] = o0;
         opix[it] = ((int)bq * p.H + 2 * ty + a) * p.W + 2 * tx;
diff --git a/downsampled-diffusion_amd/csrc/ddk_internal.h b/downsampled-diffusion_amd/csrc/ddk_internal.h
--- a/downsampled-diffusion_amd/csrc/ddk_internal.h
+++ b/downsampled-diffusion_amd/csrc/ddk_internal.h
@@ -168,6 +168,17 @@
 int convT_wino_forward(const ddk_conv_args& a, int splits, hipStream_t st);
 int conv_wino_init_device();
 int conv_wino_stats_parts(int B, int H, int W, int cin, int N, int groups);
+int conv_wino_d2s_parts(int B, int H, int W, int cin, int n_out, int groups, bool forced);
+int conv_wino_d2s_forward(const float* x, const float* wu, const float* bias, const float* ring, float* out, float* gn_partials, int B, int H,
+                          int W, int cin, int n_out, int groups, hipStream_t st);
+struct UpFoldOps {
+    size_t wc, wu, bias, edge_w, edge_b;
+};
+UpFoldOps upsample_fold_floats(int C, int N);
+inline size_t upsample_fold_ring_floats(int B, int H, int W, int N) { return (size_t)B * (4 * H + 4 * W - 4) * N; }
+int upsample_fold_pack(const float* wt_packed, const float* bt, const float* w3_packed, const float* b3, float* wc, float* wu, float* bias4,
+                       float* edge_w, float* edge_b, int C, int N, hipStream_t st);
+int upsample_fold_ring(const float* x, const float* edge_w, const float* edge_b, float* ring, int B, int H, int W, int C, int N, hipStream_t st);
 bool conv_first_ok(int cin, int N, int H, int W, int groups);
 int conv_first(const float* x, const float* wp, const float* bias, float* out, float* gn_partials, int B, int H, int W, int cin, int N,
                int groups, int64_t* counter, int64_t* t_cur, hipStream_t st);
diff --git a/downsampled-diffusion_amd/csrc/unet_plan.hip b/downsampled-diffusion_amd/csrc/unet_plan.hip
--- a/downsampled-diffusion_amd/csrc/unet_plan.hip
+++ b/downsampled-diffusion_amd/csrc/unet_plan.hip
@@ -118,6 +118,9 @@
     int level_chain_max_batch = 32;
     int attn_fold_min_hw = 256;
     bool attn_fold = true;
+    bool up_fold = true;
+    bool has_uf = false;
+    size_t uf_wc = 0, uf_wu = 0, uf_bias = 0, uf_ew = 0, uf_eb = 0;
     bool generic = false;
     std::vector<int> dimp;
     std::vector<Slot> slots;
@@ -333,6 +336,11 @@
     }
     u->final_conv = u->add_conv("final_conv.0.block.0.", cfg->chan, cfg->chan, 3, true, true);
     u->final_norm = u->add_norm("final_conv.0.block.1.weight", "final_conv.0.block.1.bias", cfg->chan);
+    if (!u->generic && u->L >= 2 && u->final_conv.has_wu) {
+        const UpFoldOps o = upsample_fold_floats(cfg->chan, cfg->chan);
+        u->uf_wc = u->alloc(o.wc); u->uf_wu = u->alloc(o.wu); u->uf_bias = u->alloc(o.bias); u->uf_ew = u->alloc(o.edge_w); u->uf_eb = u->alloc(o.edge_b);
+        u->has_uf = true;
+    }
     if (u->generic) {
         u->final_w = u->alloc((size_t)cfg->in_ch * pad32(cfg->chan));
         u->slots.push_back(Slot{"final_conv.1.weight", (long long)cfg->in_ch * cfg->chan, PK_ROWS, u->final_w, cfg->in_ch, cfg->chan, 0, 0, 0,
@@ -411,6 +419,7 @@
         {DDK_OPT_FIRST_GROUPNORM, true, [](ddk_unet& p, int v) { p.first_gn = v != 0; }},
         {DDK_OPT_RESTORE_FUSED_TAIL, true, [](ddk_unet& p, int v) { p.restore_fused = v != 0; }},
         {DDK_OPT_ATTENTION_SPLIT, true, [](ddk_unet& p, int v) { p.attn_split = v != 0; }},
+        {DDK_OPT_UPSAMPLE_FINAL_FOLD, true, [](ddk_unet& p, int v) { p.up_fold = v != 0; }},
         {DDK_OPT_LEVEL_CHAIN, true, [](ddk_unet& p, int v) {
              p.level_chain = v == 1 ? 9 : v == 2 ? 1 : v == 3 ? 15 : v == 4 ? 6 : v == 8 ? 2 : v == 16 ? 4 : v != 0 ? 9 : 0;
          }},
@@ -474,6 +483,18 @@
     return qkv_operand_pack(P + a.qkv_lnw, P + a.qkv_op, HEADS, pad32(a.c), st);
 }
 
+static int fold_upsample(const ddk_unet& u, float* P, hipStream_t st) {
+    const ConvW& t = u.up_conv.back();
+    return upsample_fold_pack(P + t.w, P + t.b, P + u.final_conv.w, P + u.final_conv.b, P + u.uf_wc, P + u.uf_wu, P + u.uf_bias, P + u.uf_ew,
+                              P + u.uf_eb, u.cfg.chan, u.cfg.chan, st);
+}
+static bool feeds_upsample_fold(const ddk_unet& u, const Slot& sl) {
+    if (!u.has_uf) return false;
+    const ConvW& t = u.up_conv.back();
+    return (sl.kind == PK_CONVT && sl.off == t.w) || (sl.kind == PK_CONV && sl.off == u.final_conv.w) ||
+           (sl.kind == PK_COPY && (sl.off == t.b || sl.off == u.final_conv.b));
+}
+
 static void weights_changed(const ddk_unet* u) {
     ddk_unet* m = const_cast<ddk_unet*>(u);
     std::lock_guard<std::mutex> lock(m->mu);
@@ -484,6 +505,7 @@
     DDK_REQUIRE(u && packed, "unet_finalize_pack: arguments");
     weights_changed(u);
     for (const AttnW& a : u->attn_all) DDK_TRY(fold_attn(a, static_cast<float*>(packed), as_stream(s)));
+    if (u->has_uf) DDK_TRY(fold_upsample(*u, static_cast<float*>(packed), as_stream(s)));
     return DDK_OK;
 }
 
@@ -521,6 +543,7 @@
     }
     DDK_TRY(rc);
     if (sl.attn >= 0) DDK_TRY(fold_attn(u->attn_all[sl.attn], static_cast<float*>(packed), as_stream(s)));
+    if (feeds_upsample_fold(*u, sl)) DDK_TRY(fold_upsample(*u, static_cast<float*>(packed), as_stream(s)));
     return DDK_OK;
 }
 
@@ -528,11 +551,11 @@
 
 struct Layout {
     size_t act = 0;
-    size_t qkv = 0, o = 0, ctx = 0, splitk = 0, gn_ws = 0, cl = 0, chain = 0;
+    size_t qkv = 0, o = 0, ctx = 0, splitk = 0, gn_ws = 0, cl = 0, chain = 0, ring = 0;
     std::vector<size_t> skip;
     size_t xpad = 0, temb = 0, tact = 0;
     size_t off_A = 0, off_B = 0, off_C = 0, off_raw = 0, off_a1 = 0, off_res = 0, off_xn = 0, off_qkv = 0, off_o = 0, off_ctx = 0,
-           off_splitk = 0, off_gn = 0, off_xpad = 0, off_temb = 0, off_tact = 0, off_cl = 0, off_chain = 0;
+           off_splitk = 0, off_gn = 0, off_xpad = 0, off_temb = 0, off_tact = 0, off_cl = 0, off_chain = 0, off_ring = 0;
     std::vector<size_t> off_skip;
     size_t total = 0;
 };
@@ -638,7 +661,8 @@
     upd(ly.splitk, conv3_ws_floats(u.final_conv, B, H, W, pad32(u.cfg.chan), pad32(u.cfg.chan)));
     upd(ly.gn_ws, groupnorm_workspace_bytes(B, H * W, pad32(u.cfg.chan), GROUPS) / 4);
     upd(ly.gn_ws, (size_t)2 * GROUPS * ((size_t)B * H * W / 128 + 1));
-    ly.xpad = al4((size_t)B * H0 * W0 * pad32(u.cfg.in_ch));
+    if (u.has_uf) ly.ring = al4(upsample_fold_ring_floats(B, H / 2, W / 2, u.cfg.chan));
+    ly.xpad =al4((size_t)B * H0 * W0 * pad32(u.cfg.in_ch));
     ly.temb = al4((size_t)B * u.temb_total);
     ly.tact = al4((size_t)B * u.time_dim);
     ly.act = al4(ly.act); ly.qkv = al4(ly.qkv); ly.o = al4(ly.o); ly.ctx = al4(ly.ctx);
@@ -655,6 +679,7 @@
     ly.off_xpad = take(ly.xpad); ly.off_temb = take(ly.temb); ly.off_tact = take(ly.tact);
     ly.off_skip.resize(u.L);
     for (int l = 0; l < u.L; ++l) ly.off_skip[l] = take(ly.skip[l]);
+    ly.off_ring = take(ly.ring);
     ly.total = off;
     return ly;
 }
@@ -1018,6 +1043,17 @@
     return final_tail_ok(H * W, chan, GROUPS, n_out, npf, kind, W, restore_n) ? npf : 0;
 }
 
+static int upsample_fold_parts(const ddk_unet& u, int B, int H0, int W0, StepKind kind, int restore_n = 0) {
+    if (!u.up_fold || !u.has_uf || u.generic || H0 % 2 || W0 % 2) return 0;
+    if (u.L == 2 && level_chain_shape_ok(u, H0, W0)) return 0;
+    const int chan = u.cfg.chan;
+    const int np = conv_wino_d2s_parts(B, H0 / 2, W0 / 2, chan, chan, GROUPS, false);
+    if (np <= 0) return 0;
+    int tail = fused_tail_parts(u, B, H0, W0, u.dimp[1], kind, restore_n);
+    if (tail == 0 && restore_kind(kind)) tail = fused_tail_parts(u, B, H0, W0, u.dimp[1], StepKind::Eps);
+    return np == tail ? np : 0;
+}
+
 __global__ __launch_bounds__(256) void step_prepare_kernel(const float* __restrict__ x, float* __restrict__ xpad, long long total,
                                                            int C, int c_pad, int64_t* __restrict__ counter,
                                                            int64_t* __restrict__ t_cur, int B) {
@@ -1166,6 +1202,20 @@
         DDK_TRY(run_res(c, u.mid2, bufC, cur_c, nullptr, 0, bufA, H, W));
         cur = bufA;
     }
+    const int chan = u.generic ? pad32(u.cfg.chan) : u.cfg.chan, n_out = u.cfg.in_ch;
+    StepRule plain{};
+    plain.kind = StepKind::Eps;
+    plain.eps_out = out;
+    const StepRule& rule = step ? step->rule : plain;
+    ChainHooks hooks{};
+    if (step) {
+        hooks.chain_state = step->state;
+        hooks.dec_counter = dec_counter;
+    }
+    const int npf = fused_tail_parts(u, B, H0, W0, u.dimp[1], rule.kind, rule.rst.n);
+    const int npe = (npf == 0 && step && restore_kind(rule.kind)) ? fused_tail_parts(u, B, H0, W0, u.dimp[1], StepKind::Eps) : 0;
+    const bool one_launch_tail = (npf > 0 || npe > 0) && (!step || step->per == (long long)H0 * W0 * n_out);
+    const bool folded = one_launch_tail && upsample_fold_parts(u, B, H0, W0, rule.kind, rule.rst.n) > 0 && !(chain_edges && u.L == 2);
     for (int i = 0; i < u.L - 1; ++i) {
         const int lvl = u.L - 1 - i;
         const float* skip = ws + ly.off_skip[lvl];
@@ -1177,26 +1227,19 @@
             DDK_TRY(run_res(c, u.up_res[2 * i + 1], bufB, din, nullptr, 0, bufC, H, W));
             DDK_TRY(run_attn(c, u.up_attn[i], bufC, bufB, H, W));
         }
-        if (!(chain_edges && i == 0))
+        if (folded && i == u.L - 2) {
+            float* ring = ws + ly.off_ring;
+            DDK_TRY(upsample_fold_ring(bufB, P + u.uf_ew, P + u.uf_eb, ring, B, H, W, din, chan, st));
+            DDK_TRY(conv_wino_d2s_forward(bufB, P + u.uf_wu, P + u.uf_bias, ring, raw, gnp, B, H, W, din, chan, GROUPS, st));
+        } else if (!(chain_edges && i == 0)) {
             DDK_TRY(run_conv(c, DDK_CONVT4X4_S2, u.up_conv[i], bufB, din, nullptr, 0, nullptr, bufA, H, W, din));
+        }
         H *= 2; W *= 2;
         cur = bufA;
         cur_c = din;
     }
-    const int chan = u.generic ? pad32(u.cfg.chan) : u.cfg.chan, n_out = u.cfg.in_ch;
-    StepRule plain{};
-    plain.kind = StepKind::Eps;
-    plain.eps_out = out;
-    const StepRule& rule = step ? step->rule : plain;
-    ChainHooks hooks{};
-    if (step) {
-        hooks.chain_state = step->state;
-        hooks.dec_counter = dec_counter;
-    }
-    const int npf = fused_tail_parts(u, B, H, W, cur_c, rule.kind, rule.rst.n);
-    const int npe = (npf == 0 && step && restore_kind(rule.kind)) ? fused_tail_parts(u, B, H, W, cur_c, StepKind::Eps) : 0;
-    if ((npf > 0 || npe > 0) && (!step || step->per == (long long)H * W * n_out)) {
-        DDK_TRY(run_conv_parts(c, u.final_conv, cur, cur_c, nullptr, 0, raw, H, W, chan));
+    if (one_launch_tail) {
+        if (!folded) DDK_TRY(run_conv_parts(c, u.final_conv, cur, cur_c, nullptr, 0, raw, H, W, chan));
         const TailIn in{raw, gnp, npf > 0 ? npf : npe, P + u.final_norm.g, P + u.final_norm.b, GN_EPS, P + u.final_w, P + u.final_b, n_out, B, H * W, chan, GROUPS};
         if (npf > 0) return final_tail(in, rule, t, hooks, st);
         StepRule eps_only{};
@@ -1319,6 +1362,7 @@
         f += 2.0 * 2.0 * B * HEADS * 32.0 * 32.0 * H * W;
     };
     int H = H0, W = W0, cur_c = pad32(u->cfg.in_ch);
+    const bool folded = upsample_fold_parts(*u, B, H0, W0, StepKind::Eps) > 0;
     for (int l = 0; l < u->L; ++l) {
         const int co = u->dims[l + 1];
         res(u->down_res[2 * l], H, W, cur_c, 0, l == 0 && first_fast(*u, B, H, W));
@@ -1333,15 +1377,24 @@
         res(u->up_res[2 * i], H, W, cur_c, dout, false);
         res(u->up_res[2 * i + 1], H, W, din, 0, false);
         attn(u->up_attn[i], H, W);
-        if (u->up_conv[i].has_wu && convT_wino_use(B, H, W, din, din))
+        if (folded && i == u->L - 2) {
+            f += 2.0 * (double)(ceil_div((long long)B * (H / 2) * (W / 2), 32) * 32) * 16.0 * din * 4.0 * u->cfg.chan;
+            f += 2.0 * B * (4.0 * H + 4.0 * W - 4.0) * 3.0 * din * u->cfg.chan;
+        } else if (u->up_conv[i].has_wu && convT_wino_use(B, H, W, din, din))
             f += 2.0 * (double)(ceil_div((long long)B * (H / 2) * (W / 2), 32) * 32) * 36.0 * din * din;
         else
             f += conv_flops(DDK_CONVT4X4_S2, B, H, W, din, din);
         H *= 2; W *= 2;
         cur_c = din;
     }
-    f += conv3(u->final_conv, H, W, cur_c, 0, u->cfg.chan) + 2.0 * B * H * W * (double)u->cfg.chan * u->cfg.in_ch;
+    if (!folded) f += conv3(u->final_conv, H, W, cur_c, 0, u->cfg.chan);
+    f += 2.0 * B * H * W * (double)u->cfg.chan * u->cfg.in_ch;
     return f;
+}
+
+extern "C" int ddk_unet_upsample_fold_parts(const ddk_unet* u, int B, int H, int W) {
+    if (check_shape(u, B, H, W) != DDK_OK) return 0;
+    return upsample_fold_parts(*u, B, H, W, StepKind::Eps);
 }
 
 namespace ddk {
diff --git a/downsampled-diffusion_amd/csrc/upsample_fold.hip b/downsampled-diffusion_amd/csrc/upsample_fold.hip
--- /dev/null
+++ b/downsampled-diffusion_amd/csrc/upsample_fold.hip
@@ -0,0 +1,283 @@
+#include "conv_common.h"
+
+namespace ddk {
+
+constexpr int UF_JOBS = 12;
+
+__device__ __forceinline__ float uf_w3(const float* __restrict__ w3p, int C, int n, int m, int ky, int kx) {
+    return w3p[((long long)n * 9 + ky * 3 + kx) * C + m];
+}
+__device__ __forceinline__ float uf_wt(const float* __restrict__ wtp, int C, int c, int m, int ty, int tx) {
+    const int py = 1 - (ty & 1), a = ty >> 1, px = 1 - (tx & 1), b = tx >> 1;
+    return wtp[((((long long)(py * 2 + px)) * C + m) * 4 + (a * 2 + b)) * C + c];
+}
+
+__global__ __launch_bounds__(256) void upfold_compose_kernel(const float* __restrict__ wtp, const float* __restrict__ w3p, float* __restrict__ wc,
+                                                             int C, int N) {
+    const long long idx = blockIdx.x * 256LL + threadIdx.x;
+    if (idx >= 4LL * N * C) return;
+    const int c = (int)(idx % C), np = (int)(idx / C), n = np % N, ph = np / N, py = ph >> 1, px = ph & 1;
+    double acc[9];
+#pragma unroll
+    for (int i = 0; i < 9; ++i) acc[i] = 0.0;
+    for (int m = 0; m < C; ++m) {
+        float g[9];
+#pragma unroll
+        for (int i = 0; i < 9; ++i) g[i] = uf_w3(w3p, C, n, m, i / 3, i % 3);
+#pragma unroll
+        for (int dy = 0; dy < 3; ++dy)
+#pragma unroll
+            for (int dx = 0; dx < 3; ++dx)
+#pragma unroll
+                for (int ky = 0; ky < 3; ++ky)
+#pragma unroll
+                    for (int kx = 0; kx < 3; ++kx) {
+                        const int ty = py + ky - 2 * dy + 2, tx = px + kx - 2 * dx + 2;
+                        if (ty >= 0 && ty < 4 && tx >= 0 && tx < 4)
+                            acc[dy * 3 + dx] += (double)g[ky * 3 + kx] * (double)uf_wt(wtp, C, c, m, ty, tx);
+                    }
+    }
+#pragma unroll
+    for (int i = 0; i < 9; ++i) wc[idx * 9 + i] = (float)acc[i];
+}
+
+__device__ __forceinline__ void uf_rep(int job, int t, int& Y, int& X, int& iy, int& ix) {
+    if (job < 8) {
+        const int e = job >> 1, p = job & 1;
+        if (e == 0) { Y = 0; X = 8 + p; iy = 0; ix = 3 + t; }
+        else if (e == 1) { Y = 15; X = 8 + p; iy = 7; ix = 3 + t; }
+        else if (e == 2) { Y = 8 + p; X = 0; iy = 3 + t; ix = 0; }
+        else { Y = 8 + p; X = 15; iy = 3 + t; ix = 7; }
+    } else {
+        const int k = job - 8, bot = k >> 1, rgt = k & 1;
+        Y = bot ? 15 : 0; X = rgt ? 15 : 0;
+        iy = (bot ? 7 : 0) + (t == 2 ? (bot ? -1 : 1) : 0);
+        ix = (rgt ? 7 : 0) + (t == 1 ? (rgt ? -1 : 1) : 0);
+    }
+}
+
+__global__ __launch_bounds__(256) void upfold_edge_kernel(const float* __restrict__ wtp, const float* __restrict__ w3p, float* __restrict__ ew,
+                                                          int C, int N) {
+    const long long idx = blockIdx.x * 256LL + threadIdx.x;
+    if (idx >= (long long)UF_JOBS * 3 * N * C) return;
+    const int c = (int)(idx % C);
+    long long r = idx / C;
+    const int n = (int)(r % N); r /= N;
+    const int t = (int)(r % 3), job = (int)(r / 3);
+    int Y, X, iy, ix;
+    uf_rep(job, t, Y, X, iy, ix);
+    double acc = 0.0;
+    for (int ky = 0; ky < 3; ++ky)
+        for (int kx = 0; kx < 3; ++kx) {
+            const int qy = Y + ky - 1, qx = X + kx - 1;
+            if (qy >= 0 && qy < 16 && qx >= 0 && qx < 16) continue;
+            const int ty = qy + 1 - 2 * iy, tx = qx + 1 - 2 * ix;
+            if (ty < 0 || ty > 3 || tx < 0 || tx > 3) continue;
+            for (int m = 0; m < C; ++m) acc += (double)uf_w3(w3p, C, n, m, ky, kx) * (double)uf_wt(wtp, C, c, m, ty, tx);
+        }
+    const int chunk = t * (C / 8) + c / 8, lane = (n & 31) + 32 * ((c & 7) >> 2);
+    ew[((((long long)job * (N / 32) + n / 32) * (3 * C / 8) + chunk) * 64 + lane) * 4 + (c & 3)] = (float)-acc;
+}
+
+__global__ __launch_bounds__(256) void upfold_bias_kernel(const float* __restrict__ w3p, const float* __restrict__ bt, const float* __restrict__ b3,
+                                                          float* __restrict__ eb, float* __restrict__ bias4, int C, int N) {
+    const int idx = blockIdx.x * 256 + threadIdx.x;
+    if (idx >= (UF_JOBS + 4) * N) return;
+    const int n = idx % N, job = idx / N;
+    int Y = 8, X = 8, iy, ix;
+    if (job < UF_JOBS) uf_rep(job, 0, Y, X, iy, ix);
+    double acc = 0.0;
+    for (int ky = 0; ky < 3; ++ky)
+        for (int kx = 0; kx < 3; ++kx) {
+            const int qy = Y + ky - 1, qx = X + kx - 1;
+            const bool inside = qy >= 0 && qy < 16 && qx >= 0 && qx < 16;
+            if ((job < UF_JOBS) == inside || !bt) continue;
+            for (int m = 0; m < C; ++m) acc += (double)uf_w3(w3p, C, n, m, ky, kx) * (double)bt[m];
+        }
+    if (job < UF_JOBS) eb[idx] = (float)-acc;
+    else bias4[idx - UF_JOBS * N] = (float)(acc + (b3 ? (double)b3[n] : 0.0));
+}
+
+struct RingParams {
+    const float* x;
+    const float* ew;
+    const float* eb;
+    float* ring;
+    int B, H, W, C, N;
+    int ks;
+    FastDivU dH, dW;
+};
+__device__ float g_uf_trash[32];
+struct RingRow { int b, pix[3], ring; };
+
+__device__ __forceinline__ RingRow uf_row(const RingParams& p, int job, int R) {
+    RingRow o;
+    const int H = p.H, W = p.W;
+    if (job >= 8) {
+        const int k = job - 8, bot = k >> 1, rgt = k & 1;
+        const int cy = bot ? H - 1 : 0, cx = rgt ? W - 1 : 0;
+        o.b = R;
+        o.pix[0] = cy * W + cx;
+        o.pix[1] = cy * W + cx + (rgt ? -1 : 1);
+        o.pix[2] = (cy + (bot ? -1 : 1)) * W + cx;
+        o.ring = (bot ? 2 * W : 0) + (rgt ? 2 * W - 1 : 0);
+        return o;
+    }
+    const int e = job >> 1, ph = job & 1, L = e < 2 ? W : H;
+    o.b = (int)fdiv_u((unsigned)R, e < 2 ? p.dW : p.dH);
+    const int j = R - o.b * L, pos = 2 * j + ph;
+#pragma unroll
+    for (int t = 0; t < 3; ++t) {
+        const int jj = j + t - 1;
+        o.pix[t] = (jj < 0 || jj >= L) ? -1 : e == 0 ? jj : e == 1 ? (H - 1) * W + jj : e == 2 ? jj * W : jj * W + W - 1;
+    }
+    const bool corner = pos == 0 || pos == 2 * L - 1;
+    o.ring = corner ? -1 : e == 0 ? pos : e == 1 ? 2 * W + pos : e == 2 ? 4 * W + pos - 1 : 4 * W + (2 * H - 2) + pos - 1;
+    return o;
+}
+
+__global__ __launch_bounds__(512) void upfold_ring_kernel(const RingParams p) {
+    __shared__ float red[7 * 16 * 64];
+    __shared__ int rowoff[32];
+    int job, tile_m, tile_n;
+    {
+        const int nwg = gridDim.x * gridDim.y * gridDim.z;
+        const int bid = blockIdx.x + gridDim.x * (blockIdx.y + gridDim.y * blockIdx.z);
+        const int q = nwg >> 3, r = nwg & 7, xcd = bid & 7, idx = bid >> 3;
+        const int logical = (xcd < r ? xcd * (q + 1) : r * (q + 1) + (xcd - r) * q) + idx;
+        tile_m = logical % gridDim.x;
+        const int rest = logical / gridDim.x;
+        tile_n = rest % gridDim.y;
+        job = rest / gridDim.y;
+    }
+    const int lane = threadIdx.x & 63;
+    const int wid = __builtin_amdgcn_readfirstlane(threadIdx.x >> 6);
+    const int KS = p.ks, NTW = 8 / KS;
+    const int nw = wid & (NTW - 1), ks = wid / NTW;
+    const int rows = job >= 8 ? p.B : p.B * (job < 4 ? p.W : p.H);
+    const int R0 = tile_m * 32;
+    if (R0 >= rows) return;
+    const int ntile = tile_n * NTW + nw;
+    const bool n_ok = ntile < p.N / 32;
+    const int cpt = p.C / 8, CH = 3 * cpt;
+    f32x16 acc;
+#pragma unroll
+    for (int r = 0; r < 16; ++r) acc[r] = 0.f;
+    const int rlen = 4 * p.H + 4 * p.W - 4;
+    const int R = R0 + (lane & 31), h = lane >> 5;
+    RingRow me = uf_row(p, job, R < rows ? R : R0);
+    if (R >= rows) { me.pix[0] = me.pix[1] = me.pix[2] = -1; me.ring = -1; }
+    if (wid == 0 && lane < 32) rowoff[lane] = me.ring < 0 ? -1 : me.b * rlen + me.ring;
+    if (n_ok) {
+        const float* xb = p.x + (long long)me.b * p.H * p.W * p.C + 4 * h;
+        const float* wj = p.ew + (((long long)job * (p.N / 32) + ntile) * CH * 64 + lane) * 4;
+        float4 a[6], b[6];
+        auto load = [&](float4 (&av)[6], float4 (&bv)[6], int q0) {
+#pragma unroll
+            for (int t = 0; t < 3; ++t)
+#pragma unroll
+                for (int j = 0; j < 2; ++j) {
+                    const int px = me.pix[t], q = q0 + j;
+                    const float4 v = *reinterpret_cast<const float4*>(xb + (long long)(px < 0 ? 0 : px) * p.C + 8 * q);
+                    av[t * 2 + j] = make_float4(px < 0 ? 0.f : v.x, px < 0 ? 0.f : v.y, px < 0 ? 0.f : v.z, px < 0 ? 0.f : v.w);
+                    bv[t * 2 + j] = *reinterpret_cast<const float4*>(wj + (long long)(t * cpt + q) * 256);
+                }
+        };
+        const int q_begin = ks * (cpt / KS), q_end = q_begin + cpt / KS;
+        load(a, b, q_begin);
+        for (int q0 = q_begin; q0 < q_end; q0 += 2) {
+            float4 an[6] = {}, bn[6] = {};
+            if (q0 + 2 < q_end) load(an, bn, q0 + 2);
+#pragma unroll
+            for (int i = 0; i < 6; ++i) {
+                acc = __builtin_amdgcn_mfma_f32_32x32x2f32(a[i].x, b[i].x, acc, 0, 0, 0);
+                acc = __builtin_amdgcn_mfma_f32_32x32x2f32(a[i].y, b[i].y, acc, 0, 0, 0);
+                acc = __builtin_amdgcn_mfma_f32_32x32x2f32(a[i].z, b[i].z, acc, 0, 0, 0);
+                acc = __builtin_amdgcn_mfma_f32_32x32x2f32(a[i].w, b[i].w, acc, 0, 0, 0);
+            }
+#pragma unroll
+            for (int i = 0; i < 6; ++i) { a[i] = an[i]; b[i] = bn[i]; }
+        }
+    }
+    if (ks > 0) {
+#pragma unroll
+        for (int r = 0; r < 16; ++r) red[(((ks - 1) * NTW + nw) * 16 + r) * 64 + lane] = acc[r];
+    }
+    __syncthreads();
+    if (ks > 0 || !n_ok) return;
+    for (int k = 1; k < KS; ++k) {
+#pragma unroll
+        for (int r = 0; r < 16; ++r) acc[r] += red[(((k - 1) * NTW + nw) * 16 + r) * 64 + lane];
+    }
+    const int n = ntile * 32 + (lane & 31);
+    const float bias = p.eb[job * p.N + n];
+    float* trash = g_uf_trash + (lane & 31);
+#pragma unroll
+    for (int r = 0; r < 16; ++r) {
+        const int off = rowoff[(r & 3) + 8 * (r >> 2) + 4 * h];
+        float* dst = off >= 0 ? p.ring + (long long)off * p.N + n : trash;
+        *dst = acc[r] + bias;
+    }
+}
+
+UpFoldOps upsample_fold_floats(int C, int N) {
+    UpFoldOps o;
+    o.wc = (size_t)4 * N * C * 9;
+    o.wu = (size_t)16 * 4 * N * C;
+    o.bias = (size_t)4 * N;
+    o.edge_w = (size_t)UF_JOBS * 3 * N * C;
+    o.edge_b = (size_t)UF_JOBS * N;
+    return o;
+}
+
+int upsample_fold_pack(const float* wtp, const float* bt, const float* w3p, const float* b3, float* wc, float* wu, float* bias4, float* edge_w,
+                       float* edge_b, int C, int N, hipStream_t st) {
+    DDK_REQUIRE(wtp && w3p && wc && wu && bias4 && edge_w && edge_b && C > 0 && C % 32 == 0 && N > 0 && N % 32 == 0,
+                "upsample_fold_pack: arguments (C % 32 == 0, N % 32 == 0)");
+    hipLaunchKernelGGL(upfold_compose_kernel, dim3((unsigned)ceil_div(4LL * N * C, 256)), dim3(256), 0, st, wtp, w3p, wc, C, N);
+    DDK_TRY(check_launch("upfold_compose_kernel"));
+    DDK_TRY(ddk_pack_conv_weight_wino(wc, wu, 4 * N, C, C, st));
+    hipLaunchKernelGGL(upfold_edge_kernel, dim3((unsigned)ceil_div((long long)UF_JOBS * 3 * N * C, 256)), dim3(256), 0, st, wtp, w3p, edge_w, C, N);
+    DDK_TRY(check_launch("upfold_edge_kernel"));
+    hipLaunchKernelGGL(upfold_bias_kernel, dim3((unsigned)ceil_div((long long)(UF_JOBS + 4) * N, 256)), dim3(256), 0, st, w3p, bt, b3, edge_b, bias4,
+                       C, N);
+    return check_launch("upfold_bias_kernel");
+}
+
+int upsample_fold_ring(const float* x, const float* edge_w, const float* edge_b, float* ring, int B, int H, int W, int C, int N, hipStream_t st) {
+    DDK_REQUIRE(x && edge_w && edge_b && ring && aligned16(x) && aligned16(edge_w) && B > 0 && H >= 2 && W >= 2 && C > 0 && C % 32 == 0 &&
+                    N > 0 && N % 32 == 0, "upsample_fold_ring: arguments (H, W >= 2, C % 32 == 0, N % 32 == 0)");
+    const int ks = C % 128 == 0 ? 8 : C % 64 == 0 ? 4 : 2;
+    RingParams p{x, edge_w, edge_b, ring, B, H, W, C, N, ks, make_fastdiv_u((unsigned)H), make_fastdiv_u((unsigned)W)};
+    const dim3 grid((unsigned)ceil_div((long long)B * (H > W ? H : W), 32), (unsigned)ceil_div(N / 32, 8 / ks), UF_JOBS);
+    hipLaunchKernelGGL(upfold_ring_kernel, grid, dim3(512), 0, st, p);
+    return check_launch("upfold_ring_kernel");
+}
+
+}
+
+using namespace ddk;
+
+extern "C" size_t ddk_upsample_fold_floats(int C, int N, int which) {
+    if (C <= 0 || N <= 0 || C % 32 || N % 32) return 0;
+    const UpFoldOps o = upsample_fold_floats(C, N);
+    return which == 0 ? o.wc : which == 1 ? o.wu : which == 2 ? o.bias : which == 3 ? o.edge_w : which == 4 ? o.edge_b : 0;
+}
+
+extern "C" int ddk_upsample_fold_pack(const float* wt_packed, const float* bt, const float* w3_packed, const float* b3, float* wc, float* wu,
+                                      float* bias4, float* edge_w, float* edge_b, int C, int N, ddk_stream_t s) {
+    return upsample_fold_pack(wt_packed, bt, w3_packed, b3, wc, wu, bias4, edge_w, edge_b, C, N, as_stream(s));
+}
+
+extern "C" int ddk_upsample_fold_parts(int B, int H, int W, int C, int N, int groups) {
+    return (C > 0 && C % 32 == 0 && N > 0 && N % 32 == 0) ? conv_wino_d2s_parts(B, H, W, C, N, groups, true) : 0;
+}
+
+extern "C" int ddk_upsample_fold_forward(const float* x, const float* wu, const float* bias4, const float* edge_w, const float* edge_b,
+                                         float* ring, float* out, float* gn_partials, int B, int H, int W, int C, int N, int groups,
+                                         ddk_stream_t s) {
+    DDK_REQUIRE(ddk_upsample_fold_parts(B, H, W, C, N, groups) > 0, "upsample_fold_forward: shape not eligible (ddk_upsample_fold_parts)");
+    DDK_TRY(ensure_device_init());
+    DDK_TRY(upsample_fold_ring(x, edge_w, edge_b, ring, B, H, W, C, N, as_stream(s)));
+    return conv_wino_d2s_forward(x, wu, bias4, ring, out, gn_partials, B, H, W, C, N, groups, as_stream(s));
+}
diff --git a/downsampled-diffusion_amd/ddk/lib.py b/downsampled-diffusion_amd/ddk/lib.py
--- a/downsampled-diffusion_amd/ddk/lib.py
+++ b/downsampled-diffusion_amd/ddk/lib.py
@@ -180,6 +180,11 @@
     "ddk_conv3x3_gn_mish_cluster_split_workspace_bytes": (_SZ, [_I, _I, _I, _I, _I, _I]),
     "ddk_conv3x3_gn_mish_cluster": (_I, [_P, _I, _P, _I, _P, _P, _P, _P, _P, _I, _P, _P, _I, _I, _I, _I, _I, _F, _P, _SZ, _P]),
     "ddk_unet_set_option": (_I, [_P, _I, _I]),
+    "ddk_unet_upsample_fold_parts": (_I, [_P, _I, _I, _I]),
+    "ddk_upsample_fold_floats": (_SZ, [_I, _I, _I]),
+    "ddk_upsample_fold_pack": (_I, [_P, _P, _P, _P, _P, _P, _P, _P, _P, _I, _I, _P]),
+    "ddk_upsample_fold_parts": (_I, [_I, _I, _I, _I, _I, _I]),
+    "ddk_upsample_fold_forward": (_I, [_P, _P, _P, _P, _P, _P, _P, _P, _I, _I, _I, _I, _I, _I, _P]),
     "ddk_debug_cluster_timeouts": (C.c_uint, []),
     "ddk_conv3x3_gn_mish_cluster_check": (_I, [_P, _I, _P]),
     "ddk_unet_cluster_check": (_I, [_P, _P, _I, _I, _I, _P]),
diff --git a/downsampled-diffusion_amd/ddk/plan.py b/downsampled-diffusion_amd/ddk/plan.py
--- a/downsampled-diffusion_amd/ddk/plan.py
+++ b/downsampled-diffusion_amd/ddk/plan.py
@@ -102,6 +102,7 @@
     OPT_FIRST_GROUPNORM = 8
     OPT_RESTORE_FUSED_TAIL = 12
     OPT_ATTENTION_SPLIT = 13
+    OPT_UPSAMPLE_FINAL_FOLD = 14
 
     def set_option(self, option, value):
         L.check(self._lib.ddk_unet_set_option(self.handle, option, int(value)), "unet_set_option")
@@ -163,6 +164,9 @@
 
     def flops_executed(self, b, h, w):
         return self._lib.ddk_unet_flops_executed(self.handle, b, h, w)
+
+    def upsample_fold_parts(self, b, h, w):
+        return int(self._lib.ddk_unet_upsample_fold_parts(self.handle, b, h, w))
 
     def forward_nhwc(self, x, t):
         if self.packed is None:
diff --git a/include/ddk.h b/include/ddk.h
--- a/include/ddk.h
+++ b/include/ddk.h
@@ -116,6 +116,12 @@
                                 const float* gamma, const float* beta, const float* temb, int temb_stride, const float* addend,
                                 float* out, int B, int H, int W, int N, int groups, float eps, void* workspace, size_t workspace_bytes,
                                 ddk_stream_t s);
+size_t ddk_upsample_fold_floats(int C, int N, int which);
+int ddk_upsample_fold_pack(const float* wt_packed, const float* bt, const float* w3_packed, const float* b3, float* wc, float* wu,
+                           float* bias4, float* edge_w, float* edge_b, int C, int N, ddk_stream_t s);
+int ddk_upsample_fold_parts(int B, int H, int W, int C, int N, int groups);
+int ddk_upsample_fold_forward(const float* x, const float* wu, const float* bias4, const float* edge_w, const float* edge_b, float* ring,
+                              float* out, float* gn_partials, int B, int H, int W, int C, int N, int groups, ddk_stream_t s);
 int ddk_chan_layernorm(const float* x, const float* g, const float* b, float* out, long long M, int C,
                        float eps, ddk_stream_t s);
 int ddk_mish(const float* x, float* out, long long n, ddk_stream_t s);
@@ -236,7 +242,9 @@
 #define DDK_OPT_FIRST_GROUPNORM 8
 #define DDK_OPT_RESTORE_FUSED_TAIL 12
 #define DDK_OPT_ATTENTION_SPLIT 13
+#define DDK_OPT_UPSAMPLE_FINAL_FOLD 14
 int ddk_unet_set_option(ddk_unet* u, int option, int value);
+int ddk_unet_upsample_fold_parts(const ddk_unet* u, int B, int H, int W);
 int ddk_unet_cluster_check(const ddk_unet* u, void* workspace, int B, int H, int W, ddk_stream_t s);
 unsigned ddk_debug_cluster_timeouts(void);
 int ddk_debug_clock_probe(unsigned long long* out, int workgroups, ddk_stream_t s);
```
